# OpenMendel/MendelIHT.jl

Measured on NVIDIA B200. Metric: iht_iterations_per_sec, higher is better.
Workload: dtype f64 (sweep: f32 LUT partials per slab of 640 samples (512 without the ternary copy), f64 across slabs; top-k candidates re-scored in f64)

## Files before the change

mendeliht.jl_b200/csrc/common.cuh:

```cuda
#pragma once
#include <cuda_runtime.h>
#include <stdint.h>
#include <stdio.h>
#include <memory>
#include <string>
#include <vector>
#include <stdexcept>
#include "../../include/ihtb200.h"

namespace ihtb {

struct Error : std::runtime_error {
    int code;
    Error(int c, const std::string& m) : std::runtime_error(m), code(c) {}
};
void set_last_error(const std::string& m);
const std::string& last_error();
struct LaunchCounter {
    int64_t v = 0;
    LaunchCounter& operator++(int) { __atomic_fetch_add(&v, 1, __ATOMIC_RELAXED); return *this; }
    operator int64_t() const { return __atomic_load_n(&v, __ATOMIC_RELAXED); }
};
LaunchCounter& launch_counter();
bool debug_sync();

#define IHTB_CUDA(call)                                                                      \
    do {                                                                                     \
        cudaError_t e__ = (call);                                                            \
        if (e__ != cudaSuccess)                                                              \
            throw ::ihtb::Error(IHTB_ECUDA, std::string(#call) + ": " + cudaGetErrorString(e__)); \
    } while (0)

#define IHTB_CHECK(cond, code, msg)                                  \
    do {                                                             \
        if (!(cond)) throw ::ihtb::Error((code), (msg));             \
    } while (0)

#define IHTB_LAUNCH(kernel, grid, block, smem, stream, ...)          \
    do {                                                             \
        kernel<<<(grid), (block), (smem), (stream)>>>(__VA_ARGS__);  \
        ::ihtb::launch_counter()++;                                  \
        IHTB_CUDA(cudaGetLastError());                               \
        if (::ihtb::debug_sync()) {                                  \
            cudaError_t e2__ = cudaStreamSynchronize(stream);        \
            if (e2__ != cudaSuccess)                                 \
                throw ::ihtb::Error(IHTB_ECUDA, std::string("kernel " #kernel " failed: ") + cudaGetErrorString(e2__)); \
        }                                                            \
    } while (0)

template <typename F>
static inline int32_t guard(F&& f) {
    try {
        f();
        return IHTB_OK;
    } catch (const Error& e) {
        set_last_error(e.what());
        return e.code;
    } catch (const std::bad_alloc&) {
        set_last_error("out of host memory");
        return IHTB_ENOMEM;
    } catch (const std::exception& e) {
        set_last_error(e.what());
        return IHTB_EINVAL;
    }
}

template <typename T>
struct DBuf {
    T* p = nullptr;
    size_t n = 0;
    DBuf() = default;
    explicit DBuf(size_t count) { alloc(count); }
    DBuf(const DBuf&) = delete;
    DBuf& operator=(const DBuf&) = delete;
    ~DBuf() { release(); }
    void alloc(size_t count) {
        release();
        n = count;
        if (count) {
            cudaError_t e = cudaMalloc((void**)&p, count * sizeof(T));
            if (e != cudaSuccess) {
                p = nullptr; n = 0;
                throw Error(IHTB_ENOMEM, std::string("cudaMalloc of ") + std::to_string(count * sizeof(T)) +
                                             " bytes failed: " + cudaGetErrorString(e));
            }
        }
    }
    void release() {
        if (p) cudaFree(p);
        p = nullptr; n = 0;
    }
    void zero(cudaStream_t s) { if (n) IHTB_CUDA(cudaMemsetAsync(p, 0, n * sizeof(T), s)); }
};

template <typename T>
struct HBuf {
    T* p = nullptr;
    size_t n = 0;
    HBuf() = default;
    HBuf(const HBuf&) = delete;
    HBuf& operator=(const HBuf&) = delete;
    ~HBuf() { if (p) cudaFreeHost(p); }
    void alloc(size_t count) {
        if (p) cudaFreeHost(p);
        p = nullptr; n = count;
        if (count) IHTB_CUDA(cudaMallocHost((void**)&p, count * sizeof(T)));
    }
};

static inline int64_t ceil_div(int64_t a, int64_t b) { return (a + b - 1) / b; }

bool smem_attr_needed(const void* kernel, int device);
template <typename K>
static inline void ensure_dynamic_smem(K kernel, int bytes) {
    int dev = 0;
    IHTB_CUDA(cudaGetDevice(&dev));
    if (!smem_attr_needed(reinterpret_cast<const void*>(kernel), dev)) return;
    IHTB_CUDA(cudaFuncSetAttribute(kernel, cudaFuncAttributeMaxDynamicSharedMemorySize, bytes));
}

struct TopkFuse;
ihtb_geno* dense_new_handle(int64_t n, int64_t p, int dtype, int standardize, int32_t den = 0);
void dense_upload(ihtb_geno* g, const void* x, int64_t ld_host, int64_t j_dst, int64_t ncols);
void dense_finalize(ihtb_geno* g);
int64_t dense_stream_bytes(const ihtb_geno* g);
void dense_decode_block(const ihtb_geno* g, int64_t i0, int64_t i1, int64_t j0, int64_t j1, double* d_out);
void dense_xt_v(const ihtb_geno* g, const double* dV, int64_t m, double* dOut, cudaStream_t s, DBuf<double>* part,
                const TopkFuse* tf);
void dense_sweep_kernel_only(const ihtb_geno* g, const double* dV, DBuf<double>* part, cudaStream_t s);
void dense_x_support(const ihtb_geno* g, const int64_t* d_idx, int64_t k, const double* d_coef, int64_t m,
                     double* d_out, cudaStream_t s);
void dense_xt_gather2(const ihtb_geno* g, const int64_t* d_cols_a, int64_t n_a, const int64_t* d_cols_b, int64_t n_b,
                      const double* d_v, int64_t m, double* d_out, cudaStream_t s);
void dense_init_beta_moments(const ihtb_geno* g, const double* d_w, const double* d_wy, double* d_sx, double* d_sxx,
                             double* d_sxy, cudaStream_t s);
void dense_decode_cols(const ihtb_geno* g, const int64_t* d_cols, int64_t k, double* d_out, cudaStream_t s);
const double* geno_bound_scale(const ihtb_geno* g);
double geno_bound_coef(const ihtb_geno* g, double plink_coef);

}

enum { GENO_PLINK = 0, GENO_DENSE = 1 };

struct ihtb_geno {
    int kind = 0;
    int device = 0;
    int64_t n = 0;
    int64_t p = 0;
    int64_t j0 = 0;
    int64_t nbytes = 0;
    int64_t stride = 0;
    int64_t cs_j = 0, cs_s = 0;
    int quad = 0;
    int64_t p4 = 0;
    int center = 1, scale = 1, impute = 1;
    int sm_count = 148;
    ihtb::DBuf<uint8_t> bed;
    ihtb::DBuf<uint8_t> tern;
    int64_t tern_slabs = 0;
    ihtb::DBuf<double> mu, sinv;
    ihtb::DBuf<double> sgn;
    ihtb::DBuf<int32_t> nmiss;
    ihtb::DBuf<int64_t> miss_ptr;
    ihtb::DBuf<int32_t> miss_idx;
    int64_t total_missing = 0;
    bool ready = false;
    int dtype = 0;
    int standardize = 0;
    int32_t den = 0;
    int64_t ld = 0;
    ihtb::DBuf<uint8_t> dense;
    ihtb::DBuf<double> dscale;
    double dcoef = 0.0;
    std::shared_ptr<void> bgen_stage;
};
static inline bool geno_is_dense(const ihtb_geno* g) { return g->kind == GENO_DENSE; }

static inline void geno_require_ready(const ihtb_geno* g) {
    IHTB_CHECK(g && g->ready, IHTB_EINVAL, "genotype handle is not finalized (ihtb_geno_finalize)");
}

struct GenoView {
    const uint8_t* bed;
    int64_t cs_j, cs_s, nbytes, stride, n, p;
    int quad;
    const double* mu;
    const double* sinv;
    const int32_t* nmiss;
    int impute;
};
static inline GenoView geno_view(const ihtb_geno* g) {
    return GenoView{g->bed.p, g->cs_j, g->cs_s, g->nbytes, g->stride, g->n, g->p, g->quad, g->mu.p, g->sinv.p,
                    g->nmiss.p, g->impute};
}
__device__ __forceinline__ const uint8_t* gv_ptr(const GenoView& g, int64_t j, int64_t b) {
    if (g.quad)
        return g.bed + (b >> 7) * g.cs_s + (j >> 2) * 512 + ((b & 127) >> 2) * 16 + (j & 3) * 4 + (b & 3);
    return g.bed + j * g.cs_j + (b >> 7) * g.cs_s + (b & 127);
}

namespace ihtb {

__device__ __forceinline__ double warp_sum(double v) {
#pragma unroll
    for (int o = 16; o > 0; o >>= 1) v += __shfl_xor_sync(0xffffffffu, v, o);
    return v;
}
__device__ __forceinline__ float warp_sum(float v) {
#pragma unroll
    for (int o = 16; o > 0; o >>= 1) v += __shfl_xor_sync(0xffffffffu, v, o);
    return v;
}
__device__ __forceinline__ int warp_sum(int v) {
#pragma unroll
    for (int o = 16; o > 0; o >>= 1) v += __shfl_xor_sync(0xffffffffu, v, o);
    return v;
}

__device__ __forceinline__ double block_sum(double v, double* sh) {
    v = warp_sum(v);
    int lane = threadIdx.x & 31, w = threadIdx.x >> 5;
    __syncthreads();
    if (lane == 0) sh[w] = v;
    __syncthreads();
    int nw = (blockDim.x + 31) >> 5;
    v = (threadIdx.x < nw) ? sh[threadIdx.x] : 0.0;
    if (w == 0) v = warp_sum(v);
    return v;
}

void sweep_xt_v(const ihtb_geno* g, const double* dV, int64_t m, double* dOut, int mode, cudaStream_t s,
                double* sweep_seconds);
void x_support(const ihtb_geno* g, const int64_t* d_idx_local, int64_t k, const double* d_coef, int64_t m,
               double* d_out, cudaStream_t s);
void xt_gather(const ihtb_geno* g, const int64_t* d_cols_local, int64_t ncols, const double* d_v, int64_t m,
               const double* d_vsum , double* d_out , cudaStream_t s);
void xt_gather2(const ihtb_geno* g, const int64_t* d_cols_a, int64_t n_a, const int64_t* d_cols_b, int64_t n_b,
                const double* d_v, int64_t m, const double* d_vsum, double* d_out, cudaStream_t s, bool blocked = false);

struct TopkFuse;
void dense_xt_v(const ihtb_geno* g, const double* dV, int64_t m, double* dOut, cudaStream_t s, void* scratch_any,
                const TopkFuse* tf);
void dense_x_support(const ihtb_geno* g, const int64_t* d_idx, int64_t k, const double* d_coef, int64_t m,
                     double* d_out, cudaStream_t s);
void dense_xt_gather2(const ihtb_geno* g, const int64_t* d_cols_a, int64_t n_a, const int64_t* d_cols_b, int64_t n_b,
                      const double* d_v, int64_t m, double* d_out, cudaStream_t s);
void dense_init_beta_moments(const ihtb_geno* g, const double* d_w, const double* d_wy, double* d_sx, double* d_sxx,
                             double* d_sxy, cudaStream_t s, void* scratch_any);
void dense_decode_cols(const ihtb_geno* g, const int64_t* d_cols, int64_t k, double* d_out, cudaStream_t s);
const double* geno_bound_scale(const ihtb_geno* g);
double geno_bound_coef(const ihtb_geno* g, double plink_coef);

}
```

mendeliht.jl_b200/csrc/fit.cu:

```cuda
#include "glm.cuh"
#include "topk.cuh"
#include "comm.cuh"
#include "debias.cuh"
#include "groups.cuh"
#include "pairer.cuh"
#include <algorithm>
#include <chrono>
#include <cmath>
#include <memory>
#include <mutex>
#include <string.h>
#include <unordered_map>

namespace ihtb {
void sweep_xt_v_with_means(const ihtb_geno* g, const double* dV, const double* vbar_host, int64_t m, double* dOut,
                           int mode, cudaStream_t s, void* scratch_any, float* sweep_ms, double* d_l2 = nullptr,
                           const TopkFuse* tf = nullptr);
void* sweep_scratch_create();
void sweep_scratch_destroy(void* p);
void sweep_class_sums(const ihtb_geno* g, const double* d_v, double* d_w1, double* d_w2, double* d_wm, cudaStream_t s,
                      void* scratch_any);
}

using namespace ihtb;

static const double kFastBound = 1.0 / 262144.0;
static const double kExactBound = 1e-13;
static const double kPairBound = 3.1 / 2048.0;

struct ihtb_fit {
    const ihtb_geno* g = nullptr;
    int device = 0;
    int64_t n = 0, p = 0, q = 0;
    ihtb_comm* comm = nullptr;
    int64_t j0 = 0, p_global = 0;
    std::vector<int64_t> shard_j0;
    DBuf<int64_t> d_selall, d_pack, d_packall;
    HBuf<int64_t> h_selall, h_packall;
    int capx = 512;
    ihtb_cfg cfg{};
    cudaStream_t s = nullptr;
    std::vector<uint8_t> zkeep;
    int zkeepn = 0;
    int cap = 4096;

    DBuf<unsigned> d_done;
    DBuf<double> d_y, d_z, d_w, d_xb, d_zc, d_mu, d_r, d_xs, d_dfa, d_part, d_scal, d_small, d_coef, d_gout,
        d_vbar;
    DBuf<uint8_t> d_mask;
    DBuf<uint32_t> d_keyL, d_keyU;
    DBuf<int> d_hist;
    DBuf<int64_t> d_sel;
    DBuf<int64_t> d_idx, d_cols;
    HBuf<double> h_scal, h_gout;
    HBuf<int64_t> h_sel;
    void* sweep_scratch = nullptr;
    cudaEvent_t ev0 = nullptr, ev1 = nullptr, tm0 = nullptr, tm1 = nullptr;
    bool sweep_pending = false;
    struct FusedStep {
        std::vector<int64_t> uni_loc;
        size_t maxsupp = 0;
        int M = 0;
        int winner = -1;
    };
    FusedStep* fz = nullptr;
    DBuf<double> d_pick;
    HBuf<double> h_pick;
    SweepPairer* pairer = nullptr;
    int pair_slot = 0;
    double sweep_coef = kFastBound;
    GlmCtx glm{};
    TopkCtx tk{};

    std::vector<int64_t> idx, idx0, best_idx;
    std::vector<double> b, b0, best_b;
    std::vector<double> c, c0, best_c, df2, h_y, h_mu;
    std::vector<uint8_t> idc, idc0;
    std::unordered_map<int64_t, double> df_exact;
    std::vector<double> wt;
    DBuf<double> d_wt;
    double w_at(int64_t j) const { return wt.empty() ? 1.0 : wt[(size_t)j]; }
    void set_weights(const double* w) {
        if (!w) { wt.clear(); tk.wt = nullptr; return; }
        for (int64_t j = 0; j < p_global; ++j)
            IHTB_CHECK(w[j] > 0.0 && std::isfinite(w[j]), IHTB_EDOMAIN, "weights must be positive and finite");
        wt.assign(w, w + p_global);
        if (d_wt.n < (size_t)p) d_wt.alloc((size_t)p);
        IHTB_CUDA(cudaMemcpyAsync(d_wt.p, wt.data() + j0, (size_t)p * sizeof(double), cudaMemcpyHostToDevice, s));
        sync();
        tk.wt = d_wt.p;
    }
    std::vector<int64_t> cand_cache;
    bool df_sparse = false;
    std::vector<int64_t> dfs_idx;
    std::vector<double> dfs_val;
    double rbar = 0.0, bound = 0.0, sum_w = 0.0, sum_wy = 0.0, last_dev = 0.0, denom_next = 0.0;
    bool denom_ready = false;
    bool inited = false;

    int64_t n_sweeps = 0, n_backtracks = 0, n_cand_iter = 0, n_pair_overflow = 0;
    int last_count = 0;
    double sweep_ms_total = 0.0;
    double pve = 0.0;

    ~ihtb_fit() {
        if (sweep_scratch) sweep_scratch_destroy(sweep_scratch);
        if (ev0) cudaEventDestroy(ev0);
        if (ev1) cudaEventDestroy(ev1);
        if (tm0) cudaEventDestroy(tm0);
        if (tm1) cudaEventDestroy(tm1);
        if (s) cudaStreamDestroy(s);
    }

    void sync() { IHTB_CUDA(cudaStreamSynchronize(s)); }
    void readback_scal(int nv) {
        IHTB_CUDA(cudaMemcpyAsync(h_scal.p, d_scal.p, nv * sizeof(double), cudaMemcpyDeviceToHost, s));
        sync();
    }
    template <typename T>
    void upload(T* dst, const T* src, size_t count) {
        if (count) IHTB_CUDA(cudaMemcpyAsync(dst, src, count * sizeof(T), cudaMemcpyHostToDevice, s));
    }

    bool is_local(int64_t j) const { return j >= j0 && j < j0 + p; }
    int nranks() const { return comm ? comm->nranks : 1; }

    void support_matvec(const std::vector<int64_t>& cols, const std::vector<double>& coef, double* d_out) {
        std::vector<int64_t> ii; std::vector<double> vv;
        for (size_t t = 0; t < cols.size(); ++t)
            if (coef[t] != 0.0 && is_local(cols[t])) { ii.push_back(cols[t] - j0); vv.push_back(coef[t]); }
        if (!ii.empty()) {
            upload(d_idx.p, ii.data(), ii.size());
            upload(d_coef.p, vv.data(), vv.size());
        }
        support_matvec_dev(ii.empty() ? nullptr : d_idx.p, (int64_t)ii.size(), d_coef.p, d_out);
    }

    void support_matvec_dev(const int64_t* d_idx_loc, int64_t k_loc, const double* d_coef_loc, double* d_out) {
        support_matvec_dev_m(d_idx_loc, k_loc, d_coef_loc, 1, d_out);
    }
    void support_matvec_dev_m(const int64_t* d_idx_loc, int64_t k_loc, const double* d_coef_loc, int m, double* d_out) {
        const size_t cnt = (size_t)n * (size_t)m;
        if (!comm) {
            if (k_loc > 0) x_support(g, d_idx_loc, k_loc, d_coef_loc, m, d_out, s);
            else IHTB_CUDA(cudaMemsetAsync(d_out, 0, cnt * sizeof(double), s));
            return;
        }
        if (m == 1 && p2p_pushall_ok(comm, cnt)) {
            if (k_loc > 0) x_support_push(g, d_idx_loc, k_loc, d_coef_loc, comm, s);
            else p2p_push(comm, nullptr, cnt, s);
            p2p_reduce(comm, d_out, cnt, s);
            return;
        }
        if (p2p_mapped(comm) && cnt <= comm->red_cap) {
            double* part = p2p_partial_ptr(comm);
            if (k_loc > 0) x_support(g, d_idx_loc, k_loc, d_coef_loc, m, part, s);
            else IHTB_CUDA(cudaMemsetAsync(part, 0, cnt * sizeof(double), s));
            p2p_allreduce_2phase(comm, cnt, d_out, s);
            return;
        }
        if (k_loc > 0) x_support(g, d_idx_loc, k_loc, d_coef_loc, m, d_out, s);
        else IHTB_CUDA(cudaMemsetAsync(d_out, 0, cnt * sizeof(double), s));
        comm_allreduce_sum_f64(comm, d_out, cnt, s);
    }

    void update_xb() { support_matvec(idx, b, d_xb.p); }

    double glm_update(int add_zc) {
        upload(d_small.p, c.data(), (size_t)q);
        glm_mu(glm, d_small.p, add_zc, s);
        readback_scal(3);
        double dev = h_scal.p[0], lp = h_scal.p[1], sw = h_scal.p[2];
        last_dev = dev;
        if (cfg.dist == IHTB_NORMAL) {
            double phi = dev / (double)n;
            double sigma = std::sqrt(phi);
            return -0.5 * (dev / phi) - sw * (0.5 * std::log(2.0 * M_PI) + std::log(sigma));
        }
        return lp;
    }

    static double digamma(double x) {
        double r = 0.0;
        while (x < 6.0) { r -= 1.0 / x; x += 1.0; }
        double f = 1.0 / (x * x);
        return r + std::log(x) - 0.5 / x -
               f * (1.0 / 12 - f * (1.0 / 120 - f * (1.0 / 252 - f * (1.0 / 240 - f * (1.0 / 132)))));
    }
    static double trigamma(double x) {
        double r = 0.0;
        while (x < 6.0) { r += 1.0 / (x * x); x += 1.0; }
        double f = 1.0 / (x * x);
        return r + 1.0 / x + f / 2 + f / x * (1.0 / 6 - f * (1.0 / 30 - f * (1.0 / 42 - f * (1.0 / 30))));
    }
    void fetch_mu() {
        h_mu.resize((size_t)n);
        IHTB_CUDA(cudaMemcpyAsync(h_mu.data(), d_mu.p, n * sizeof(double), cudaMemcpyDeviceToHost, s));
        sync();
    }
    double nb_logl(double r) {
        glm.nb_r = r;
        return glm_update(1);
    }
    void mle_for_r() {
        fetch_mu();
        const std::vector<double>& y = h_y;
        double r = glm.nb_r;
        if (cfg.est_r == 1) {
            double num = 0.0, den = 0.0;
            for (int64_t i = 0; i < n; ++i) {
                for (int64_t j = 0; j <= (int64_t)y[i] - 1; ++j) num += r / (r + (double)j);
                den += std::log(r / (r + h_mu[i]));
            }
            glm.nb_r = -num / den;
            return;
        }
        auto d1 = [&](double rr) {
            double a = 0.0;
            for (int64_t i = 0; i < n; ++i)
                a += -(y[i] + rr) / (h_mu[i] + rr) - std::log(h_mu[i] + rr) + 1.0 + std::log(rr) + digamma(rr + y[i]) -
                     digamma(rr);
            return a;
        };
        auto d2 = [&](double rr) {
            double a = 0.0;
            for (int64_t i = 0; i < n; ++i)
                a += (y[i] + rr) / ((h_mu[i] + rr) * (h_mu[i] + rr)) - 2.0 / (h_mu[i] + rr) + 1.0 / rr +
                     trigamma(rr + y[i]) - trigamma(rr);
            return a;
        };
        double new_r = 1.0, stepsize = 1.0;
        for (int it = 0; it < 100; ++it) {
            double dx = d1(r), dx2 = d2(r);
            double increment = dx2 < 0 ? dx / dx2 : dx;
            new_r = r - stepsize * increment;
            double old_logl = nb_logl(r);
            for (int j = 0; j < 20; ++j) {
                if (new_r <= 0) {
                    stepsize /= 2; new_r = r - stepsize * increment;
                } else {
                    double new_logl = nb_logl(new_r);
                    if (old_logl >= new_logl) { stepsize /= 2; new_r = r - stepsize * increment; }
                    else break;
                }
            }
            if (std::fabs(r - new_r) <= 1e-6) { glm.nb_r = new_r; return; }
            r = new_r;
        }
        glm.nb_r = r;
    }
    double mu_r_logl() {
        double l = glm_update(1);
        if (cfg.est_r != 0) {
            mle_for_r();
            l = glm_update(1);
        }
        return l;
    }

    void exact_df(const std::vector<int64_t>& cols, bool exchange = true) {
        std::vector<int64_t> need;
        for (int64_t j : cols)
            if (!df_exact.count(j) && (exchange || is_local(j))) need.push_back(j);
        if (need.empty()) { if (!exchange) sync(); return; }
        IHTB_CHECK((int64_t)need.size() <= (int64_t)d_cols.n, IHTB_ENUMERIC, "too many columns to re-score");
        std::vector<int64_t> loc(need.size());
        for (size_t t = 0; t < need.size(); ++t) loc[t] = is_local(need[t]) ? need[t] - j0 : -1;
        upload(d_cols.p, loc.data(), loc.size());
        xt_gather2(g, d_cols.p, (int64_t)need.size(), nullptr, 0, d_r.p, 1, d_vbar.p, d_gout.p, s,
                   false);
        if (exchange) comm_allreduce_sum_f64(comm, d_gout.p, need.size(), s);
        IHTB_CUDA(cudaMemcpyAsync(h_gout.p, d_gout.p, need.size() * sizeof(double), cudaMemcpyDeviceToHost, s));
        sync();
        for (size_t t = 0; t < need.size(); ++t) df_exact[need[t]] = h_gout.p[t];
        n_cand_iter += (int64_t)need.size();
    }

    void score_and_sweep() {
        glm_score(glm, s, d_vbar.p);
        IHTB_CUDA(cudaMemcpyAsync(h_scal.p, d_scal.p, (2 + q) * sizeof(double), cudaMemcpyDeviceToHost, s));
        IHTB_CUDA(cudaEventRecord(ev0, s));
        sweep_coef = geno_bound_coef(g, cfg.sweep_mode == IHTB_SWEEP_FAST ? kFastBound : kExactBound);
        const double t_sw = now();
        if (pairer && cfg.sweep_mode == IHTB_SWEEP_FAST) {
            IHTB_CHECK(!grouped() && !comm, IHTB_EUNSUPPORTED, "paired sweeps serve plain single-device fits only");
            if (pairer->sweep(pair_slot, g, d_r.p, d_vbar.p, d_dfa.p, s, sweep_scratch)) {
                sweep_coef = kPairBound;
                IHTB_CUDA(cudaMemcpyAsync(h_scal.p + 3 + q, pairer->d_l2 + pair_slot, sizeof(double), cudaMemcpyDeviceToHost, s));
            }
        } else if (cfg.k > 0 && !(grouped() && !init_plain)) {
            const TopkFuse tf = topk_absdf_fuse_begin(tk, geno_bound_scale(g), d_scal.p, sweep_coef);
            sweep_xt_v_with_means(g, d_r.p, d_vbar.p, 1, d_dfa.p, cfg.sweep_mode, s, sweep_scratch, nullptr, nullptr, &tf);
        } else {
            sweep_xt_v_with_means(g, d_r.p, d_vbar.p, 1, d_dfa.p, cfg.sweep_mode, s, sweep_scratch, nullptr);
        }
        IHTB_CUDA(cudaEventRecord(ev1, s));
        ++n_sweeps;
        const double t_sel = now();
        dbg[0] += t_sel - t_sw;
        select_rescore(false);
        dbg[1] += now() - t_sel;
    }

    void select_rescore(bool rerun) {
        if (grouped() && !init_plain) {
            select_groups(rerun);
            if (!rerun) finish_sweep_scalars(sweep_coef);
            return;
        }
        df_exact.clear(); cand_cache.clear();
        df_sparse = false;
        const double coef = sweep_coef;
        std::vector<std::pair<int64_t, double>> cvals;
        const bool fused = fz != nullptr && !rerun;
        std::vector<int64_t> supp_loc;
        if (fused) supp_loc = fz->uni_loc;
        else
            for (int64_t j : idx)
                if (is_local(j)) supp_loc.push_back(j - j0);
        const int nsupp = (int)supp_loc.size();
        const int64_t* d_supp = fused ? d_idx.p : d_cols.p;
        int glaunch = 0;
        if (cfg.k > 0) {
            const int64_t ksel = cfg.k + (int64_t)(fused ? fz->maxsupp : idx.size());
            const bool paired = coef == kPairBound;
            if (tk.fused_hist) topk_candidates_absdf_finish(tk, ksel, s);
            else
                topk_candidates_absdf(tk, d_dfa.p, paired ? g->sgn.p : geno_bound_scale(g), rerun ? nullptr : d_scal.p, coef, ksel, s,
                                      bound, (paired && !rerun) ? pairer->d_l2 + pair_slot : nullptr);
            const int64_t want = sweep_coef == kPairBound ? std::max<int64_t>(ksel + 1024, last_count + last_count / 4 + 256)
                                                          : ksel + 64;
            glaunch = (int)std::min<int64_t>(comm ? capx / 2 : cap, want);
        }
        if (nsupp && !fused) upload(d_cols.p, supp_loc.data(), supp_loc.size());
        xt_gather2(g, tk.cand, glaunch, d_supp, nsupp, d_r.p, 1, d_vbar.p, d_gout.p, s);
        denom_ready = false;
        if (!rerun) {
            if (fused) {
                glm_winner_coef(d_pick.p, d_coefM.p, nsupp, d_gout.p + glaunch, d_coef.p, d_cM.p, q, d_small.p + q, s);
                support_matvec_dev(d_supp, nsupp, d_coef.p, d_xs.p);
                IHTB_CUDA(cudaMemcpyAsync(h_pick.p, d_pick.p, (size_t)(1 + fz->M) * sizeof(double), cudaMemcpyDeviceToHost, s));
                IHTB_CUDA(cudaMemcpyAsync(h_scalM.p, d_scalM.p, (size_t)(3 * fz->M) * sizeof(double), cudaMemcpyDeviceToHost, s));
            } else {
                support_matvec_dev(d_supp, nsupp, d_gout.p + glaunch, d_xs.p);
                std::vector<double> mask((size_t)q);
                for (int64_t l = 0; l < q; ++l) mask[l] = idc[l] ? 1.0 : 0.0;
                upload(d_small.p + q, mask.data(), (size_t)q);
            }
            glm_stepsize(glm, d_scal.p + 2, d_xs.p, s, d_small.p + q, d_scal.p + 2 + q);
            IHTB_CUDA(cudaMemcpyAsync(h_scal.p + 2 + q, d_scal.p + 2 + q, sizeof(double), cudaMemcpyDeviceToHost, s));
            denom_ready = true;
        }
        if (!comm) {
            IHTB_CUDA(cudaMemcpyAsync(h_sel.p, d_sel.p, (2 + glaunch) * sizeof(int64_t), cudaMemcpyDeviceToHost, s));
            IHTB_CUDA(cudaMemcpyAsync(h_gout.p, d_gout.p, (glaunch + nsupp) * sizeof(double), cudaMemcpyDeviceToHost, s));
            sync();
            const double t_host = now();
            struct Acc { double& a; double t0; ~Acc() { a += now() - t0; } } acc_host{dbg[2], t_host};
            if (fused) adopt_winner();
            const TopkState* st = reinterpret_cast<const TopkState*>(h_sel.p);
            const int count = cfg.k > 0 ? st->count : 0;
            dbg[3] += (double)std::min(count, glaunch);
            if (count > cap && coef == kPairBound && !rerun) {
                ++n_pair_overflow;
                sweep_coef = kFastBound;
                sweep_xt_v_with_means(g, d_r.p, d_vbar.p, 1, d_dfa.p, IHTB_SWEEP_FAST, s, sweep_scratch, nullptr);
                IHTB_CUDA(cudaEventRecord(ev1, s));
                select_rescore(false);
                return;
            }
            IHTB_CHECK(count <= cap, IHTB_ENUMERIC,
                       "degenerate projection: more than " + std::to_string(cap) +
                           " entries lie within the sweep error bound of the k-th largest |gradient|");
            last_count = count;
            cvals.reserve((size_t)count);
            for (int t = 0; t < std::min(count, glaunch); ++t) cvals.push_back({h_sel.p[2 + t], h_gout.p[t]});
            for (int t = 0; t < nsupp; ++t) df_exact[supp_loc[t] + j0] = h_gout.p[glaunch + t];
            if (count > glaunch) {
                IHTB_CUDA(cudaMemcpyAsync(h_sel.p, d_sel.p, (2 + count) * sizeof(int64_t), cudaMemcpyDeviceToHost, s));
                sync();
                std::vector<int64_t> rest(h_sel.p + 2 + glaunch, h_sel.p + 2 + count);
                exact_df(rest);
                for (int64_t j : rest) cvals.push_back({j, df_exact.at(j)});
            }
        } else {
            const int nr = nranks();
            const size_t blk = 2 + 2 * (size_t)capx;
            IHTB_CHECK(nsupp <= capx / 2, IHTB_ENUMERIC, "support too large for the sharded candidate exchange");
            pack_sweep_candidates(d_pack.p, reinterpret_cast<const TopkState*>(d_sel.p), tk.cand, glaunch, d_gout.p,
                                  d_supp, nsupp, d_gout.p + glaunch, j0, capx, s);
            comm_allgather_i64(comm, d_pack.p, d_packall.p, blk, s);
            IHTB_CUDA(cudaMemcpyAsync(h_packall.p, d_packall.p, nr * blk * sizeof(int64_t), cudaMemcpyDeviceToHost, s));
            sync();
            if (fused) adopt_winner();
            for (int r = 0; r < nr; ++r) {
                const int64_t* b_ = h_packall.p + (size_t)r * blk;
                IHTB_CHECK(b_[0] <= glaunch, IHTB_ENUMERIC,
                           "degenerate projection: too many local candidates within the sweep error bound");
                const int half = capx / 2;
                auto take = [&](int t, bool is_cand) {
                    const int64_t j = b_[2 + t];
                    if (j < 0) return;
                    double v;
                    memcpy(&v, &b_[2 + capx + t], sizeof(double));
                    if (is_cand) cvals.push_back({j, v});
                    else df_exact[j] = v;
                };
                for (int t = 0; t < (int)b_[0]; ++t) take(t, true);
                for (int t = 0; t < (int)b_[1]; ++t) take(half + t, false);
            }
        }
        std::sort(cvals.begin(), cvals.end());
        cvals.erase(std::unique(cvals.begin(), cvals.end(), [](const std::pair<int64_t, double>& x, const std::pair<int64_t, double>& y) {
                        return x.first == y.first; }), cvals.end());
        n_cand_iter += (int64_t)cvals.size();
        std::vector<char> keep(cvals.size(), 1);
        if ((int64_t)cvals.size() > cfg.k) {
            std::vector<std::pair<double, size_t>> outside;
            outside.reserve(cvals.size());
            for (size_t t = 0; t < cvals.size(); ++t)
                if (!std::binary_search(idx.begin(), idx.end(), cvals[t].first))
                    outside.push_back({std::fabs(cvals[t].second) * w_at(cvals[t].first), t});
            if ((int64_t)outside.size() > cfg.k) {
                std::nth_element(outside.begin(), outside.begin() + (cfg.k - 1), outside.end(),
                                 [](const std::pair<double, size_t>& x, const std::pair<double, size_t>& y) {
                                     return x.first > y.first;
                                 });
                const double thr = outside[(size_t)cfg.k - 1].first * (1.0 - 1e-12);
                std::fill(keep.begin(), keep.end(), 0);
                for (const auto& e : outside)
                    if (e.first >= thr) keep[e.second] = 1;
            }
        }
        for (size_t t = 0; t < cvals.size(); ++t)
            if (keep[t]) {
                cand_cache.push_back(cvals[t].first);
                df_exact[cvals[t].first] = cvals[t].second;
            }
        if (rerun) return;
        finish_sweep_scalars(coef);
    }

    void finish_sweep_scalars(double coef) {
        float ms = 0.f;
        IHTB_CUDA(cudaEventElapsedTime(&ms, ev0, ev1));
        sweep_ms_total += ms;
        double rsum = h_scal.p[0], rl1 = h_scal.p[1];
        for (int64_t l = 0; l < q; ++l) df2[l] = h_scal.p[2 + l];
        denom_next = h_scal.p[2 + q];
        rbar = rsum / (double)n;
        bound = coef == kPairBound ? coef * h_scal.p[3 + q]
                                   : coef * (rl1 + std::fabs(rsum));
    }

    double df_at(int64_t j) const {
        if (df_sparse) {
            auto it = std::lower_bound(dfs_idx.begin(), dfs_idx.end(), j);
            return (it != dfs_idx.end() && *it == j) ? dfs_val[it - dfs_idx.begin()] : 0.0;
        }
        return df_exact.at(j);
    }

    double stepsize() {
        std::vector<double> coef(idx.size());
        double numer = 0.0;
        for (size_t t = 0; t < idx.size(); ++t) { coef[t] = df_at(idx[t]); numer += coef[t] * coef[t]; }
        if (denom_ready && !df_sparse) {
            denom_ready = false;
            for (int64_t l = 0; l < q; ++l)
                if (idc[l]) numer += df2[l] * df2[l];
            double eta = numer / denom_next;
            if (std::isinf(eta) || std::isnan(eta)) eta = 1e-8;
            return eta;
        }
        denom_ready = false;
        support_matvec(idx, coef, d_xs.p);
        std::vector<double> d2((size_t)q);
        for (int64_t l = 0; l < q; ++l) {
            d2[l] = idc[l] ? df2[l] : 0.0;
            if (idc[l]) numer += df2[l] * df2[l];
        }
        upload(d_small.p + q, d2.data(), (size_t)q);
        glm_stepsize(glm, d_small.p + q, d_xs.p, s);
        readback_scal(1);
        double denom = h_scal.p[0];
        double eta = numer / denom;
        if (std::isinf(eta) || std::isnan(eta)) eta = 1e-8;
        return eta;
    }

    static double b_lookup(const std::vector<int64_t>& ii, const std::vector<double>& vv, int64_t j) {
        auto it = std::lower_bound(ii.begin(), ii.end(), j);
        return (it != ii.end() && *it == j) ? vv[it - ii.begin()] : 0.0;
    }

    void gradstep(double eta) {
        if (grouped()) { gradstep_group(eta); return; }
        std::vector<int64_t> cand;
        cand = df_sparse ? dfs_idx : cand_cache;
        cand.insert(cand.end(), idx0.begin(), idx0.end());
        std::sort(cand.begin(), cand.end());
        cand.erase(std::unique(cand.begin(), cand.end()), cand.end());

        struct Item { double a; int64_t pos; double v; };
        std::vector<Item> items;
        items.reserve(cand.size() + (size_t)q);
        for (int64_t j : cand) {
            double v = b_lookup(idx0, b0, j) + eta * df_at(j);
            if (!wt.empty()) {
                const double w = wt[(size_t)j], a = v * w;
                items.push_back({std::fabs(a), j, a / w});
            } else {
                items.push_back({std::fabs(v), j, v});
            }
        }
        for (int64_t l = 0; l < q; ++l) {
            c[l] = c0[l] + eta * df2[l];
            if (!zkeep[l]) items.push_back({std::fabs(c[l]), p_global + l, c[l]});
        }
        int64_t k = cfg.k;
        std::sort(items.begin(), items.end(), [](const Item& x, const Item& y) {
            return x.a > y.a || (x.a == y.a && x.pos < y.pos);
        });
        idx.clear(); b.clear();
        const double thr = project_threshold(items, k);
        std::vector<std::pair<int64_t, double>> keep;
        for (size_t t = 0; t < items.size(); ++t) {
            const bool kept = items[t].a >= thr;
            if (items[t].pos >= p_global) {
                if (!kept) c[items[t].pos - p_global] = 0.0;
            } else if (kept && items[t].v != 0.0) {
                keep.push_back({items[t].pos, items[t].v});
            }
        }
        for (int64_t l = 0; l < q; ++l) idc[l] = c[l] != 0.0;
        choose_prune(keep);
        std::sort(keep.begin(), keep.end());
        for (auto& kv : keep) { idx.push_back(kv.first); b.push_back(kv.second); }
    }

    template <typename ItemT>
    static double project_threshold(const std::vector<ItemT>& sorted_items, int64_t k) {
        if (k <= 0) return INFINITY;
        return (int64_t)sorted_items.size() >= k ? sorted_items[(size_t)k - 1].a : 0.0;
    }
    void choose_prune(std::vector<std::pair<int64_t, double>>& keep) const {
        int64_t nonzero = (int64_t)keep.size() - zkeepn;
        for (int64_t l = 0; l < q; ++l) nonzero += idc[l] ? 1 : 0;
        const int64_t limit = cfg.k + zkeepn;
        if (nonzero <= limit) return;
        std::vector<std::pair<int64_t, double>> byabs = keep;
        std::sort(byabs.begin(), byabs.end(), [](const std::pair<int64_t, double>& x, const std::pair<int64_t, double>& y) {
            return std::fabs(x.second) < std::fabs(y.second) || (std::fabs(x.second) == std::fabs(y.second) && x.first > y.first);
        });
        const size_t excess = std::min<size_t>((size_t)(nonzero - limit), byabs.size());
        for (size_t t = 0; t < excess; ++t) keep.erase(std::find(keep.begin(), keep.end(), byabs[t]));
    }

    std::unique_ptr<GroupCtx> grpctx;
    bool init_plain = false;
    bool grouped() const { return (bool)grpctx; }
    void set_groups(const int32_t* group1, int J, const int64_t* ks, int64_t n_groups) {
        if (!group1) { grpctx.reset(); return; }
        IHTB_CHECK(J >= 0, IHTB_EINVAL, "Value of J (max number of groups) must be nonnegative!");
        std::unique_ptr<GroupCtx> gc(new GroupCtx());
        std::vector<double> h_sinv((size_t)p);
        IHTB_CUDA(cudaMemcpy(h_sinv.data(), geno_bound_scale(g), (size_t)p * sizeof(double), cudaMemcpyDeviceToHost));
        gc->build(p, j0, p_global, group1, J, ks, n_groups, cfg.k, h_sinv.data());
        grpctx = std::move(gc);
    }

    void select_groups(bool rerun) {
        GroupCtx& gc = *grpctx;
        df_exact.clear(); cand_cache.clear();
        df_sparse = false; denom_ready = false;
        const double coef = sweep_coef;
        group_topk(gc, d_dfa.p, geno_bound_scale(g), rerun ? nullptr : d_scal.p, coef, bound, cfg.k, s);
        const size_t G = (size_t)gc.G, nT = 2 * G + 1;
        const int nr = nranks();
        std::vector<double> TL(G), TU(G);
        bool overflow = false;
        if (comm) {
            if (gc.d_Tall.n < nT * (size_t)nr) { gc.d_Tall.alloc(nT * (size_t)nr); gc.h_Tall.alloc(nT * (size_t)nr); }
            comm_allgather_i64(comm, reinterpret_cast<const int64_t*>(gc.d_gT.p), gc.d_Tall.p, nT, s);
            IHTB_CUDA(cudaMemcpyAsync(gc.h_Tall.p, gc.d_Tall.p, nT * (size_t)nr * sizeof(int64_t), cudaMemcpyDeviceToHost, s));
            sync();
            std::fill(TL.begin(), TL.end(), 0.0); std::fill(TU.begin(), TU.end(), 0.0);
            for (int rk = 0; rk < nr; ++rk) {
                const double* T = reinterpret_cast<const double*>(gc.h_Tall.p) + (size_t)rk * nT;
                for (size_t gi = 0; gi < G; ++gi) { TL[gi] = std::max(TL[gi], T[gi]); TU[gi] += T[G + gi]; }
                overflow = overflow || T[2 * G] != 0.0;
            }
        } else {
            IHTB_CUDA(cudaMemcpyAsync(gc.h_gT.p, gc.d_gT.p, nT * sizeof(double), cudaMemcpyDeviceToHost, s));
            sync();
            for (size_t gi = 0; gi < G; ++gi) { TL[gi] = gc.h_gT.p[gi]; TU[gi] = gc.h_gT.p[G + gi]; }
            overflow = gc.h_gT.p[2 * G] != 0.0;
        }
        IHTB_CHECK(!overflow, IHTB_ENUMERIC,
                   "degenerate group projection: too many entries of one group lie within the sweep error bound of its "
                   "2k-th largest |gradient|");
        std::vector<char> has(G, 0);
        for (int64_t j : idx) has[(size_t)gc.grp[(size_t)j]] = 1;
        std::vector<int32_t> chosen;
        std::vector<double> lows;
        for (size_t gi = 0; gi < G; ++gi) {
            if (has[gi]) chosen.push_back((int32_t)gi);
            else lows.push_back(TL[gi]);
        }
        if (gc.J > 0 && !lows.empty()) {
            const size_t need = std::min<size_t>((size_t)gc.J, lows.size());
            std::nth_element(lows.begin(), lows.begin() + (need - 1), lows.end(), std::greater<double>());
            const double thr = lows[need - 1];
            for (size_t gi = 0; gi < G; ++gi)
                if (!has[gi] && TU[gi] >= thr) chosen.push_back((int32_t)gi);
        }
        IHTB_CHECK(chosen.size() <= 65536, IHTB_ENUMERIC, "degenerate group projection: too many groups tie at the J-th norm");
        std::sort(chosen.begin(), chosen.end());
        const int nc = (int)chosen.size();
        const int64_t nsupp = (int64_t)idx.size();
        const int64_t list_slots = (int64_t)nc * gc.lcap, slots = list_slots + nsupp;
        if (slots == 0) return;
        gc.ensure_chosen(std::max(nc, 1));
        if (gc.d_oidx.n < (size_t)slots) {
            gc.d_oidx.alloc((size_t)slots); gc.d_oval.alloc((size_t)slots);
            gc.h_oidx.alloc((size_t)slots); gc.h_oval.alloc((size_t)slots);
        }
        if (nc) {
            IHTB_CUDA(cudaMemcpyAsync(gc.d_chosen.p, chosen.data(), (size_t)nc * sizeof(int32_t), cudaMemcpyHostToDevice, s));
            group_take(gc, nc, s);
        }
        std::vector<int64_t> supp_loc((size_t)nsupp);
        for (int64_t t = 0; t < nsupp; ++t) supp_loc[(size_t)t] = is_local(idx[(size_t)t]) ? idx[(size_t)t] - j0 : -1;
        upload(gc.d_oidx.p + list_slots, supp_loc.data(), (size_t)nsupp);
        xt_gather(g, gc.d_oidx.p, slots, d_r.p, 1, d_vbar.p, gc.d_oval.p, s);
        auto take = [&](int64_t t, int64_t j, double v) {
            if (j < 0) return;
            df_exact[j] = v;
            if (t < list_slots) cand_cache.push_back(j);
        };
        if (comm) {
            const size_t blk = 2 * (size_t)slots;
            if (gc.d_blk.n < blk) gc.d_blk.alloc(blk);
            if (gc.d_blkall.n < blk * (size_t)nr) { gc.d_blkall.alloc(blk * (size_t)nr); gc.h_blkall.alloc(blk * (size_t)nr); }
            group_pack(gc.d_oidx.p, gc.d_oval.p, slots, j0, gc.d_blk.p, s);
            comm_allgather_i64(comm, gc.d_blk.p, gc.d_blkall.p, blk, s);
            IHTB_CUDA(cudaMemcpyAsync(gc.h_blkall.p, gc.d_blkall.p, blk * (size_t)nr * sizeof(int64_t), cudaMemcpyDeviceToHost, s));
            sync();
            for (int rk = 0; rk < nr; ++rk) {
                const int64_t* b_ = gc.h_blkall.p + (size_t)rk * blk;
                for (int64_t t = 0; t < slots; ++t) {
                    double v;
                    memcpy(&v, &b_[slots + t], sizeof(double));
                    take(t, b_[t], v);
                }
            }
        } else {
            IHTB_CUDA(cudaMemcpyAsync(gc.h_oidx.p, gc.d_oidx.p, (size_t)slots * sizeof(int64_t), cudaMemcpyDeviceToHost, s));
            IHTB_CUDA(cudaMemcpyAsync(gc.h_oval.p, gc.d_oval.p, (size_t)slots * sizeof(double), cudaMemcpyDeviceToHost, s));
            sync();
            for (int64_t t = 0; t < slots; ++t) take(t, gc.h_oidx.p[t], gc.h_oval.p[t]);
        }
        std::sort(cand_cache.begin(), cand_cache.end());
        cand_cache.erase(std::unique(cand_cache.begin(), cand_cache.end()), cand_cache.end());
        n_cand_iter += (int64_t)cand_cache.size();
    }

    struct GItem { double a; int64_t j; double v; int g; };
    std::vector<std::pair<int64_t, double>> project_groups(std::vector<GItem>& items) const {
        const GroupCtx& gc = *grpctx;
        std::sort(items.begin(), items.end(), [](const GItem& x, const GItem& y) { return x.a > y.a || (x.a == y.a && x.j < y.j); });
        std::unordered_map<int, std::pair<int64_t, double>> acc;
        for (const GItem& it : items) {
            auto& e = acc[it.g];
            if (e.first < gc.k_of(it.g, cfg.k)) { e.second += it.v * it.v; ++e.first; }
        }
        std::vector<std::pair<double, int>> order;
        for (const auto& kv : acc) order.push_back({kv.second.second, kv.first});
        std::sort(order.begin(), order.end(), [](const std::pair<double, int>& x, const std::pair<double, int>& y) {
            return x.first > y.first || (x.first == y.first && x.second < y.second);
        });
        std::unordered_map<int, int> rank;
        for (size_t i = 0; i < order.size(); ++i) rank[order[i].second] = (int)i + 1;
        std::unordered_map<int, int64_t> cnt;
        std::vector<std::pair<int64_t, double>> keep;
        for (const GItem& it : items) {
            int64_t& c_ = cnt[it.g];
            if (rank[it.g] > gc.J || c_ >= gc.k_of(it.g, cfg.k)) continue;
            ++c_;
            if (it.v != 0.0) keep.push_back({it.j, it.v});
        }
        std::sort(keep.begin(), keep.end());
        return keep;
    }

    void gradstep_group(double eta) {
        const GroupCtx& gc = *grpctx;
        std::vector<int64_t> cand = df_sparse ? dfs_idx : cand_cache;
        cand.insert(cand.end(), idx0.begin(), idx0.end());
        std::sort(cand.begin(), cand.end());
        cand.erase(std::unique(cand.begin(), cand.end()), cand.end());
        std::vector<GItem> items;
        items.reserve(cand.size());
        for (int64_t j : cand) {
            const double v = b_lookup(idx0, b0, j) + eta * df_at(j);
            items.push_back({std::fabs(v), j, v, gc.grp[(size_t)j]});
        }
        for (int64_t l = 0; l < q; ++l) c[l] = c0[l] + eta * df2[l];
        auto keep = project_groups(items);
        for (int64_t l = 0; l < q; ++l) idc[l] = c[l] != 0.0;
        if (!gc.ks_vector) {
            int64_t nonzero = (int64_t)keep.size() - zkeepn;
            for (int64_t l = 0; l < q; ++l) nonzero += idc[l] ? 1 : 0;
            const int64_t limit = (int64_t)(gc.J == 0 ? 1 : gc.J) * (cfg.k + zkeepn);
            if (nonzero > limit) {
                std::vector<std::pair<int64_t, double>> byabs = keep;
                std::sort(byabs.begin(), byabs.end(), [](const std::pair<int64_t, double>& x, const std::pair<int64_t, double>& y) {
                    return std::fabs(x.second) < std::fabs(y.second) || (std::fabs(x.second) == std::fabs(y.second) && x.first > y.first);
                });
                const size_t excess = std::min<size_t>((size_t)(nonzero - limit), byabs.size());
                for (size_t t = 0; t < excess; ++t)
                    keep.erase(std::find(keep.begin(), keep.end(), byabs[t]));
            }
        }
        idx.clear(); b.clear();
        for (auto& kv : keep) { idx.push_back(kv.first); b.push_back(kv.second); }
    }

    DebiasWs debias_ws;
    void debias() {
        if (idx.empty()) return;
        std::vector<int64_t> loc(idx.size());
        for (size_t t = 0; t < idx.size(); ++t) loc[t] = is_local(idx[t]) ? idx[t] - j0 : -1;
        upload(d_cols.p, loc.data(), loc.size());
        debias_irls(g, d_y.p, cfg.dist, cfg.link, glm.nb_r, d_cols.p, (int)idx.size(), b.data(), debias_ws, s, comm);
        ++n_debias;
    }
    int64_t n_debias = 0;

    double save_prev(double cur, double best) {
        idx0 = idx; b0 = b; c0 = c; idc0 = idc;
        if (cur > best) { best_idx = idx; best_b = b; best_c = c; }
        return std::max(cur, best);
    }

    double check_convergence() const {
        double the_norm = 0.0, b0max = 0.0;
        size_t i = 0, j = 0;
        while (i < idx.size() || j < idx0.size()) {
            double x = 0.0, y = 0.0;
            if (j >= idx0.size() || (i < idx.size() && idx[i] < idx0[j])) x = b[i++];
            else if (i >= idx.size() || idx0[j] < idx[i]) y = b0[j++];
            else { x = b[i++]; y = b0[j++]; }
            the_norm = std::max(the_norm, std::fabs(x - y));
            b0max = std::max(b0max, std::fabs(y));
        }
        for (int64_t l = 0; l < q; ++l) {
            the_norm = std::max(the_norm, std::fabs(c[l] - c0[l]));
            b0max = std::max(b0max, std::fabs(c0[l]));
        }
        return the_norm / (b0max + 1.0);
    }

    void save_best_model() {
        idx.clear(); b.clear();
        for (size_t t = 0; t < best_idx.size(); ++t)
            if (best_b[t] != 0.0) { idx.push_back(best_idx[t]); b.push_back(best_b[t]); }
        c = best_c;
        for (int64_t l = 0; l < q; ++l) idc[l] = c[l] != 0.0;
        update_xb();
        glm_update(0);
    }

    void compute_pve() {
        glm_sum2(glm, d_mu.p, d_y.p, s);
        readback_scal(2);
        double mm = h_scal.p[0] / (double)n, my = h_scal.p[1] / (double)n;
        glm_ssq2(glm, d_mu.p, mm, d_y.p, my, s);
        readback_scal(2);
        pve = h_scal.p[0] / h_scal.p[1];
    }

    void do_init_beta() {
        IHTB_CHECK(cfg.dist == IHTB_NORMAL, IHTB_EINVAL, "Intializing beta values only work for Gaussian phenotypes! Sorry!");
        DBuf<double> cls((size_t)(7 * p));
        double *W1 = cls.p, *W2 = W1 + p, *Wm = W2 + p, *Y1 = Wm + p, *Y2 = Y1 + p, *Ym = Y2 + p, *bd = Ym + p;
        init_beta_products(glm, d_xs.p, s);
        if (geno_is_dense(g)) {
            dense_init_beta_moments(g, d_w.p, d_xs.p, W1, W2, Wm, s);
            n_sweeps += 1;
            init_beta_solve_moments(glm, p, W1, W2, Wm, sum_w, sum_wy, bd, s);
        } else {
            sweep_class_sums(g, d_w.p, W1, W2, Wm, s, sweep_scratch);
            sweep_class_sums(g, d_xs.p, Y1, Y2, Ym, s, sweep_scratch);
            n_sweeps += 2;
            init_beta_solve(glm, p, W1, W2, Wm, Y1, Y2, Ym, sum_w, sum_wy, g->mu.p, g->sinv.p, g->impute, bd, s);
        }
        if (comm) comm_allreduce_sum_f64(comm, d_scal.p, 1, s);
        readback_scal(1);
        double c0sum = h_scal.p[0];
        std::fill(c.begin(), c.end(), 0.0);
        if (q > 1) {
            init_beta_cov_sums(glm, s);
            readback_scal(3 * ((int)q - 1));
            for (int64_t l = 1; l < q; ++l) {
                double sx = h_scal.p[3 * (l - 1)], sxx = h_scal.p[3 * (l - 1) + 1], sxy = h_scal.p[3 * (l - 1) + 2];
                double icpt = sum_wy, slope = sxy;
                double u11 = std::sqrt(sum_w), u12 = sx / u11, dd = sxx - u12 * u12;
                if (sum_w > 0 && dd > 0) {
                    double u22 = std::sqrt(dd), t1 = sum_wy / u11, t2 = (sxy - u12 * t1) / u22;
                    slope = t2 / u22; icpt = (t1 - u12 * slope) / u11;
                }
                c0sum += icpt;
                c[l] = std::min(std::max(slope, -2.0), 2.0);
            }
        }
        c[0] = std::min(std::max(c0sum / (double)(p_global + q - 1), -2.0), 2.0);
        std::vector<int64_t> cand;
        if (cfg.k > 0) {
            topk_candidates(tk, bd, nullptr, g->sinv.p, 1.0, 0.0, cfg.k, s);
            IHTB_CUDA(cudaMemcpyAsync(h_sel.p, d_sel.p, (2 + cap) * sizeof(int64_t), cudaMemcpyDeviceToHost, s));
            sync();
            const TopkState* st = reinterpret_cast<const TopkState*>(h_sel.p);
            IHTB_CHECK(st->count <= cap, IHTB_ENUMERIC, "degenerate projection of the initial beta (too many ties)");
            cand.assign(h_sel.p + 2, h_sel.p + 2 + st->count);
            std::sort(cand.begin(), cand.end());
        }
        std::vector<double> vals(cand.size());
        if (!cand.empty()) {
            upload(d_cols.p, cand.data(), cand.size());
            take_values(bd, d_cols.p, (int64_t)cand.size(), d_gout.p, s);
            IHTB_CUDA(cudaMemcpyAsync(vals.data(), d_gout.p, cand.size() * sizeof(double), cudaMemcpyDeviceToHost, s));
            sync();
        }
        if (comm) {
            const size_t blk = 2 + 2 * (size_t)capx;
            IHTB_CHECK((int64_t)cand.size() <= capx, IHTB_ENUMERIC, "degenerate projection of the initial beta (too many ties)");
            std::vector<int64_t> mine(blk, 0);
            mine[0] = (int64_t)cand.size();
            for (size_t t = 0; t < cand.size(); ++t) {
                mine[2 + t] = cand[t] + j0;
                memcpy(&mine[2 + capx + t], &vals[t], sizeof(double));
            }
            upload(d_pack.p, mine.data(), blk);
            comm_allgather_i64(comm, d_pack.p, d_packall.p, blk, s);
            const int nr = nranks();
            IHTB_CUDA(cudaMemcpyAsync(h_packall.p, d_packall.p, nr * blk * sizeof(int64_t), cudaMemcpyDeviceToHost, s));
            sync();
            cand.clear(); vals.clear();
            for (int rk = 0; rk < nr; ++rk) {
                const int64_t* b_ = h_packall.p + (size_t)rk * blk;
                for (int64_t t = 0; t < b_[0]; ++t) {
                    double v;
                    memcpy(&v, &b_[2 + capx + t], sizeof(double));
                    cand.push_back(b_[2 + t]);
                    vals.push_back(v);
                }
            }
        }
        struct Item { double a; int64_t pos; double v; };
        std::vector<Item> items;
        for (size_t t = 0; t < cand.size(); ++t) {
            const double w = w_at(cand[t]), a = vals[t] * w;
            items.push_back({std::fabs(a), cand[t], wt.empty() ? vals[t] : a / w});
        }
        for (int64_t l = 0; l < q; ++l)
            if (!zkeep[l]) items.push_back({std::fabs(c[l]), p_global + l, c[l]});
        std::sort(items.begin(), items.end(), [](const Item& x, const Item& y) {
            return x.a > y.a || (x.a == y.a && x.pos < y.pos);
        });
        const double thr = project_threshold(items, cfg.k);
        std::vector<std::pair<int64_t, double>> keep;
        for (size_t t = 0; t < items.size(); ++t) {
            const bool kept = items[t].a >= thr;
            if (items[t].pos >= p_global) {
                if (!kept) c[items[t].pos - p_global] = 0.0;
            } else if (kept && items[t].v != 0.0) {
                keep.push_back({items[t].pos, items[t].v});
            }
        }
        std::sort(keep.begin(), keep.end());
        idx.clear(); b.clear();
        for (auto& kv : keep) { idx.push_back(kv.first); b.push_back(kv.second); }
        for (int64_t l = 0; l < q; ++l) idc[l] = c[l] != 0.0;
        select_rescore(true);
    }

    void init(const uint8_t* train_mask, bool init_beta = false) {
        idx.clear(); b.clear(); idx0.clear(); b0.clear(); best_idx.clear(); best_b.clear();
        c.assign((size_t)q, 0.0); c0 = c; best_c = c; df2.assign((size_t)q, 0.0);
        idc.assign(zkeep.begin(), zkeep.end()); idc0 = idc;
        df_exact.clear(); dfs_idx.clear(); dfs_val.clear(); df_sparse = false;
        last_bt = kMaxBatch;
        d_xb.zero(s);
        const uint8_t* dm = nullptr;
        if (train_mask) {
            upload(d_mask.p, train_mask, (size_t)n);
            dm = d_mask.p;
        }
        glm_set_weights(glm, dm, s);
        readback_scal(2);
        sum_w = h_scal.p[0];
        sum_wy = h_scal.p[1];
        double ybar = h_scal.p[1] / sum_w;
        for (int it = 0; it < 20; ++it) {
            double g1 = glm_linkinv(cfg.link, c[0]);
            double g2 = glm_mueta(cfg.link, c[0]);
            double step = (g1 - ybar) / g2;
            step = std::min(std::max(step, -1.0), 1.0);
            c[0] = c[0] - step;
            if (std::fabs(g1 - ybar) < 1e-10) break;
        }
        glm_update(1);
        init_plain = grouped() && !grpctx->ks_vector && !init_beta;
        score_and_sweep();
        init_plain = false;
        if (grouped() && grpctx->ks_vector && !init_beta) {
            std::vector<GItem> items;
            for (int64_t j : cand_cache) { double v = df_exact.at(j); items.push_back({std::fabs(v), j, v, grpctx->grp[(size_t)j]}); }
            auto keep = project_groups(items);
            for (auto& kv : keep) { dfs_idx.push_back(kv.first); dfs_val.push_back(kv.second); }
            df_sparse = true;
            idx.clear(); b.clear();
            for (int64_t l = 0; l < q; ++l) idc[l] = 1;
            inited = true;
            return;
        }
        if (init_beta) {
            do_init_beta();
            inited = true;
            return;
        }
        std::vector<int64_t> cand = cand_cache;
        struct Item { double a; int64_t pos; double v; };
        std::vector<Item> items;
        for (int64_t j : cand) {
            double v = df_exact.at(j);
            const double w = w_at(j), a = v * w;
            items.push_back({std::fabs(a), j, wt.empty() ? v : a / w});
        }
        for (int64_t l = 0; l < q; ++l)
            if (!zkeep[l]) items.push_back({std::fabs(df2[l]), p_global + l, df2[l]});
        std::sort(items.begin(), items.end(), [](const Item& x, const Item& y) {
            return x.a > y.a || (x.a == y.a && x.pos < y.pos);
        });
        const double thr = project_threshold(items, cfg.k);
        std::vector<std::pair<int64_t, double>> keep;
        for (size_t t = 0; t < items.size(); ++t) {
            const bool kept = items[t].a >= thr;
            if (items[t].pos >= p_global) {
                if (!kept) df2[items[t].pos - p_global] = 0.0;
            } else if (kept && items[t].v != 0.0) {
                keep.push_back({items[t].pos, items[t].v});
            }
        }
        std::sort(keep.begin(), keep.end());
        for (auto& kv : keep) { dfs_idx.push_back(kv.first); dfs_val.push_back(kv.second); }
        df_sparse = true;
        for (int64_t l = 0; l < q; ++l) idc[l] = zkeep[l];
        choose_prune(keep);
        std::sort(keep.begin(), keep.end());
        idx.clear();
        for (auto& kv : keep) idx.push_back(kv.first);
        b.assign(idx.size(), 0.0);
        inited = true;
    }

    double phase[4] = {0, 0, 0, 0};
    double dbg[6] = {0, 0, 0, 0, 0, 0};
    static double now() {
        return std::chrono::duration<double>(std::chrono::steady_clock::now().time_since_epoch()).count();
    }
    static constexpr int kMaxBatch = 4;
    static constexpr int64_t kAdaptiveBatchN = 131072;
    int last_bt = kMaxBatch;
    DBuf<double> d_xbM, d_zcM, d_muM, d_partM, d_scalM, d_cM, d_coefM;
    HBuf<double> h_scalM;
    bool batch_ok() const {
        static const bool off = [] { const char* e = getenv("IHTB_NO_BATCH"); return e && *e == '1'; }();
        return !off && cfg.est_r == 0 && cfg.max_step >= 1 && cfg.max_step + 1 <= kMaxBatch;
    }
    struct StepModel { double eta; std::vector<int64_t> idx; std::vector<double> b, c; std::vector<uint8_t> idc; };
    std::vector<StepModel> step_models;
    void ensure_batch_buffers() {
        if (d_xbM.n < (size_t)(kMaxBatch * n)) {
            d_xbM.alloc((size_t)(kMaxBatch * n)); d_zcM.alloc((size_t)(kMaxBatch * n)); d_muM.alloc((size_t)(kMaxBatch * n));
            d_partM.alloc((size_t)kMaxBatch * GLM_MAX_BLOCKS * 3); d_scalM.alloc(kMaxBatch * 3); h_scalM.alloc(kMaxBatch * 3);
            d_cM.alloc((size_t)(kMaxBatch * q)); d_coefM.alloc((size_t)kMaxBatch * (size_t)cap);
            d_pick.alloc(1 + kMaxBatch); h_pick.alloc(1 + kMaxBatch);
        }
    }
    struct StepPlan { int M; int m0; std::vector<int64_t> uni, loc; size_t UL; };
    StepPlan plan_step(double eta0, int m0 = 0, int m1 = -1) {
        const int Mtot = cfg.max_step + 1;
        if (m1 < 0) m1 = Mtot;
        if (m0 == 0) step_models.assign((size_t)Mtot, StepModel{});
        for (int m = m0; m < m1; ++m) {
            double e = eta0;
            for (int i = 0; i < m; ++i) e /= 2;
            if (m) { idx = idx0; b = b0; c = c0; }
            gradstep(e);
            step_models[(size_t)m] = StepModel{e, idx, b, c, idc};
        }
        const int M = m1 - m0;
        StepPlan pl; pl.M = M; pl.m0 = m0;
        for (int m = m0; m < m1; ++m) {
            const StepModel& md = step_models[(size_t)m];
            pl.uni.insert(pl.uni.end(), md.idx.begin(), md.idx.end());
        }
        std::sort(pl.uni.begin(), pl.uni.end());
        pl.uni.erase(std::unique(pl.uni.begin(), pl.uni.end()), pl.uni.end());
        const size_t U = pl.uni.size();
        IHTB_CHECK(U * (size_t)M <= d_coefM.n && U <= d_idx.n, IHTB_ENUMERIC, "support union too large for the batched step");
        std::vector<size_t> keep_pos;
        for (size_t t = 0; t < U; ++t)
            if (is_local(pl.uni[t])) { pl.loc.push_back(pl.uni[t] - j0); keep_pos.push_back(t); }
        pl.UL = pl.loc.size();
        std::vector<double> coefL(pl.UL * (size_t)M, 0.0), cM((size_t)(M * q));
        for (int m = 0; m < M; ++m) {
            const StepModel& md = step_models[(size_t)(m0 + m)];
            size_t u = 0;
            for (size_t t = 0; t < md.idx.size(); ++t) {
                if (!is_local(md.idx[t])) continue;
                const int64_t lj = md.idx[t] - j0;
                while (pl.loc[u] != lj) ++u;
                coefL[u + (size_t)m * pl.UL] = md.b[t];
            }
            for (int64_t l = 0; l < q; ++l) cM[(size_t)(m * q + l)] = md.c[(size_t)l];
        }
        if (pl.UL) {
            upload(d_idx.p, pl.loc.data(), pl.UL);
            upload(d_coefM.p, coefL.data(), coefL.size());
        }
        upload(d_cM.p, cM.data(), cM.size());
        return pl;
    }
    void adopt_model(int m) {
        const StepModel& win = step_models[(size_t)m];
        idx = win.idx; b = win.b; c = win.c; idc = win.idc;
    }
    double logl_from_sums(const double* s3) const {
        if (cfg.dist == IHTB_NORMAL) {
            const double dev = s3[0], sw = s3[2], phi = dev / (double)n, sigma = std::sqrt(phi);
            return -0.5 * (dev / phi) - sw * (0.5 * std::log(2.0 * M_PI) + std::log(sigma));
        }
        return s3[1];
    }

    void one_step_batched(double old_logl, double& eta, int& eta_step, double& new_logl) {
        ensure_batch_buffers();
        double t0 = now();
        const double eta0 = stepsize();
        double t1 = now(); phase[0] += t1 - t0;
        const int Mtot = cfg.max_step + 1;
        int first = Mtot;
        if (n >= kAdaptiveBatchN) first = std::min(Mtot, last_bt + 1 + (last_bt > 0 ? 1 : 0));
        const StepPlan pl = plan_step(eta0, 0, first);
        double t2 = now(); phase[1] += t2 - t1;
        finish_batched(pl, eta0, t2, old_logl, eta, eta_step, new_logl);
    }
    void finish_batched(const StepPlan& pl, double eta0, double t2, double old_logl, double& eta, int& eta_step,
                        double& new_logl) {
        const int Mtot = cfg.max_step + 1;
        auto eval = [&](const StepPlan& P) {
            const size_t off = (size_t)P.m0 * (size_t)n;
            support_matvec_dev_m(P.UL ? d_idx.p : nullptr, (int64_t)P.UL, d_coefM.p, P.M, d_xbM.p + off);
            glm_mu_batched(glm, d_cM.p, P.M, d_xbM.p + off, d_zcM.p + off, d_muM.p + off, d_partM.p, d_scalM.p + 3 * P.m0, s);
            IHTB_CUDA(cudaMemcpyAsync(h_scalM.p + 3 * P.m0, d_scalM.p + 3 * P.m0, (size_t)(3 * P.M) * sizeof(double),
                                      cudaMemcpyDeviceToHost, s));
            sync();
        };
        int have = pl.M;
        eval(pl);
        int sidx = 0;
        new_logl = logl_from_sums(h_scalM.p);
        while (old_logl > new_logl && sidx < cfg.max_step) {
            ++sidx;
            if (sidx >= have) { eval(plan_step(eta0, have, Mtot)); have = Mtot; }
            new_logl = logl_from_sums(h_scalM.p + 3 * sidx);
            ++n_backtracks;
        }
        last_bt = sidx;
        adopt_model(sidx);
        eta = step_models[(size_t)sidx].eta; eta_step = sidx;
        last_dev = h_scalM.p[3 * sidx];
        const size_t nb = (size_t)n * sizeof(double);
        IHTB_CUDA(cudaMemcpyAsync(d_xb.p, d_xbM.p + (size_t)sidx * n, nb, cudaMemcpyDeviceToDevice, s));
        IHTB_CUDA(cudaMemcpyAsync(d_zc.p, d_zcM.p + (size_t)sidx * n, nb, cudaMemcpyDeviceToDevice, s));
        IHTB_CUDA(cudaMemcpyAsync(d_mu.p, d_muM.p + (size_t)sidx * n, nb, cudaMemcpyDeviceToDevice, s));
        double t3 = now(); phase[2] += t3 - t2;
        score_and_sweep();
        phase[3] += now() - t3;
        IHTB_CHECK(!std::isnan(new_logl), IHTB_ENUMERIC, "Loglikelihood function is NaN, aborting...");
        IHTB_CHECK(!std::isinf(new_logl), IHTB_ENUMERIC, "Loglikelihood function is Inf, aborting...");
    }

    bool fuse_ok() const {
        const char* e = getenv("IHTB_FUSE");
        return e && *e == '1' && !grouped() && denom_ready && !df_sparse;
    }
    void adopt_winner() {
        fz->winner = (int)h_pick.p[0];
        adopt_model(fz->winner);
    }
    void one_step_fused(double old_logl, double& eta, int& eta_step, double& new_logl) {
        ensure_batch_buffers();
        double t0 = now();
        const double eta0 = stepsize();
        double t1 = now(); phase[0] += t1 - t0;
        const StepPlan pl = plan_step(eta0);
        const int M = pl.M;
        double t2 = now(); phase[1] += t2 - t1;
        if (comm && pl.UL > (size_t)capx / 2) {
            finish_batched(pl, eta0, t2, old_logl, eta, eta_step, new_logl);
            return;
        }
        support_matvec_dev_m(pl.UL ? d_idx.p : nullptr, (int64_t)pl.UL, d_coefM.p, M, d_xbM.p);
        glm_mu_batched(glm, d_cM.p, M, d_xbM.p, d_zcM.p, d_muM.p, d_partM.p, d_scalM.p, s);
        glm_pick_model(glm, d_scalM.p, M, old_logl, cfg.max_step, d_pick.p, d_xbM.p, d_zcM.p, d_muM.p, s);
        FusedStep ctx;
        ctx.uni_loc = pl.loc; ctx.M = M;
        for (const StepModel& md : step_models) ctx.maxsupp = std::max(ctx.maxsupp, md.idx.size());
        double t3 = now(); phase[2] += t3 - t2;
        fz = &ctx;
        try {
            score_and_sweep();
        } catch (...) {
            fz = nullptr;
            throw;
        }
        fz = nullptr;
        phase[3] += now() - t3;
        const int w = ctx.winner;
        n_backtracks += w;
        eta = step_models[(size_t)w].eta; eta_step = w;
        new_logl = h_pick.p[1 + w];
        last_dev = h_scalM.p[3 * w];
        IHTB_CHECK(!std::isnan(new_logl), IHTB_ENUMERIC, "Loglikelihood function is NaN, aborting...");
        IHTB_CHECK(!std::isinf(new_logl), IHTB_ENUMERIC, "Loglikelihood function is Inf, aborting...");
    }

    void one_step(double old_logl, double& eta, int& eta_step, double& new_logl) {
        if (batch_ok()) {
            if (fuse_ok()) one_step_fused(old_logl, eta, eta_step, new_logl);
            else one_step_batched(old_logl, eta, eta_step, new_logl);
            return;
        }
        double t0 = now();
        eta = stepsize();
        double t1 = now(); phase[0] += t1 - t0;
        gradstep(eta);
        double t2 = now(); phase[1] += t2 - t1;
        update_xb();
        new_logl = mu_r_logl();
        double t3 = now(); phase[2] += t3 - t2;
        eta_step = 0;
        while (old_logl > new_logl && eta_step < cfg.max_step) {
            eta /= 2;
            idx = idx0; b = b0; c = c0;
            double u0 = now();
            gradstep(eta);
            double u1 = now(); phase[1] += u1 - u0;
            update_xb();
            new_logl = mu_r_logl();
            phase[2] += now() - u1;
            ++eta_step;
            ++n_backtracks;
        }
        double t4 = now();
        score_and_sweep();
        phase[3] += now() - t4;
        IHTB_CHECK(!std::isnan(new_logl), IHTB_ENUMERIC, "Loglikelihood function is NaN, aborting...");
        IHTB_CHECK(!std::isinf(new_logl), IHTB_ENUMERIC, "Loglikelihood function is Inf, aborting...");
    }

    void run(ihtb_result* res, ihtb_iter_trace* trace, int64_t trace_cap) {
        IHTB_CHECK(inited, IHTB_EINVAL, "ihtb_fit_init must be called before ihtb_fit_run");
        auto t0 = std::chrono::steady_clock::now();
        int64_t launches0 = launch_counter();
        int64_t mm_iter = 0, n_steps = 0;
        double next_logl = -INFINITY, best_logl = -INFINITY;
        n_backtracks = 0;
        int64_t sweeps0 = n_sweeps;
        double sweep_ms0 = sweep_ms_total;
        for (int64_t iter = 1; iter <= cfg.max_iter; ++iter) {
            if (iter >= cfg.max_iter) {
                best_logl = save_prev(next_logl, best_logl);
                save_best_model();
                mm_iter = iter;
                break;
            }
            best_logl = save_prev(next_logl, best_logl);
            double eta; int eta_step;
            n_cand_iter = 0;
            one_step(next_logl, eta, eta_step, next_logl);
            ++n_steps;
            if (cfg.debias && iter >= 5 && idx == idx0) debias();
            double scaled_norm = check_convergence();
            if (trace && iter - 1 < trace_cap)
                trace[iter - 1] = ihtb_iter_trace{next_logl, scaled_norm, eta, eta_step, (int32_t)n_cand_iter};
            if (iter >= cfg.min_iter && scaled_norm < cfg.tol) {
                best_logl = save_prev(next_logl, best_logl);
                save_best_model();
                mm_iter = iter;
                break;
            }
        }
        compute_pve();
        IHTB_CHECK(!p2p_failed(comm), IHTB_ECUDA, "peer-memory all-reduce timed out waiting for another rank");
        inited = false;
        if (res) {
            res->time = std::chrono::duration<double>(std::chrono::steady_clock::now() - t0).count();
            res->logl = best_logl;
            res->iter = mm_iter;
            res->sigma_g = pve;
            res->n_sweeps = n_sweeps - sweeps0 + 1;
            res->n_backtracks = n_backtracks;
            res->sweep_seconds = (sweep_ms_total - sweep_ms0) * 1e-3;
            res->n_launches = launch_counter() - launches0;
            res->n_steps = n_steps;
        }
    }
};

extern "C" {

static std::mutex g_cache_mu;
static std::vector<ihtb_fit*> g_cache;
static const size_t kCacheMax = 16;

static ihtb_fit* cache_take(int device, int64_t n, int64_t p, int64_t q, int cap) {
    std::lock_guard<std::mutex> lk(g_cache_mu);
    for (size_t i = 0; i < g_cache.size(); ++i) {
        ihtb_fit* f = g_cache[i];
        if (f->device == device && f->n == n && f->p == p && f->q == q && f->cap == cap) {
            g_cache.erase(g_cache.begin() + i);
            return f;
        }
    }
    return nullptr;
}

void ihtb_internal_fit_cache_clear(int device) {
    std::vector<ihtb_fit*> drop;
    {
        std::lock_guard<std::mutex> lk(g_cache_mu);
        for (size_t i = 0; i < g_cache.size();) {
            if (device < 0 || g_cache[i]->device == device) { drop.push_back(g_cache[i]); g_cache.erase(g_cache.begin() + i); }
            else ++i;
        }
    }
    for (ihtb_fit* f : drop) { cudaSetDevice(f->device); delete f; }
}

static thread_local int t_min_cap = 0;
void ihtb_internal_next_fit_min_cap(int cap) { t_min_cap = cap; }

static ihtb_fit* fit_allocate(const ihtb_geno* g, int64_t q, int cap) {
    std::unique_ptr<ihtb_fit> f(new ihtb_fit());
    int64_t n = g->n, p = g->p;
    f->device = g->device; f->n = n; f->p = p; f->q = q; f->cap = cap;
    IHTB_CUDA(cudaStreamCreateWithFlags(&f->s, cudaStreamNonBlocking));
    IHTB_CUDA(cudaEventCreate(&f->ev0));
    IHTB_CUDA(cudaEventCreate(&f->ev1));
    f->d_y.alloc(n); f->d_z.alloc(n * q); f->d_w.alloc(n); f->d_xb.alloc(n); f->d_zc.alloc(n); f->d_mu.alloc(n);
    f->d_r.alloc(n); f->d_xs.alloc(n + 2 * (size_t)cap + 64); f->d_dfa.alloc(p); f->d_mask.alloc(n);
    f->d_part.alloc((size_t)GLM_MAX_BLOCKS * (2 + q)); f->d_scal.alloc(2 + q + 8); f->d_small.alloc(2 * q);
    size_t cols_cap = 2 * (size_t)cap + 64;
    f->d_coef.alloc(cols_cap); f->d_gout.alloc(cols_cap); f->d_vbar.alloc(1);
    f->d_idx.alloc(cols_cap); f->d_cols.alloc(cols_cap);
    f->d_keyL.alloc(p); f->d_keyU.alloc(p); f->d_hist.alloc(2 * 3 * 2048); f->d_sel.alloc(2 + cap);
    f->h_scal.alloc(2 + q + 8); f->h_gout.alloc(cols_cap); f->h_sel.alloc(2 + cap);
    f->sweep_scratch = sweep_scratch_create();
    f->d_hist.zero(f->s);
    return f.release();
}

int32_t ihtb_fit_create_sharded(const ihtb_geno* g, ihtb_comm* comm, int64_t p_global, const double* y,
                                const double* z, int64_t q, const uint8_t* zkeep, const ihtb_cfg* cfg, ihtb_fit** out);

int32_t ihtb_fit_create(const ihtb_geno* g, const double* y, const double* z, int64_t q, const uint8_t* zkeep,
                        const ihtb_cfg* cfg, ihtb_fit** out) {
    return ihtb_fit_create_sharded(g, nullptr, g ? g->p : 0, y, z, q, zkeep, cfg, out);
}

int32_t ihtb_fit_create_sharded(const ihtb_geno* g, ihtb_comm* comm, int64_t p_global, const double* y,
                                const double* z, int64_t q, const uint8_t* zkeep, const ihtb_cfg* cfg, ihtb_fit** out) {
    return guard([&] {
        IHTB_CHECK(g && y && z && cfg && out, IHTB_EINVAL, "NULL argument");
        IHTB_CHECK(p_global >= g->p, IHTB_EDIM, "p_global is smaller than the local shard");
        geno_require_ready(g);
        IHTB_CHECK(!(geno_is_dense(g) && comm && comm->nranks > 1), IHTB_EUNSUPPORTED,
                   "SNP-sharded fits need PLINK handles: a dense matrix is fitted on one device");
        IHTB_CHECK(q >= 1, IHTB_EDIM, "z must have at least the intercept column");
        IHTB_CHECK(cfg->k >= 0, IHTB_EINVAL, "Value of k (max predictors per group) must be nonnegative!");
        IHTB_CHECK(cfg->max_iter >= 0, IHTB_EINVAL, "Value of max_iter must be nonnegative!");
        IHTB_CHECK(cfg->max_step >= 0, IHTB_EINVAL, "Value of max_step must be nonnegative!");
        IHTB_CHECK(cfg->tol > 2.220446049250313e-16, IHTB_EINVAL, "Value of global tol must exceed machine precision!");
        IHTB_CHECK(cfg->dist >= IHTB_NORMAL && cfg->dist <= IHTB_NEGBIN, IHTB_EINVAL, "unknown distribution");
        IHTB_CHECK(cfg->link >= IHTB_LINK_IDENTITY && cfg->link <= IHTB_LINK_INVSQ, IHTB_EINVAL, "unknown link");
        IHTB_CHECK(cfg->sweep_mode == IHTB_SWEEP_FAST || cfg->sweep_mode == IHTB_SWEEP_EXACT, IHTB_EINVAL,
                   "bad sweep_mode");
        IHTB_CHECK(cfg->k <= p_global, IHTB_EINVAL, "k cannot exceed the number of SNPs");
        IHTB_CUDA(cudaSetDevice(g->device));
        int cap = (int)std::max<int64_t>(4096, 4 * cfg->k + 1024);
        if (t_min_cap > cap) cap = t_min_cap;
        t_min_cap = 0;
        std::unique_ptr<ihtb_fit> f(cache_take(g->device, g->n, g->p, q, cap));
        if (!f) f.reset(fit_allocate(g, q, cap));
        int64_t n = g->n, p = g->p;
        f->g = g; f->cfg = *cfg;
        f->comm = (comm && comm->nranks > 1) ? comm : nullptr;
        f->j0 = f->comm ? g->j0 : 0;
        f->p_global = f->comm ? p_global : g->p;
        f->shard_j0.clear();
        if (f->comm) {
            const int nr = comm->nranks;
            p2p_setup(comm, (size_t)ihtb_fit::kMaxBatch * (size_t)n,
                      (size_t)(2 + 2 * std::max<int64_t>(1024, 2 * (2 * cfg->k + 64 + 64))), f->s);
            if (f->d_selall.n < (size_t)nr * (2 + cap)) {
                f->d_selall.alloc((size_t)nr * (2 + cap));
                f->h_selall.alloc((size_t)nr * (2 + cap));
            }
            f->capx = (int)std::max<int64_t>(1024, 2 * (2 * cfg->k + 64 + 64));
            const size_t blk = 2 + 2 * (size_t)f->capx;
            if (f->d_packall.n < (size_t)nr * blk) {
                f->d_pack.alloc(blk);
                f->d_packall.alloc((size_t)nr * blk);
                f->h_packall.alloc((size_t)nr * blk);
            }
            int64_t mine = g->j0;
            IHTB_CUDA(cudaMemcpyAsync(f->d_sel.p, &mine, sizeof(int64_t), cudaMemcpyHostToDevice, f->s));
            comm_allgather_i64(comm, f->d_sel.p, f->d_selall.p, 1, f->s);
            f->shard_j0.resize(nr);
            IHTB_CUDA(cudaMemcpyAsync(f->shard_j0.data(), f->d_selall.p, nr * sizeof(int64_t), cudaMemcpyDeviceToHost,
                                      f->s));
            IHTB_CUDA(cudaStreamSynchronize(f->s));

        }
        f->zkeep.assign((size_t)q, 1);
        if (zkeep) for (int64_t l = 0; l < q; ++l) f->zkeep[l] = zkeep[l] ? 1 : 0;
        f->zkeepn = 0;
        for (auto v : f->zkeep) f->zkeepn += v;
        f->d_hist.zero(f->s);
        f->inited = false; f->sweep_pending = false; f->denom_ready = false;
        f->n_sweeps = 0; f->n_backtracks = 0; f->sweep_ms_total = 0.0;
        for (int i = 0; i < 4; ++i) f->phase[i] = 0.0;
        IHTB_CHECK(cfg->est_r == 0 || cfg->dist == IHTB_NEGBIN, IHTB_EINVAL,
                   "Only negative binomial regression currently supports nuisance parameter estimation");
        IHTB_CHECK(cfg->est_r >= 0 && cfg->est_r <= 2, IHTB_EINVAL, "Only support method is Newton or MM");
        if (cfg->est_r != 0) f->h_y.assign(y, y + n); else f->h_y.clear();
        IHTB_CUDA(cudaMemcpyAsync(f->d_y.p, y, n * sizeof(double), cudaMemcpyHostToDevice, f->s));
        IHTB_CUDA(cudaMemcpyAsync(f->d_z.p, z, n * q * sizeof(double), cudaMemcpyHostToDevice, f->s));
        f->d_xb.zero(f->s); f->d_zc.zero(f->s);
        f->glm = GlmCtx{n, q, f->d_z.p, f->d_y.p, f->d_w.p, f->d_xb.p, f->d_zc.p, f->d_mu.p, f->d_r.p, f->d_part.p,
                        f->d_scal.p, cfg->dist, cfg->link, cfg->nb_r};
        if (f->d_done.n < 8) { f->d_done.alloc(8); }
        IHTB_CUDA(cudaMemsetAsync(f->d_done.p, 0, 8 * sizeof(unsigned), f->s));
        f->glm.done = f->d_done.p;
        f->tk = TopkCtx{p, f->d_keyL.p, f->d_keyU.p, f->d_hist.p, reinterpret_cast<TopkState*>(f->d_sel.p),
                        f->d_sel.p + 2, f->cap};
        f->wt.clear();
        f->grpctx.reset();
        f->init_plain = false;
        f->sync();
        *out = f.release();
    });
}

int32_t ihtb_fit_set_weights(ihtb_fit* f, const double* weight) {
    return guard([&] {
        IHTB_CHECK(f, IHTB_EINVAL, "NULL fit handle");
        IHTB_CUDA(cudaSetDevice(f->g->device));
        f->set_weights(weight);
    });
}

int32_t ihtb_fit_set_groups(ihtb_fit* f, const int32_t* group, int32_t J, const int64_t* ks, int64_t n_groups) {
    return guard([&] {
        IHTB_CHECK(f, IHTB_EINVAL, "NULL fit handle");
        IHTB_CUDA(cudaSetDevice(f->g->device));
        f->set_groups(group, J, ks, n_groups);
    });
}

int32_t ihtb_fit_set_k(ihtb_fit* f, int64_t k) {
    return guard([&] {
        IHTB_CHECK(f, IHTB_EINVAL, "NULL fit handle");
        IHTB_CHECK(k >= 0 && k <= f->p, IHTB_EINVAL, "Sparsity level cannot be larger than total number of variables");
        IHTB_CHECK(4 * k + 1024 <= f->cap, IHTB_EINVAL,
                   "k exceeds the candidate capacity this fit handle was created with (create it with the largest k)");
        IHTB_CHECK(!f->grouped() || f->grpctx->ks_vector || k <= f->grpctx->kcap, IHTB_EINVAL,
                   "k exceeds the group candidate capacity (create the fit with the largest k of the path)");
        f->cfg.k = k;
    });
}

int32_t ihtb_fit_init(ihtb_fit* f, const uint8_t* train_mask) {
    return guard([&] {
        IHTB_CHECK(f, IHTB_EINVAL, "NULL fit handle");
        IHTB_CUDA(cudaSetDevice(f->g->device));
        f->init(train_mask);
    });
}

int32_t ihtb_fit_init_beta(ihtb_fit* f, const uint8_t* train_mask) {
    return guard([&] {
        IHTB_CHECK(f, IHTB_EINVAL, "NULL fit handle");
        IHTB_CUDA(cudaSetDevice(f->g->device));
        f->init(train_mask, true);
    });
}

int32_t ihtb_fit_run(ihtb_fit* f, ihtb_result* result, ihtb_iter_trace* trace, int64_t trace_cap) {
    return guard([&] {
        IHTB_CHECK(f, IHTB_EINVAL, "NULL fit handle");
        IHTB_CUDA(cudaSetDevice(f->g->device));
        f->run(result, trace, trace_cap);
    });
}

int32_t ihtb_fit_get(const ihtb_fit* f, double* beta, double* c, double* mu, double* xb) {
    return guard([&] {
        IHTB_CHECK(f, IHTB_EINVAL, "NULL fit handle");
        IHTB_CUDA(cudaSetDevice(f->g->device));
        if (beta) {
            std::fill(beta, beta + f->p_global, 0.0);
            for (size_t t = 0; t < f->best_idx.size(); ++t) beta[f->best_idx[t]] = f->best_b[t];
        }
        if (c) std::copy(f->best_c.begin(), f->best_c.end(), c);
        if (mu) IHTB_CUDA(cudaMemcpy(mu, f->d_mu.p, f->n * sizeof(double), cudaMemcpyDeviceToHost));
        if (xb) IHTB_CUDA(cudaMemcpy(xb, f->d_xb.p, f->n * sizeof(double), cudaMemcpyDeviceToHost));
    });
}

int32_t ihtb_fit_get_sparse(const ihtb_fit* f, int64_t* idx, double* val, int64_t cap, int64_t* nnz) {
    return guard([&] {
        IHTB_CHECK(f && nnz, IHTB_EINVAL, "NULL argument");
        *nnz = (int64_t)f->best_idx.size();
        for (size_t t = 0; t < f->best_idx.size() && (int64_t)t < cap; ++t) {
            if (idx) idx[t] = f->best_idx[t];
            if (val) val[t] = f->best_b[t];
        }
    });
}

int32_t ihtb_fit_predict(ihtb_fit* f, const uint8_t* test_mask, double* deviance) {
    return guard([&] {
        IHTB_CHECK(f && deviance, IHTB_EINVAL, "NULL argument");
        IHTB_CUDA(cudaSetDevice(f->g->device));
        const uint8_t* dm = nullptr;
        if (test_mask) {
            f->upload(f->d_mask.p, test_mask, (size_t)f->n);
            dm = f->d_mask.p;
        }
        glm_set_weights(f->glm, dm, f->s);
        f->update_xb();
        f->glm_update(1);
        *deviance = f->last_dev;
    });
}

int32_t ihtb_fit_timer(ihtb_fit* f, int32_t which, double* ms) {
    return guard([&] {
        IHTB_CHECK(f, IHTB_EINVAL, "NULL fit handle");
        IHTB_CUDA(cudaSetDevice(f->g->device));
        if (!f->tm0) { IHTB_CUDA(cudaEventCreate(&f->tm0)); IHTB_CUDA(cudaEventCreate(&f->tm1)); }
        if (which == 0) {
            IHTB_CUDA(cudaStreamSynchronize(f->s));
            IHTB_CUDA(cudaEventRecord(f->tm0, f->s));
        } else {
            IHTB_CUDA(cudaEventRecord(f->tm1, f->s));
            IHTB_CUDA(cudaEventSynchronize(f->tm1));
            float t = 0.f;
            IHTB_CUDA(cudaEventElapsedTime(&t, f->tm0, f->tm1));
            if (ms) *ms = t;
        }
    });
}

int32_t ihtb_fit_phase_times(const ihtb_fit* f, double* out4) {
    return guard([&] {
        IHTB_CHECK(f && out4, IHTB_EINVAL, "NULL argument");
        for (int i = 0; i < 4; ++i) out4[i] = f->phase[i];
    });
}

void ihtb_internal_fit_debug(const ihtb_fit* f, double* out8) {
    for (int i = 0; i < 6; ++i) out8[i] = f->dbg[i];
    out8[6] = f->sweep_ms_total * 1e-3;
    out8[7] = (double)f->n_sweeps;
}

void ihtb_internal_fit_set_pairer(ihtb_fit* f, void* pairer, int slot) {
    f->pairer = reinterpret_cast<ihtb::SweepPairer*>(pairer);
    f->pair_slot = slot;
}

int32_t ihtb_fit_destroy(ihtb_fit* f) {
    return guard([&] {
        if (!f) return;
        cudaSetDevice(f->device);
        cudaStreamSynchronize(f->s);
        f->g = nullptr;
        f->pairer = nullptr;
        {
            std::lock_guard<std::mutex> lk(g_cache_mu);
            if (g_cache.size() < kCacheMax) { g_cache.push_back(f); return; }
        }
        delete f;
    });
}

}
```

mendeliht.jl_b200/csrc/glm.cu:

```cuda
#include "glm.cuh"

namespace ihtb {

constexpr int GLM_THREADS = 256;

static inline int glm_grid(int64_t n) {
    int64_t b = ceil_div(n, GLM_THREADS);
    return (int)(b < 1 ? 1 : (b > GLM_MAX_BLOCKS ? GLM_MAX_BLOCKS : b));
}

__device__ __forceinline__ void cta_finalize(const double* part, int nv, double* out, unsigned* done,
                                             double* mean_out = nullptr, int64_t n = 1) {
    __shared__ int s_last;
    if (threadIdx.x == 0) {
        __threadfence();
        const unsigned t = atomicAdd(done, 1u);
        s_last = (t == gridDim.x - 1);
    }
    __syncthreads();
    if (!s_last) return;
    __threadfence();
    const int warp = threadIdx.x >> 5, lane = threadIdx.x & 31, nw = blockDim.x >> 5;
    const int nblocks = (int)gridDim.x;
    for (int v = warp; v < nv; v += nw) {
        double a = 0.0;
        for (int b = lane; b < nblocks; b += 32) a += __ldcg(part + (int64_t)b * nv + v);
        a = warp_sum(a);
        if (lane == 0) {
            out[v] = a;
            if (mean_out && v == 0) mean_out[0] = a / (double)n;
        }
    }
    if (threadIdx.x == 0) *done = 0u;
}

__global__ void __launch_bounds__(GLM_THREADS)
k_glm_mu(int64_t n, int64_t q, const double* __restrict__ Z, const double* __restrict__ c, double* __restrict__ xb,
         double* __restrict__ zc, double* __restrict__ mu, const double* __restrict__ y, const double* __restrict__ w,
         int dist, int link, double nb_r, int add_zc, double* __restrict__ part, double* __restrict__ out = nullptr,
         unsigned* __restrict__ done = nullptr) {
    __shared__ double sh[32];
    c += blockIdx.y * q; xb += blockIdx.y * n; zc += blockIdx.y * n; mu += blockIdx.y * n;
    part += (int64_t)blockIdx.y * gridDim.x * 3;
    double a_dev = 0.0, a_lp = 0.0, a_w = 0.0;
    const bool clampit = dist != IHTB_NORMAL;
    for (int64_t i = blockIdx.x * (int64_t)blockDim.x + threadIdx.x; i < n; i += (int64_t)gridDim.x * blockDim.x) {
        double z = 0.0;
        for (int64_t l = 0; l < q; ++l) z += Z[i + l * n] * c[l];
        double x = xb[i];
        if (clampit) {
            x = fmin(fmax(x, -20.0), 20.0);
            z = fmin(fmax(z, -20.0), 20.0);
            xb[i] = x;
        }
        zc[i] = z;
        double m = glm_linkinv(link, add_zc ? x + z : x);
        mu[i] = m;
        double wi = w[i], yi = y[i];
        a_dev += wi * glm_devresid(dist, yi, m, nb_r);
        if (dist != IHTB_NORMAL) a_lp += wi * glm_logpdf_nophi(dist, yi, m, nb_r);
        a_w += wi;
    }
    a_dev = block_sum(a_dev, sh);
    a_lp = block_sum(a_lp, sh);
    a_w = block_sum(a_w, sh);
    if (threadIdx.x == 0) {
        part[blockIdx.x * 3 + 0] = a_dev;
        part[blockIdx.x * 3 + 1] = a_lp;
        part[blockIdx.x * 3 + 2] = a_w;
    }
    if (done) cta_finalize(part, 3, out + blockIdx.y * 3, done + blockIdx.y);
}

__global__ void __launch_bounds__(GLM_THREADS)
k_score(int64_t n, int64_t q, const double* __restrict__ Z, const double* __restrict__ xb,
        const double* __restrict__ zc, const double* __restrict__ mu, const double* __restrict__ y,
        const double* __restrict__ w, int dist, int link, double nb_r, double* __restrict__ r,
        double* __restrict__ part, double* __restrict__ out = nullptr, unsigned* __restrict__ done = nullptr,
        double* __restrict__ mean_out = nullptr) {
    __shared__ double sh[32];
    const int nv = 2 + (int)q;
    double a_r = 0.0, a_abs = 0.0;
    for (int64_t i = blockIdx.x * (int64_t)blockDim.x + threadIdx.x; i < n; i += (int64_t)gridDim.x * blockDim.x) {
        double eta = xb[i] + zc[i];
        double m = mu[i];
        double ri = glm_mueta(link, eta) / glm_var(dist, m, nb_r) * (y[i] - m) * w[i];
        r[i] = ri;
        a_r += ri;
        a_abs += fabs(ri);
    }
    a_r = block_sum(a_r, sh);
    a_abs = block_sum(a_abs, sh);
    if (threadIdx.x == 0) {
        part[blockIdx.x * nv + 0] = a_r;
        part[blockIdx.x * nv + 1] = a_abs;
    }
    for (int64_t l = 0; l < q; ++l) {
        double a = 0.0;
        for (int64_t i = blockIdx.x * (int64_t)blockDim.x + threadIdx.x; i < n; i += (int64_t)gridDim.x * blockDim.x)
            a += Z[i + l * n] * r[i];
        a = block_sum(a, sh);
        if (threadIdx.x == 0) part[blockIdx.x * nv + 2 + l] = a;
    }
    if (done) cta_finalize(part, nv, out, done, mean_out, n);
}

__global__ void __launch_bounds__(GLM_THREADS)
k_stepsize(int64_t n, int64_t q, const double* __restrict__ Z, const double* __restrict__ d2,
           const double* __restrict__ d2mask, const double* __restrict__ xs, const double* __restrict__ xb,
           const double* __restrict__ zc,
           const double* __restrict__ mu, const double* __restrict__ w, int dist, int link, double nb_r,
           double* __restrict__ part, double* __restrict__ out = nullptr, unsigned* __restrict__ done = nullptr) {
    __shared__ double sh[32];
    double a = 0.0;
    for (int64_t i = blockIdx.x * (int64_t)blockDim.x + threadIdx.x; i < n; i += (int64_t)gridDim.x * blockDim.x) {
        double zd = 0.0;
        for (int64_t l = 0; l < q; ++l) zd += Z[i + l * n] * (d2mask ? d2[l] * d2mask[l] : d2[l]);
        double g = glm_mueta(link, xb[i] + zc[i]);
        double sw = sqrt(g * g / glm_var(dist, mu[i], nb_r)) * w[i];
        double v = (xs[i] + zd) * sw;
        a += v * v;
    }
    a = block_sum(a, sh);
    if (threadIdx.x == 0) part[blockIdx.x] = a;
    if (done) cta_finalize(part, 1, out, done);
}

__global__ void __launch_bounds__(GLM_THREADS)
k_sum2(int64_t n, const double* __restrict__ a, const double* __restrict__ b, double* __restrict__ part) {
    __shared__ double sh[32];
    double sa = 0.0, sb = 0.0;
    for (int64_t i = blockIdx.x * (int64_t)blockDim.x + threadIdx.x; i < n; i += (int64_t)gridDim.x * blockDim.x) {
        sa += a[i]; sb += b[i];
    }
    sa = block_sum(sa, sh); sb = block_sum(sb, sh);
    if (threadIdx.x == 0) { part[blockIdx.x * 2] = sa; part[blockIdx.x * 2 + 1] = sb; }
}
__global__ void __launch_bounds__(GLM_THREADS)
k_ssq2(int64_t n, const double* __restrict__ a, double ma, const double* __restrict__ b, double mb,
       double* __restrict__ part) {
    __shared__ double sh[32];
    double sa = 0.0, sb = 0.0;
    for (int64_t i = blockIdx.x * (int64_t)blockDim.x + threadIdx.x; i < n; i += (int64_t)gridDim.x * blockDim.x) {
        double da = a[i] - ma, db = b[i] - mb;
        sa += da * da; sb += db * db;
    }
    sa = block_sum(sa, sh); sb = block_sum(sb, sh);
    if (threadIdx.x == 0) { part[blockIdx.x * 2] = sa; part[blockIdx.x * 2 + 1] = sb; }
}

__global__ void __launch_bounds__(GLM_THREADS)
k_set_weights(int64_t n, const uint8_t* __restrict__ mask, const double* __restrict__ y, double* __restrict__ w,
              double* __restrict__ part) {
    __shared__ double sh[32];
    double sw = 0.0, sy = 0.0;
    for (int64_t i = blockIdx.x * (int64_t)blockDim.x + threadIdx.x; i < n; i += (int64_t)gridDim.x * blockDim.x) {
        double wi = (mask == nullptr || mask[i]) ? 1.0 : 0.0;
        w[i] = wi;
        sw += wi;
        sy += y[i] * wi;
    }
    sw = block_sum(sw, sh); sy = block_sum(sy, sh);
    if (threadIdx.x == 0) { part[blockIdx.x * 2] = sw; part[blockIdx.x * 2 + 1] = sy; }
}

__global__ void k_finalize(const double* __restrict__ part, int nblocks, int nv, double* __restrict__ out,
                           double* __restrict__ mean_out = nullptr, int64_t n = 1) {
    part += (int64_t)blockIdx.y * nblocks * nv; out += blockIdx.y * nv;
    int v = (blockIdx.x * blockDim.x + threadIdx.x) >> 5;
    int lane = threadIdx.x & 31;
    if (v >= nv) return;
    double a = 0.0;
    for (int b = lane; b < nblocks; b += 32) a += part[b * nv + v];
    a = warp_sum(a);
    if (lane == 0) {
        out[v] = a;
        if (mean_out && v == 0 && blockIdx.y == 0) mean_out[0] = a / (double)n;
    }
}

__global__ void k_mean_from_sum(const double* __restrict__ scal, int64_t n, double* __restrict__ out) {
    out[0] = scal[0] / (double)n;
}

__global__ void k_wy(int64_t n, const double* __restrict__ w, const double* __restrict__ y, double* __restrict__ out) {
    int64_t i = blockIdx.x * (int64_t)blockDim.x + threadIdx.x;
    if (i < n) out[i] = w[i] * y[i];
}
__device__ __forceinline__ void init_beta_regress(double N, double SY, double sx, double sxx, double sxy, double& beta,
                                                  double& icpt) {
    double slope = sxy;
    icpt = SY;
    const double u11 = sqrt(N), u12 = sx / u11, dd = sxx - u12 * u12;
    if (N > 0.0 && dd > 0.0) {
        const double u22 = sqrt(dd), t1 = SY / u11, t2 = (sxy - u12 * t1) / u22;
        slope = t2 / u22;
        icpt = (t1 - u12 * slope) / u11;
    }
    beta = fmin(fmax(slope, -2.0), 2.0);
}
__global__ void __launch_bounds__(GLM_THREADS)
k_init_beta(int64_t p, const double* __restrict__ W1, const double* __restrict__ W2, const double* __restrict__ Wm,
            const double* __restrict__ Y1, const double* __restrict__ Y2, const double* __restrict__ Ym, double N,
            double SY, const double* __restrict__ mu, const double* __restrict__ sinv, int impute,
            double* __restrict__ beta, double* __restrict__ part) {
    __shared__ double sh[32];
    double acc = 0.0;
    for (int64_t j = blockIdx.x * (int64_t)blockDim.x + threadIdx.x; j < p; j += (int64_t)gridDim.x * blockDim.x) {
        const double m = mu[j], si = sinv[j];
        const double a0 = (0.0 - m) * si, a1 = (1.0 - m) * si, a2 = (2.0 - m) * si, am = impute ? 0.0 : a0;
        const double w1 = W1[j], w2 = W2[j], wm = Wm[j], w0 = N - w1 - w2 - wm;
        const double y1 = Y1[j], y2 = Y2[j], ym = Ym[j], y0 = SY - y1 - y2 - ym;
        const double sx = a0 * w0 + a1 * w1 + a2 * w2 + am * wm;
        const double sxx = a0 * a0 * w0 + a1 * a1 * w1 + a2 * a2 * w2 + am * am * wm;
        const double sxy = a0 * y0 + a1 * y1 + a2 * y2 + am * ym;
        double icpt;
        init_beta_regress(N, SY, sx, sxx, sxy, beta[j], icpt);
        acc += icpt;
    }
    acc = block_sum(acc, sh);
    if (threadIdx.x == 0) part[blockIdx.x] = acc;
}
__global__ void __launch_bounds__(GLM_THREADS)
k_init_beta_moments(int64_t p, const double* __restrict__ SX, const double* __restrict__ SXX,
                    const double* __restrict__ SXY, double N, double SY, double* __restrict__ beta,
                    double* __restrict__ part) {
    __shared__ double sh[32];
    double acc = 0.0;
    for (int64_t j = blockIdx.x * (int64_t)blockDim.x + threadIdx.x; j < p; j += (int64_t)gridDim.x * blockDim.x) {
        double icpt;
        init_beta_regress(N, SY, SX[j], SXX[j], SXY[j], beta[j], icpt);
        acc += icpt;
    }
    acc = block_sum(acc, sh);
    if (threadIdx.x == 0) part[blockIdx.x] = acc;
}
__global__ void __launch_bounds__(GLM_THREADS)
k_cov_sums(int64_t n, int64_t q, const double* __restrict__ Z, const double* __restrict__ y,
           const double* __restrict__ w, double* __restrict__ part) {
    __shared__ double sh[32];
    const int nv = 3 * ((int)q - 1);
    for (int64_t l = 1; l < q; ++l) {
        double a = 0.0, b = 0.0, c = 0.0;
        for (int64_t i = blockIdx.x * (int64_t)blockDim.x + threadIdx.x; i < n; i += (int64_t)gridDim.x * blockDim.x) {
            double z = Z[i + l * n], wi = w[i];
            a += wi * z; b += wi * z * z; c += wi * z * y[i];
        }
        a = block_sum(a, sh); b = block_sum(b, sh); c = block_sum(c, sh);
        if (threadIdx.x == 0) {
            part[blockIdx.x * nv + 3 * (l - 1)] = a;
            part[blockIdx.x * nv + 3 * (l - 1) + 1] = b;
            part[blockIdx.x * nv + 3 * (l - 1) + 2] = c;
        }
    }
}

void init_beta_products(GlmCtx& c, double* d_wy, cudaStream_t s) {
    IHTB_LAUNCH(k_wy, (unsigned)ceil_div(c.n, 256), 256, 0, s, c.n, c.w, c.y, d_wy);
}
void init_beta_solve(GlmCtx& c, int64_t p, const double* W1, const double* W2, const double* Wm, const double* Y1,
                     const double* Y2, const double* Ym, double N, double SY, const double* mu, const double* sinv,
                     int impute, double* d_beta, cudaStream_t s) {
    int grid = glm_grid(p);
    IHTB_LAUNCH(k_init_beta, grid, GLM_THREADS, 0, s, p, W1, W2, Wm, Y1, Y2, Ym, N, SY, mu, sinv, impute, d_beta, c.part);
    IHTB_LAUNCH(k_finalize, 1, 32, 0, s, c.part, grid, 1, c.scal);
}
void init_beta_solve_moments(GlmCtx& c, int64_t p, const double* SX, const double* SXX, const double* SXY, double N,
                             double SY, double* d_beta, cudaStream_t s) {
    int grid = glm_grid(p);
    IHTB_LAUNCH(k_init_beta_moments, grid, GLM_THREADS, 0, s, p, SX, SXX, SXY, N, SY, d_beta, c.part);
    IHTB_LAUNCH(k_finalize, 1, 32, 0, s, c.part, grid, 1, c.scal);
}
void init_beta_cov_sums(GlmCtx& c, cudaStream_t s) {
    int grid = glm_grid(c.n);
    int nv = 3 * ((int)c.q - 1);
    IHTB_LAUNCH(k_cov_sums, grid, GLM_THREADS, 0, s, c.n, c.q, c.Z, c.y, c.w, c.part);
    IHTB_LAUNCH(k_finalize, (unsigned)ceil_div(nv, 4), 128, 0, s, c.part, grid, nv, c.scal);
}
void glm_mean_from_sum(GlmCtx& c, double* d_mean, cudaStream_t s) {
    IHTB_LAUNCH(k_mean_from_sum, 1, 1, 0, s, c.scal, c.n, d_mean);
}
void glm_mu(GlmCtx& c, const double* d_c, int add_zc, cudaStream_t s) {
    int grid = glm_grid(c.n);
    IHTB_LAUNCH(k_glm_mu, grid, GLM_THREADS, 0, s, c.n, c.q, c.Z, d_c, c.xb, c.zc, c.mu, c.y, c.w, c.dist, c.link,
                c.nb_r, add_zc, c.part, c.scal, c.done);
    if (!c.done) IHTB_LAUNCH(k_finalize, 1, 96, 0, s, c.part, grid, 3, c.scal);
}
void glm_mu_batched(GlmCtx& c, const double* d_cM, int M, double* xbM, double* zcM, double* muM, double* d_partM,
                    double* d_scalM, cudaStream_t s) {
    int grid = glm_grid(c.n);
    IHTB_LAUNCH(k_glm_mu, dim3(grid, M), GLM_THREADS, 0, s, c.n, c.q, c.Z, d_cM, xbM, zcM, muM, c.y, c.w, c.dist, c.link,
                c.nb_r, 1, d_partM, d_scalM, c.done);
    if (!c.done) IHTB_LAUNCH(k_finalize, dim3(1, M), 96, 0, s, d_partM, grid, 3, d_scalM);
}
__global__ void k_pick_model(const double* __restrict__ scalM, int M, double old_logl, int max_step, int dist, int64_t n,
                             double* __restrict__ pick) {
    if (threadIdx.x != 0 || blockIdx.x != 0) return;
    for (int m = 0; m < M; ++m) {
        const double dev = scalM[3 * m], lp = scalM[3 * m + 1], sw = scalM[3 * m + 2];
        double l = lp;
        if (dist == IHTB_NORMAL) {
            const double phi = dev / (double)n, sigma = sqrt(phi);
            l = -0.5 * (dev / phi) - sw * (0.5 * log(2.0 * 3.14159265358979323846) + log(sigma));
        }
        pick[1 + m] = l;
    }
    int w = 0;
    while (old_logl > pick[1 + w] && w < max_step) ++w;
    pick[0] = (double)w;
}
__global__ void k_take_model(const double* __restrict__ pick, int64_t n, const double* __restrict__ xbM,
                             const double* __restrict__ zcM, const double* __restrict__ muM, double* __restrict__ xb,
                             double* __restrict__ zc, double* __restrict__ mu) {
    const int64_t off = (int64_t)pick[0] * n;
    for (int64_t i = blockIdx.x * (int64_t)blockDim.x + threadIdx.x; i < n; i += (int64_t)gridDim.x * blockDim.x) {
        xb[i] = xbM[off + i]; zc[i] = zcM[off + i]; mu[i] = muM[off + i];
    }
}
__global__ void k_winner_coef(const double* __restrict__ pick, const double* __restrict__ coefM, int64_t U,
                              const double* __restrict__ df_uni, double* __restrict__ coef_out,
                              const double* __restrict__ cM, int64_t q, double* __restrict__ mask_out) {
    const int64_t w = (int64_t)pick[0];
    const int64_t t = blockIdx.x * (int64_t)blockDim.x + threadIdx.x;
    if (t < U) coef_out[t] = coefM[t + w * U] != 0.0 ? df_uni[t] : 0.0;
    if (t < q) mask_out[t] = cM[t + w * q] != 0.0 ? 1.0 : 0.0;
}
void glm_pick_model(GlmCtx& c, const double* d_scalM, int M, double old_logl, int max_step, double* d_pick,
                    const double* xbM, const double* zcM, const double* muM, cudaStream_t s) {
    IHTB_LAUNCH(k_pick_model, 1, 32, 0, s, d_scalM, M, old_logl, max_step, c.dist, c.n, d_pick);
    IHTB_LAUNCH(k_take_model, glm_grid(c.n), GLM_THREADS, 0, s, d_pick, c.n, xbM, zcM, muM, c.xb, c.zc, c.mu);
}
void glm_winner_coef(const double* d_pick, const double* d_coefM, int64_t U, const double* d_df_uni, double* d_coef_out,
                     const double* d_cM, int64_t q, double* d_mask_out, cudaStream_t s) {
    const int64_t m = U > q ? U : q;
    IHTB_LAUNCH(k_winner_coef, (unsigned)ceil_div(m > 0 ? m : 1, 128), 128, 0, s, d_pick, d_coefM, U, d_df_uni, d_coef_out,
                d_cM, q, d_mask_out);
}

void glm_score(GlmCtx& c, cudaStream_t s, double* d_mean) {
    int grid = glm_grid(c.n);
    int nv = 2 + (int)c.q;
    IHTB_LAUNCH(k_score, grid, GLM_THREADS, 0, s, c.n, c.q, c.Z, c.xb, c.zc, c.mu, c.y, c.w, c.dist, c.link, c.nb_r,
                c.r, c.part, c.scal, c.done, d_mean);
    if (!c.done) IHTB_LAUNCH(k_finalize, (unsigned)ceil_div(nv, 4), 128, 0, s, c.part, grid, nv, c.scal, d_mean, c.n);
}
void glm_stepsize(GlmCtx& c, const double* d_d2, const double* d_xs, cudaStream_t s, const double* d_d2mask,
                  double* d_out) {
    int grid = glm_grid(c.n);
    IHTB_LAUNCH(k_stepsize, grid, GLM_THREADS, 0, s, c.n, c.q, c.Z, d_d2, d_d2mask, d_xs, c.xb, c.zc, c.mu, c.w, c.dist,
                c.link, c.nb_r, c.part, d_out ? d_out : c.scal, c.done);
    if (!c.done) IHTB_LAUNCH(k_finalize, 1, 32, 0, s, c.part, grid, 1, d_out ? d_out : c.scal);
}
void glm_sum2(GlmCtx& c, const double* a, const double* b, cudaStream_t s) {
    int grid = glm_grid(c.n);
    IHTB_LAUNCH(k_sum2, grid, GLM_THREADS, 0, s, c.n, a, b, c.part);
    IHTB_LAUNCH(k_finalize, 1, 64, 0, s, c.part, grid, 2, c.scal);
}
void glm_ssq2(GlmCtx& c, const double* a, double ma, const double* b, double mb, cudaStream_t s) {
    int grid = glm_grid(c.n);
    IHTB_LAUNCH(k_ssq2, grid, GLM_THREADS, 0, s, c.n, a, ma, b, mb, c.part);
    IHTB_LAUNCH(k_finalize, 1, 64, 0, s, c.part, grid, 2, c.scal);
}
void glm_set_weights(GlmCtx& c, const uint8_t* d_mask, cudaStream_t s) {
    int grid = glm_grid(c.n);
    IHTB_LAUNCH(k_set_weights, grid, GLM_THREADS, 0, s, c.n, d_mask, c.y, c.w, c.part);
    IHTB_LAUNCH(k_finalize, 1, 64, 0, s, c.part, grid, 2, c.scal);
}

}
```

mendeliht.jl_b200/csrc/support.cu:

```cuda
#include "common.cuh"
#include "comm.cuh"
#include <algorithm>
#include <memory>
#include <mutex>
#include <unordered_map>

namespace ihtb {

constexpr int XS_CHUNK = 32;

template <int M, bool PUSH>
__global__ void __launch_bounds__(256)
k_x_support(GenoView gv, const int64_t* __restrict__ idx, int64_t k, const double* __restrict__ coef,
            double* __restrict__ out, P2PView pv, unsigned long long seq) {
    const int64_t nbytes = gv.nbytes, n = gv.n;
    const double* __restrict__ mu = gv.mu;
    const double* __restrict__ sinv = gv.sinv;
    const int impute = gv.impute;
    __shared__ double tab[XS_CHUNK][4][M];
    __shared__ int64_t cols[XS_CHUNK];
    int64_t b = blockIdx.x * (int64_t)blockDim.x + threadIdx.x;
    double acc[4][M];
#pragma unroll
    for (int s = 0; s < 4; ++s)
#pragma unroll
        for (int t = 0; t < M; ++t) acc[s][t] = 0.0;

    for (int64_t c0 = 0; c0 < k; c0 += XS_CHUNK) {
        int nc = (int)((k - c0 < XS_CHUNK) ? (k - c0) : XS_CHUNK);
        __syncthreads();
        for (int e = threadIdx.x; e < nc * 4 * M; e += blockDim.x) {
            int c = e / (4 * M), code = (e / M) & 3, t = e % M;
            int64_t j = idx[c0 + c];
            double m = mu[j];
            double g = (code == 2) ? 1.0 : (code == 3) ? 2.0 : (code == 1) ? (impute ? m : 0.0) : 0.0;
            double x = __dmul_rn(__dsub_rn(g, m), sinv[j]);
            tab[c][code][t] = __dmul_rn(x, coef[(c0 + c) + (int64_t)t * k]);
            if (code == 0 && t == 0) cols[c] = j;
        }
        __syncthreads();
        if (b < nbytes) {
            for (int c = 0; c < nc; ++c) {
                uint32_t byte = *gv_ptr(gv, cols[c], b);
#pragma unroll
                for (int s = 0; s < 4; ++s) {
                    uint32_t code = (byte >> (2 * s)) & 3u;
#pragma unroll
                    for (int t = 0; t < M; ++t) acc[s][t] = __dadd_rn(acc[s][t], tab[c][code][t]);
                }
            }
        }
    }
    if (PUSH) {
        __shared__ double stage[PUSH ? 1024 : 1];
        __syncthreads();
#pragma unroll
        for (int s = 0; s < 4; ++s) stage[4 * threadIdx.x + s] = acc[s][0];
        __syncthreads();
        const int64_t base = 1024 * (int64_t)blockIdx.x;
        for (int e = 2 * threadIdx.x; e < 1024; e += 512) {
            const int64_t i = base + e;
            if (i + 1 < n) {
                const double2 x = make_double2(stage[e], stage[e + 1]);
                for (int r = 0; r < pv.nranks; ++r) *reinterpret_cast<double2*>(pv.push_slot[r] + i) = x;
            } else if (i < n) {
                for (int r = 0; r < pv.nranks; ++r) pv.push_slot[r][i] = stage[e];
            }
        }
        p2p_publish(pv, seq);
        return;
    }
    if (b < nbytes) {
#pragma unroll
        for (int s = 0; s < 4; ++s) {
            int64_t i = 4 * b + s;
            if (i < n)
#pragma unroll
                for (int t = 0; t < M; ++t) out[i + (int64_t)t * n] = acc[s][t];
        }
    }
}

template <int M>
static void launch_x_support(const ihtb_geno* g, const int64_t* d_idx, int64_t k, const double* d_coef, double* d_out,
                             cudaStream_t s) {
    IHTB_LAUNCH((k_x_support<M, false>), (unsigned)ceil_div(g->nbytes, 256), 256, 0, s, geno_view(g), d_idx, k, d_coef,
                d_out, P2PView{}, 0ull);
}

void x_support_push(const ihtb_geno* g, const int64_t* d_idx, int64_t k, const double* d_coef, ihtb_comm* c,
                    cudaStream_t s) {
    IHTB_LAUNCH((k_x_support<1, true>), (unsigned)ceil_div(g->nbytes, 256), 256, 0, s, geno_view(g), d_idx, k, d_coef,
                (double*)nullptr, p2p_view(c), (unsigned long long)(c->seq[0] + 1));
}

void x_support(const ihtb_geno* g, const int64_t* d_idx, int64_t k, const double* d_coef, int64_t m, double* d_out,
               cudaStream_t s) {
    if (geno_is_dense(g)) { dense_x_support(g, d_idx, k, d_coef, m, d_out, s); return; }
    for (int64_t t0 = 0; t0 < m;) {
        int64_t mm = m - t0;
        const double* cf = d_coef + t0 * k;
        double* o = d_out + t0 * g->n;
        if (mm >= 4) { launch_x_support<4>(g, d_idx, k, cf, o, s); t0 += 4; }
        else if (mm == 3) { launch_x_support<3>(g, d_idx, k, cf, o, s); t0 += 3; }
        else if (mm == 2) { launch_x_support<2>(g, d_idx, k, cf, o, s); t0 += 2; }
        else { launch_x_support<1>(g, d_idx, k, cf, o, s); t0 += 1; }
    }
}

constexpr int XG_MAX_SPLIT = 64;


template <int M>
__global__ void __launch_bounds__(256)
k_xt_gather(GenoView gv, const int64_t* __restrict__ cols, int64_t n_a, const int64_t* __restrict__ cols_b,
            int64_t split_bytes, const double* __restrict__ v,
            const double* __restrict__ vbar, double* __restrict__ part ) {
    __shared__ double sh[32];
    const int64_t nbytes = gv.nbytes, n = gv.n;
    const int64_t c = blockIdx.x, sp = blockIdx.y;
    const int64_t j = c < n_a ? cols[c] : cols_b[c - n_a];
    if (j < 0) return;
    const int64_t b0 = sp * split_bytes;
    const int64_t b1 = (b0 + split_bytes < nbytes) ? b0 + split_bytes : nbytes;
    double a[M], mm[M], vb[M];
#pragma unroll
    for (int t = 0; t < M; ++t) { a[t] = 0.0; mm[t] = 0.0; vb[t] = vbar[t]; }
    for (int64_t b = b0 + threadIdx.x; b < b1; b += blockDim.x) {
        uint32_t byte = *gv_ptr(gv, j, b);
        if (byte == 0) continue;
#pragma unroll
        for (int s = 0; s < 4; ++s) {
            uint32_t code = (byte >> (2 * s)) & 3u;
            int64_t i = 4 * b + s;
            if (code != 0 && i < n) {
#pragma unroll
                for (int t = 0; t < M; ++t) {
                    double u = __dsub_rn(v[i + (int64_t)t * n], vb[t]);
                    if (code == 1) mm[t] = __dadd_rn(mm[t], u);
                    else a[t] = __dadd_rn(a[t], (code == 3) ? __dadd_rn(u, u) : u);
                }
            }
        }
    }
    double* o = part + (c * gridDim.y + sp) * (2 * M);
#pragma unroll
    for (int t = 0; t < M; ++t) {
        double at = block_sum(a[t], sh);
        double mt = block_sum(mm[t], sh);
        if (threadIdx.x == 0) { o[2 * t] = at; o[2 * t + 1] = mt; }
    }
}

template <int M>
__global__ void k_xt_gather_fin(GenoView gv, const int64_t* __restrict__ cols, int64_t n_a,
                                const int64_t* __restrict__ cols_b, int64_t ncols, int nsplit,
                                const double* __restrict__ vbar, const double* __restrict__ part,
                                double* __restrict__ out) {
    int64_t e = blockIdx.x * (int64_t)blockDim.x + threadIdx.x;
    if (e >= ncols * M) return;
    int64_t c = e / M;
    int t = (int)(e % M);
    const int64_t jc = c < n_a ? cols[c] : cols_b[c - n_a];
    if (jc < 0) { out[c + (int64_t)t * ncols] = 0.0; return; }
    double at = 0.0, mt = 0.0;
    for (int sp = 0; sp < nsplit; ++sp) {
        const double* o = part + (c * nsplit + sp) * (2 * M);
        at = __dadd_rn(at, o[2 * t]);
        mt = __dadd_rn(mt, o[2 * t + 1]);
    }
    int64_t j = jc;
    double corr = gv.impute ? mt : __dmul_rn(-vbar[t], (double)gv.nmiss[j]);
    out[c + (int64_t)t * ncols] = __dmul_rn(gv.sinv[j], __dadd_rn(at, __dmul_rn(gv.mu[j], corr)));
}

constexpr int XN_CHUNK = 512;
__global__ void __launch_bounds__(256)
k_xt_gather_nib(GenoView gv, const int64_t* __restrict__ cols, int64_t n_a, const int64_t* __restrict__ cols_b,
                int64_t ncols, const double* __restrict__ v, const double* __restrict__ vbar,
                double* __restrict__ part ) {
    __shared__ double T[8][16][32];
    const int64_t n = gv.n;
    const int64_t chunk = blockIdx.x, nchunks = gridDim.x;
    const int warp = threadIdx.x >> 5, lane = threadIdx.x & 31;
    {
        const double vb = vbar[0];
        const int64_t i0 = chunk * XN_CHUNK + 16 * lane + 2 * warp;
        const double u0 = (i0 < n) ? __dsub_rn(v[i0], vb) : 0.0;
        const double u1 = (i0 + 1 < n) ? __dsub_rn(v[i0 + 1], vb) : 0.0;
        const double d0[4] = {0.0, 0.0, u0, __dadd_rn(u0, u0)};
        const double d1[4] = {0.0, 0.0, u1, __dadd_rn(u1, u1)};
#pragma unroll
        for (int nib = 0; nib < 16; ++nib) T[warp][nib][lane] = __dadd_rn(d0[nib & 3], d1[nib >> 2]);
    }
    __syncthreads();
    const int64_t w = chunk * (XN_CHUNK / 16) + lane;
    const bool in_col = w < ((gv.nbytes + 3) >> 2);
    for (int64_t c = (int64_t)blockIdx.y * 8 + warp; c < ncols; c += (int64_t)gridDim.y * 8) {
        const int64_t j = c < n_a ? cols[c] : cols_b[c - n_a];
        if (j < 0) continue;
        const uint32_t x = in_col ? *reinterpret_cast<const uint32_t*>(gv_ptr(gv, j, 4 * w)) : 0u;
        double a = 0.0;
#pragma unroll
        for (int k = 0; k < 8; ++k) a = __dadd_rn(a, T[k][(x >> (4 * k)) & 15u][lane]);
        a = warp_sum(a);
        if (lane == 0) part[c * nchunks + chunk] = a;
    }
}

__global__ void __launch_bounds__(128)
k_xt_gather_fin_nib(GenoView gv, const int64_t* __restrict__ miss_ptr, const int32_t* __restrict__ miss_idx,
                    const int64_t* __restrict__ cols, int64_t n_a, const int64_t* __restrict__ cols_b, int64_t ncols,
                    int nchunks, const double* __restrict__ v, const double* __restrict__ vbar,
                    const double* __restrict__ part, double* __restrict__ out) {
    const int64_t c = (blockIdx.x * (int64_t)blockDim.x + threadIdx.x) >> 5;
    const int lane = threadIdx.x & 31;
    if (c >= ncols) return;
    const int64_t jc = c < n_a ? cols[c] : cols_b[c - n_a];
    if (jc < 0) { if (lane == 0) out[c] = 0.0; return; }
    double at = 0.0, mt = 0.0;
    for (int sp = lane; sp < nchunks; sp += 32) at = __dadd_rn(at, part[c * nchunks + sp]);
    const double vb = vbar[0];
    if (gv.impute)
        for (int64_t e = miss_ptr[jc] + lane; e < miss_ptr[jc + 1]; e += 32) mt = __dadd_rn(mt, __dsub_rn(v[miss_idx[e]], vb));
    at = warp_sum(at); mt = warp_sum(mt);
    if (lane == 0) {
        const double corr = gv.impute ? mt : __dmul_rn(-vb, (double)gv.nmiss[jc]);
        out[c] = __dmul_rn(gv.sinv[jc], __dadd_rn(at, __dmul_rn(gv.mu[jc], corr)));
    }
}

static DBuf<double>& gather_scratch(cudaStream_t s) {
    static std::mutex mu;
    static std::unordered_map<cudaStream_t, std::unique_ptr<DBuf<double>>> pool;
    std::lock_guard<std::mutex> lk(mu);
    auto& slot = pool[s];
    if (!slot) slot.reset(new DBuf<double>());
    return *slot;
}

template <int M>
static void launch_xt_gather(const ihtb_geno* g, const int64_t* d_cols, int64_t n_a, const int64_t* d_cols_b,
                             int64_t ncols, const double* d_v, const double* d_vbar, double* d_out, cudaStream_t s,
                             bool blocked) {
    DBuf<double>& sc = gather_scratch(s);
    (void)blocked;
    if (M == 1) {
        const int nchunks = (int)ceil_div(g->n, XN_CHUNK);
        const size_t need_b = (size_t)ncols * nchunks;
        if (sc.n < need_b) {
            IHTB_CUDA(cudaStreamSynchronize(s));
            sc.alloc(need_b < 65536 ? 65536 : need_b);
        }
        int groups = (int)std::max<int64_t>(1, std::min<int64_t>(ceil_div(ncols, 8), (8 * g->sm_count) / nchunks + 1));
        IHTB_LAUNCH(k_xt_gather_nib, dim3((unsigned)nchunks, (unsigned)groups), 256, 0, s, geno_view(g), d_cols, n_a,
                    d_cols_b, ncols, d_v, d_vbar, sc.p);
        IHTB_LAUNCH(k_xt_gather_fin_nib, (unsigned)ceil_div(ncols * 32, 128), 128, 0, s, geno_view(g), g->miss_ptr.p,
                    g->miss_idx.p, d_cols, n_a, d_cols_b, ncols, nchunks, d_v, d_vbar, sc.p, d_out);
        return;
    }
    int64_t split_bytes = ceil_div(ceil_div(g->nbytes, XG_MAX_SPLIT), 256) * 256;
    if (split_bytes < 1024) split_bytes = 1024;
    int nsplit = (int)ceil_div(g->nbytes, split_bytes);
    size_t need = (size_t)ncols * nsplit * 2 * M;
    if (sc.n < need) {
        IHTB_CUDA(cudaStreamSynchronize(s));
        sc.alloc(need < 65536 ? 65536 : need);
    }
    dim3 grid((unsigned)ncols, (unsigned)nsplit);
    IHTB_LAUNCH((k_xt_gather<M>), grid, 256, 0, s, geno_view(g), d_cols, n_a, d_cols_b, split_bytes, d_v, d_vbar, sc.p);
    IHTB_LAUNCH((k_xt_gather_fin<M>), (unsigned)ceil_div(ncols * M, 128), 128, 0, s, geno_view(g), d_cols, n_a, d_cols_b,
                ncols, nsplit, d_vbar, sc.p, d_out);
}

void xt_gather2(const ihtb_geno* g, const int64_t* d_cols_a, int64_t n_a, const int64_t* d_cols_b, int64_t n_b,
                const double* d_v, int64_t m, const double* d_vbar, double* d_out, cudaStream_t s, bool blocked) {
    const int64_t ncols = n_a + n_b;
    if (ncols == 0) return;
    if (geno_is_dense(g)) { dense_xt_gather2(g, d_cols_a, n_a, d_cols_b, n_b, d_v, m, d_out, s); return; }
    for (int64_t t0 = 0; t0 < m;) {
        int64_t mm = m - t0;
        const double* vv = d_v + t0 * g->n;
        const double* vb = d_vbar + t0;
        double* o = d_out + t0 * ncols;
        if (mm >= 4) { launch_xt_gather<4>(g, d_cols_a, n_a, d_cols_b, ncols, vv, vb, o, s, blocked); t0 += 4; }
        else if (mm == 3) { launch_xt_gather<3>(g, d_cols_a, n_a, d_cols_b, ncols, vv, vb, o, s, blocked); t0 += 3; }
        else if (mm == 2) { launch_xt_gather<2>(g, d_cols_a, n_a, d_cols_b, ncols, vv, vb, o, s, blocked); t0 += 2; }
        else { launch_xt_gather<1>(g, d_cols_a, n_a, d_cols_b, ncols, vv, vb, o, s, blocked); t0 += 1; }
    }
}

void xt_gather(const ihtb_geno* g, const int64_t* d_cols, int64_t ncols, const double* d_v, int64_t m,
               const double* d_vbar, double* d_out, cudaStream_t s) {
    xt_gather2(g, d_cols, ncols, nullptr, 0, d_v, m, d_vbar, d_out, s, false);
}

}

using namespace ihtb;

__global__ void k_gb_fill(double* v, int64_t n) {
    int64_t i = blockIdx.x * (int64_t)blockDim.x + threadIdx.x;
    if (i < n) {
        uint64_t h = (uint64_t)i * 0x9E3779B97F4A7C15ull + 12345ull;
        h ^= h >> 31; h *= 0xBF58476D1CE4E5B9ull; h ^= h >> 29;
        v[i] = (double)(h >> 11) * (1.0 / 9007199254740992.0) - 0.4;
        v[i + n] = v[i];
    }
}
extern "C" int32_t ihtb_gather_bench(const ihtb_geno* g, int64_t ncols, int32_t reps, double* ms_per_call,
                                     double* max_rel_diff) {
    return guard([&] {
        IHTB_CHECK(g && ncols >= 1 && reps >= 1, IHTB_EINVAL, "bad argument");
        IHTB_CHECK(!geno_is_dense(g), IHTB_EUNSUPPORTED, "the gather bench times the PLINK re-scoring kernels");
        geno_require_ready(g);
        IHTB_CUDA(cudaSetDevice(g->device));
        cudaStream_t s;
        IHTB_CUDA(cudaStreamCreateWithFlags(&s, cudaStreamNonBlocking));
        std::vector<int64_t> hc((size_t)ncols);
        for (int64_t t = 0; t < ncols; ++t) hc[(size_t)t] = (t * 7919) % g->p;
        DBuf<int64_t> d_cols((size_t)ncols);
        DBuf<double> d_v((size_t)(2 * g->n)), d_mean(2), d_a((size_t)ncols), d_b((size_t)(2 * ncols));
        IHTB_CUDA(cudaMemcpyAsync(d_cols.p, hc.data(), (size_t)ncols * sizeof(int64_t), cudaMemcpyHostToDevice, s));
        IHTB_LAUNCH(k_gb_fill, (unsigned)ceil_div(g->n, 256), 256, 0, s, d_v.p, g->n);
        const double mean[2] = {0.1, 0.1};
        IHTB_CUDA(cudaMemcpyAsync(d_mean.p, mean, sizeof(mean), cudaMemcpyHostToDevice, s));
        xt_gather2(g, d_cols.p, ncols, nullptr, 0, d_v.p, 1, d_mean.p, d_a.p, s);
        cudaEvent_t e0, e1;
        IHTB_CUDA(cudaEventCreate(&e0)); IHTB_CUDA(cudaEventCreate(&e1));
        IHTB_CUDA(cudaEventRecord(e0, s));
        for (int i = 0; i < reps; ++i) xt_gather2(g, d_cols.p, ncols, nullptr, 0, d_v.p, 1, d_mean.p, d_a.p, s);
        IHTB_CUDA(cudaEventRecord(e1, s));
        xt_gather2(g, d_cols.p, ncols, nullptr, 0, d_v.p, 2, d_mean.p, d_b.p, s);
        std::vector<double> ha((size_t)ncols), hb((size_t)(2 * ncols));
        IHTB_CUDA(cudaMemcpyAsync(ha.data(), d_a.p, ha.size() * sizeof(double), cudaMemcpyDeviceToHost, s));
        IHTB_CUDA(cudaMemcpyAsync(hb.data(), d_b.p, hb.size() * sizeof(double), cudaMemcpyDeviceToHost, s));
        IHTB_CUDA(cudaStreamSynchronize(s));
        float ms = 0.f;
        IHTB_CUDA(cudaEventElapsedTime(&ms, e0, e1));
        if (ms_per_call) *ms_per_call = ms / reps;
        double worst = 0.0, scale = 0.0;
        for (int64_t t = 0; t < ncols; ++t) scale = std::max(scale, std::fabs(hb[(size_t)t]));
        for (int64_t t = 0; t < ncols; ++t) worst = std::max(worst, std::fabs(ha[(size_t)t] - hb[(size_t)t]));
        if (max_rel_diff) *max_rel_diff = scale > 0 ? worst / scale : worst;
        cudaEventDestroy(e0); cudaEventDestroy(e1);
        cudaStreamDestroy(s);
    });
}

extern "C" int32_t ihtb_x_support(const ihtb_geno* g, const int64_t* idx, int64_t k, const double* coef, int64_t m,
                                  double* out) {
    return guard([&] {
        IHTB_CHECK(g && out && m >= 1 && k >= 0, IHTB_EINVAL, "bad argument");
        geno_require_ready(g);
        IHTB_CHECK(k == 0 || (idx && coef), IHTB_EINVAL, "NULL idx/coef");
        IHTB_CUDA(cudaSetDevice(g->device));
        for (int64_t c = 0; c < k; ++c)
            IHTB_CHECK(idx[c] >= 0 && idx[c] < g->p, IHTB_EDIM, "support index out of range");
        DBuf<double> d_out((size_t)(g->n * m));
        if (k == 0) {
            d_out.zero(0);
        } else {
            DBuf<int64_t> d_idx((size_t)k);
            DBuf<double> d_coef((size_t)(k * m));
            IHTB_CUDA(cudaMemcpy(d_idx.p, idx, k * sizeof(int64_t), cudaMemcpyHostToDevice));
            IHTB_CUDA(cudaMemcpy(d_coef.p, coef, k * m * sizeof(double), cudaMemcpyHostToDevice));
            x_support(g, d_idx.p, k, d_coef.p, m, d_out.p, 0);
        }
        IHTB_CUDA(cudaMemcpy(out, d_out.p, g->n * m * sizeof(double), cudaMemcpyDeviceToHost));
    });
}
```

mendeliht.jl_b200/csrc/sweep.cu:

```cuda
#include "common.cuh"
#include "pairer.cuh"
#include "topk.cuh"
#include <stdlib.h>

namespace ihtb {

void sweep_fast_partials(const ihtb_geno* g, const double* d_v, const double* d_vbar, float* d_part, int64_t* n_slabs,
                         cudaStream_t s);
int64_t sweep_fast_num_slabs(const ihtb_geno* g);
void sweep_exact_lut_partials(const ihtb_geno* g, const double* d_v, const double* d_vbar, double* d_part, cudaStream_t s,
                              int cls = 0);
void sweep_pair_partials(const ihtb_geno* g, const double* d_v0, const double* d_v1, const double* d_vbar,
                         const float* d_scale, float* d_part, cudaStream_t s);

static bool exact_uses_lut(const ihtb_geno* g) {
    static const bool legacy = [] { const char* e = getenv("IHTB_EXACT_LEGACY"); return e && *e == '1'; }();
    return g->cs_j == 128 && !legacy;
}

constexpr int EX_THREADS = 128;
constexpr int EX_CB = 8;
constexpr int EX_COLS_PER_CTA = 512;

__global__ void __launch_bounds__(EX_THREADS)
k_sweep_exact(GenoView gv, const double* __restrict__ v, const double* __restrict__ vbar_p, double* __restrict__ part ) {
    const double vbar = *vbar_p;
    __shared__ double red[EX_THREADS / 32][EX_CB];
    const int64_t p = gv.p, n = gv.n;
    const int64_t words = gv.stride >> 2;
    const int64_t slab = blockIdx.y;
    const int64_t w = slab * EX_THREADS + threadIdx.x;
    const bool live = w < words;
    double u[16];
#pragma unroll
    for (int s = 0; s < 16; ++s) {
        int64_t i = 16 * w + s;
        u[s] = (live && i < n) ? __dsub_rn(v[i], vbar) : 0.0;
    }
    const int64_t jbeg = blockIdx.x * (int64_t)EX_COLS_PER_CTA;
    const int64_t jend = (jbeg + EX_COLS_PER_CTA < p) ? jbeg + EX_COLS_PER_CTA : p;
    const int lane = threadIdx.x & 31, warp = threadIdx.x >> 5;
    for (int64_t j0 = jbeg; j0 < jend; j0 += EX_CB) {
        uint32_t wd[EX_CB];
#pragma unroll
        for (int c = 0; c < EX_CB; ++c) {
            int64_t j = j0 + c;
            wd[c] = (live && j < jend) ? *reinterpret_cast<const uint32_t*>(gv_ptr(gv, j, 4 * w)) : 0u;
        }
        double acc[EX_CB];
#pragma unroll
        for (int c = 0; c < EX_CB; ++c) {
            double a = 0.0;
            uint32_t x = wd[c];
#pragma unroll
            for (int s = 0; s < 16; ++s) {
                uint32_t code = (x >> (2 * s)) & 3u;
                double dos = (code == 2) ? 1.0 : ((code == 3) ? 2.0 : 0.0);
                a = fma(u[s], dos, a);
            }
            acc[c] = warp_sum(a);
        }
        __syncthreads();
        if (lane == 0) {
#pragma unroll
            for (int c = 0; c < EX_CB; ++c) red[warp][c] = acc[c];
        }
        __syncthreads();
        if (threadIdx.x < EX_CB && j0 + threadIdx.x < jend) {
            double t = 0.0;
#pragma unroll
            for (int q = 0; q < EX_THREADS / 32; ++q) t += red[q][threadIdx.x];
            part[slab * p + j0 + threadIdx.x] = t;
        }
    }
}

template <typename T>
__global__ void __launch_bounds__(256)
k_sweep_epilogue(const T* __restrict__ part, int64_t n_slabs, int64_t p,
                 const double* __restrict__ mu, const double* __restrict__ sinv,
                 const int32_t* __restrict__ nmiss, const int64_t* __restrict__ miss_ptr,
                 const int32_t* __restrict__ miss_idx, const double* __restrict__ v,
                 const double* __restrict__ vbar_p,
                 int impute, double* __restrict__ out, const float* __restrict__ scale_p = nullptr,
                 TopkFuse tf = TopkFuse()) {
    __shared__ int sh[TOPK_BINS];
    const bool fuse = tf.keyL != nullptr;
    if (fuse) {
        topk_first_kernel_housekeeping(tf.hist_other, tf.st, tf.cand, tf.cand_fill);
        for (int b = threadIdx.x; b < TOPK_BINS; b += blockDim.x) sh[b] = 0;
        __syncthreads();
    }
    int64_t j = blockIdx.x * (int64_t)blockDim.x + threadIdx.x;
    if (j < p) {
        const double vbar = *vbar_p;
        double a = 0.0;
        for (int64_t s = 0; s < n_slabs; ++s) a += (double)part[s * p + j];
        if (scale_p) a /= (double)*scale_p;
        double corr = 0.0;
        int nm = nmiss[j];
        if (nm) {
            if (impute) {
                for (int64_t e = miss_ptr[j]; e < miss_ptr[j + 1]; ++e) corr += v[miss_idx[e]] - vbar;
            } else {
                corr = -vbar * (double)nm;
            }
        }
        const double df = sinv[j] * (a + mu[j] * corr);
        out[j] = df;
        if (fuse) {
            const double bound = tf.bound_coef * (tf.scal[1] + fabs(tf.scal[0]));
            const double w = tf.wt ? tf.wt[j] : 1.0;
            uint32_t kl, ku;
            topk_make_keys(0.0 + 1.0 * df, w, fabs(1.0) * tf.scale[j] * bound * w, kl, ku);
            tf.keyL[j] = kl; tf.keyU[j] = ku;
            atomicAdd(&sh[kl >> 21], 1);
        }
    }
    if (fuse) {
        __syncthreads();
        for (int b = threadIdx.x; b < TOPK_BINS; b += blockDim.x)
            if (sh[b]) atomicAdd(&tf.hist[b], sh[b]);
    }
}

__global__ void k_vec_mean(const double* __restrict__ v, int64_t n, double* __restrict__ out) {
    __shared__ double sh[32];
    double a = 0.0;
    for (int64_t i = threadIdx.x; i < n; i += blockDim.x) a += v[i];
    a = block_sum(a, sh);
    if (threadIdx.x == 0) out[0] = a / (double)n;
}

__global__ void k_pair_scale(const double* __restrict__ v0, const double* __restrict__ v1, int64_t n,
                             const double* __restrict__ vbar, float* __restrict__ scale) {
    __shared__ double sh[32];
    for (int t = 0; t < 2; ++t) {
        const double* v = t ? v1 : v0;
        const double vb = vbar[t];
        double m = 0.0;
        for (int64_t i = threadIdx.x; i < n; i += blockDim.x) m = fmax(m, fabs(v[i] - vb));
#pragma unroll
        for (int o = 16; o > 0; o >>= 1) m = fmax(m, __shfl_xor_sync(0xffffffffu, m, o));
        __syncthreads();
        if ((threadIdx.x & 31) == 0) sh[threadIdx.x >> 5] = m;
        __syncthreads();
        if (threadIdx.x == 0) {
            for (int w = 1; w < (int)(blockDim.x >> 5); ++w) m = fmax(m, sh[w]);
            int e = 0;
            if (m > 0.0 && isfinite(m)) frexp(m, &e);
            scale[t] = ldexpf(1.0f, 9 - e);
        }
    }
}

__global__ void k_l2norm(const double* __restrict__ v, int64_t n, const double* __restrict__ vbar, double* __restrict__ out) {
    __shared__ double sh[32];
    const double vb = vbar[0];
    double a = 0.0;
    for (int64_t i = threadIdx.x; i < n; i += blockDim.x) { const double u = v[i] - vb; a += u * u; }
    a = block_sum(a, sh);
    if (threadIdx.x == 0) out[0] = sqrt(a);
}

struct SweepScratch {
    DBuf<double> part64;
    DBuf<float> part32;
    DBuf<float> scale;
};

void sweep_xt_v_with_means(const ihtb_geno* g, const double* dV, const double* d_vbar, int64_t m, double* dOut,
                           int mode, cudaStream_t s, void* scratch_any, float* sweep_ms, double* d_l2 = nullptr,
                           const TopkFuse* tf = nullptr) {
    IHTB_CHECK(!tf || (m == 1 && mode != IHTB_SWEEP_PAIR), IHTB_EINVAL, "fused selection stage: one right-hand side");
    const TopkFuse fuse = tf ? *tf : TopkFuse();
    SweepScratch local;
    SweepScratch* sc = scratch_any ? reinterpret_cast<SweepScratch*>(scratch_any) : &local;
    cudaEvent_t e0 = nullptr, e1 = nullptr;
    if (sweep_ms) {
        IHTB_CUDA(cudaEventCreate(&e0)); IHTB_CUDA(cudaEventCreate(&e1));
        IHTB_CUDA(cudaEventRecord(e0, s));
    }
    if (geno_is_dense(g)) {
        dense_xt_v(g, dV, m, dOut, s, &sc->part64, tf);
    } else {
        if (d_l2)
            for (int64_t t = 0; t < m; ++t) IHTB_LAUNCH(k_l2norm, 1, 1024, 0, s, dV + t * g->n, g->n, d_vbar + t, d_l2 + t);
        for (int64_t t = 0; t < m; ++t) {
            const double* v = dV + t * g->n;
            double* out = dOut + t * g->p;
            if (mode == IHTB_SWEEP_PAIR && g->cs_j == 128 && t + 1 < m) {
                const int64_t n_slabs = sweep_fast_num_slabs(g);
                if (sc->part32.n < (size_t)(2 * n_slabs * g->p)) sc->part32.alloc((size_t)(2 * n_slabs * g->p));
                if (sc->scale.n < 2) sc->scale.alloc(2);
                IHTB_LAUNCH(k_pair_scale, 1, 1024, 0, s, v, v + g->n, g->n, d_vbar + t, sc->scale.p);
                sweep_pair_partials(g, v, v + g->n, d_vbar + t, sc->scale.p, sc->part32.p, s);
                for (int h = 0; h < 2; ++h)
                    IHTB_LAUNCH((k_sweep_epilogue<float>), (unsigned)ceil_div(g->p, 256), 256, 0, s,
                                sc->part32.p + (size_t)h * n_slabs * g->p, n_slabs, g->p, g->mu.p, g->sinv.p, g->nmiss.p,
                                g->miss_ptr.p, g->miss_idx.p, v + h * g->n, d_vbar + t + h, g->impute, out + h * g->p,
                                sc->scale.p + h);
                ++t;
                continue;
            }
            if (mode == IHTB_SWEEP_EXACT && exact_uses_lut(g)) {
                const int64_t n_slabs = g->stride / 128;
                if (sc->part64.n < (size_t)(n_slabs * g->p)) sc->part64.alloc((size_t)(n_slabs * g->p));
                sweep_exact_lut_partials(g, v, d_vbar + t, sc->part64.p, s);
                IHTB_LAUNCH((k_sweep_epilogue<double>), (unsigned)ceil_div(g->p, 256), 256, 0, s, sc->part64.p, n_slabs,
                            g->p, g->mu.p, g->sinv.p, g->nmiss.p, g->miss_ptr.p, g->miss_idx.p, v, d_vbar + t,
                            g->impute, out, (const float*)nullptr, fuse);
            } else if (mode == IHTB_SWEEP_EXACT) {
                int64_t words = g->stride >> 2;
                int64_t n_slabs = ceil_div(words, EX_THREADS);
                if (sc->part64.n < (size_t)(n_slabs * g->p)) sc->part64.alloc((size_t)(n_slabs * g->p));
                dim3 grid((unsigned)ceil_div(g->p, EX_COLS_PER_CTA), (unsigned)n_slabs);
                IHTB_LAUNCH(k_sweep_exact, grid, EX_THREADS, 0, s, geno_view(g), v, d_vbar + t, sc->part64.p);
                IHTB_LAUNCH((k_sweep_epilogue<double>), (unsigned)ceil_div(g->p, 256), 256, 0, s, sc->part64.p, n_slabs,
                            g->p, g->mu.p, g->sinv.p, g->nmiss.p, g->miss_ptr.p, g->miss_idx.p, v, d_vbar + t,
                            g->impute, out, (const float*)nullptr, fuse);
            } else {
                int64_t n_slabs = sweep_fast_num_slabs(g);
                if (sc->part32.n < (size_t)(n_slabs * g->p)) sc->part32.alloc((size_t)(n_slabs * g->p));
                sweep_fast_partials(g, v, d_vbar + t, sc->part32.p, &n_slabs, s);
                IHTB_LAUNCH((k_sweep_epilogue<float>), (unsigned)ceil_div(g->p, 256), 256, 0, s, sc->part32.p, n_slabs,
                            g->p, g->mu.p, g->sinv.p, g->nmiss.p, g->miss_ptr.p, g->miss_idx.p, v, d_vbar + t,
                            g->impute, out, (const float*)nullptr, fuse);
            }
        }
    }
    if (sweep_ms) {
        IHTB_CUDA(cudaEventRecord(e1, s));
        IHTB_CUDA(cudaEventSynchronize(e1));
        IHTB_CUDA(cudaEventElapsedTime(sweep_ms, e0, e1));
        cudaEventDestroy(e0); cudaEventDestroy(e1);
    }
}

__global__ void k_copy2(const double* __restrict__ a, const double* __restrict__ b, double* __restrict__ out) {
    out[0] = a[0]; out[1] = b[0];
}

SweepPairer::SweepPairer(int dev) : device(dev) {
    IHTB_CUDA(cudaSetDevice(dev));
    for (int i = 0; i < 2; ++i) IHTB_CUDA(cudaEventCreateWithFlags(&ready[i], cudaEventDisableTiming));
    IHTB_CUDA(cudaEventCreateWithFlags(&done, cudaEventDisableTiming));
    IHTB_CUDA(cudaMalloc((void**)&d_vbar2, 2 * sizeof(double)));
    IHTB_CUDA(cudaMalloc((void**)&d_l2, 2 * sizeof(double)));
    scratch = new SweepScratch();
}
SweepPairer::~SweepPairer() {
    cudaSetDevice(device);
    cudaDeviceSynchronize();
    for (int i = 0; i < 2; ++i) if (ready[i]) cudaEventDestroy(ready[i]);
    if (done) cudaEventDestroy(done);
    if (d_vbar2) cudaFree(d_vbar2);
    if (d_l2) cudaFree(d_l2);
    delete reinterpret_cast<SweepScratch*>(scratch);
}

void SweepPairer::leave() {
    std::lock_guard<std::mutex> lk(mu);
    --active;
    cv.notify_all();
}

bool SweepPairer::sweep(int slot, const ihtb_geno* g, const double* d_v, const double* d_vbar, double* d_out,
                        cudaStream_t s, void* solo_scratch) {
    const int other = slot ^ 1;
    IHTB_CUDA(cudaEventRecord(ready[slot], s));
    std::unique_lock<std::mutex> lk(mu);
    if (active >= 2 && !geno_is_dense(g) && g->cs_j == 128) {
        req[slot] = Req{d_v, d_vbar, d_out, s};
        has[slot] = true;
        if (has[other]) {
            const Req a = req[0], b = req[1];
            SweepScratch* sc = reinterpret_cast<SweepScratch*>(scratch);
            const int64_t n_slabs = sweep_fast_num_slabs(g);
            if (sc->part32.n < (size_t)(2 * n_slabs * g->p)) sc->part32.alloc((size_t)(2 * n_slabs * g->p));
            if (sc->scale.n < 2) sc->scale.alloc(2);
            IHTB_CUDA(cudaStreamWaitEvent(s, ready[other], 0));
            IHTB_LAUNCH(k_copy2, 1, 1, 0, s, a.vbar, b.vbar, d_vbar2);
            IHTB_LAUNCH(k_pair_scale, 1, 1024, 0, s, a.v, b.v, g->n, d_vbar2, sc->scale.p);
            IHTB_LAUNCH(k_l2norm, 1, 1024, 0, s, a.v, g->n, d_vbar2, d_l2);
            IHTB_LAUNCH(k_l2norm, 1, 1024, 0, s, b.v, g->n, d_vbar2 + 1, d_l2 + 1);
            sweep_pair_partials(g, a.v, b.v, d_vbar2, sc->scale.p, sc->part32.p, s);
            const Req* rq[2] = {&a, &b};
            for (int h = 0; h < 2; ++h)
                IHTB_LAUNCH((k_sweep_epilogue<float>), (unsigned)ceil_div(g->p, 256), 256, 0, s,
                            sc->part32.p + (size_t)h * n_slabs * g->p, n_slabs, g->p, g->mu.p, g->sinv.p, g->nmiss.p,
                            g->miss_ptr.p, g->miss_idx.p, rq[h]->v, d_vbar2 + h, g->impute, rq[h]->out, sc->scale.p + h);
            IHTB_CUDA(cudaEventRecord(done, s));
            has[0] = has[1] = false;
            ++round;
            ++n_pair;
            cv.notify_all();
            return true;
        }
        const unsigned long long r0 = round;
        cv.wait(lk, [&] { return round != r0 || active < 2; });
        if (round != r0) {
            IHTB_CUDA(cudaStreamWaitEvent(s, done, 0));
            return true;
        }
        has[slot] = false;
    }
    ++n_solo;
    lk.unlock();
    sweep_xt_v_with_means(g, d_v, d_vbar, 1, d_out, IHTB_SWEEP_FAST, s, solo_scratch, nullptr, nullptr);
    return false;
}

void* sweep_scratch_create() { return new SweepScratch(); }
void sweep_scratch_destroy(void* p) { delete reinterpret_cast<SweepScratch*>(p); }

}

using namespace ihtb;

extern "C" int32_t ihtb_xt_v(const ihtb_geno* g, const double* V, int64_t m, double* out, int32_t sweep_mode) {
    return guard([&] {
        IHTB_CHECK(g && V && out && m >= 1, IHTB_EINVAL, "bad argument");
        geno_require_ready(g);
        IHTB_CHECK(sweep_mode == IHTB_SWEEP_FAST || sweep_mode == IHTB_SWEEP_EXACT || sweep_mode == IHTB_SWEEP_PAIR,
                   IHTB_EINVAL, "bad sweep_mode");
        IHTB_CUDA(cudaSetDevice(g->device));
        DBuf<double> dV((size_t)(g->n * m)), dOut((size_t)(g->p * m)), dmean((size_t)m);
        IHTB_CUDA(cudaMemcpy(dV.p, V, g->n * m * sizeof(double), cudaMemcpyHostToDevice));
        for (int64_t t = 0; t < m; ++t)
            IHTB_LAUNCH(k_vec_mean, 1, 1024, 0, 0, dV.p + t * g->n, g->n, dmean.p + t);
        sweep_xt_v_with_means(g, dV.p, dmean.p, m, dOut.p, sweep_mode, 0, nullptr, nullptr, nullptr);
        IHTB_CUDA(cudaMemcpy(out, dOut.p, g->p * m * sizeof(double), cudaMemcpyDeviceToHost));
    });
}

namespace ihtb {
void sweep_fast_kernel_only(const ihtb_geno* g, const double* d_v, const double* d_vbar, float* d_part, cudaStream_t s);
__global__ void k_fill_vec(double* v, int64_t n, uint64_t seed) {
    int64_t i = blockIdx.x * (int64_t)blockDim.x + threadIdx.x;
    if (i >= n) return;
    uint64_t x = seed + (uint64_t)i * 0x9E3779B97F4A7C15ull;
    x ^= x >> 30; x *= 0xBF58476D1CE4E5B9ull; x ^= x >> 27; x *= 0x94D049BB133111EBull; x ^= x >> 31;
    v[i] = ((double)(x >> 11) * (1.0 / 9007199254740992.0) - 0.5) * 2.0;
}
}

extern "C" int32_t ihtb_sweep_bench(const ihtb_geno* g, int32_t sweep_mode, int32_t warmup, int32_t reps,
                                    double* ms_kernel, double* ms_total) {
    return guard([&] {
        IHTB_CHECK(g && reps >= 1 && warmup >= 0, IHTB_EINVAL, "bad argument");
        geno_require_ready(g);
        IHTB_CUDA(cudaSetDevice(g->device));
        cudaStream_t s;
        IHTB_CUDA(cudaStreamCreateWithFlags(&s, cudaStreamNonBlocking));
        const int64_t mrhs = sweep_mode == IHTB_SWEEP_PAIR ? 2 : 1;
        DBuf<double> dV((size_t)(g->n * mrhs)), dOut((size_t)(g->p * mrhs));
        IHTB_LAUNCH(k_fill_vec, (unsigned)ceil_div(g->n * mrhs, 256), 256, 0, s, dV.p, g->n * mrhs, 12345ull);
        DBuf<double> dmean((size_t)mrhs);
        for (int64_t t = 0; t < mrhs; ++t) IHTB_LAUNCH(k_vec_mean, 1, 1024, 0, s, dV.p + t * g->n, g->n, dmean.p + t);
        SweepScratch sc;
        cudaEvent_t e0, e1;
        IHTB_CUDA(cudaEventCreate(&e0)); IHTB_CUDA(cudaEventCreate(&e1));
        for (int i = 0; i < warmup; ++i)
            sweep_xt_v_with_means(g, dV.p, dmean.p, mrhs, dOut.p, sweep_mode, s, &sc, nullptr, nullptr);
        IHTB_CUDA(cudaEventRecord(e0, s));
        for (int i = 0; i < reps; ++i)
            sweep_xt_v_with_means(g, dV.p, dmean.p, mrhs, dOut.p, sweep_mode, s, &sc, nullptr, nullptr);
        IHTB_CUDA(cudaEventRecord(e1, s));
        IHTB_CUDA(cudaEventSynchronize(e1));
        float ms = 0.f;
        IHTB_CUDA(cudaEventElapsedTime(&ms, e0, e1));
        if (ms_total) *ms_total = ms / reps;
        if (ms_kernel) {
            *ms_kernel = 0.0;
            if (geno_is_dense(g)) {
                IHTB_CUDA(cudaEventRecord(e0, s));
                for (int i = 0; i < reps; ++i) dense_sweep_kernel_only(g, dV.p, &sc.part64, s);
                IHTB_CUDA(cudaEventRecord(e1, s));
                IHTB_CUDA(cudaEventSynchronize(e1));
                IHTB_CUDA(cudaEventElapsedTime(&ms, e0, e1));
                *ms_kernel = ms / reps;
            } else if (sweep_mode == IHTB_SWEEP_PAIR) {
                IHTB_CHECK(g->cs_j == 128, IHTB_EUNSUPPORTED, "the pair sweep needs a tiled layout");
                IHTB_CUDA(cudaEventRecord(e0, s));
                for (int i = 0; i < reps; ++i)
                    sweep_pair_partials(g, dV.p, dV.p + g->n, dmean.p, sc.scale.p, sc.part32.p, s);
                IHTB_CUDA(cudaEventRecord(e1, s));
                IHTB_CUDA(cudaEventSynchronize(e1));
                IHTB_CUDA(cudaEventElapsedTime(&ms, e0, e1));
                *ms_kernel = ms / reps;
            } else if (sweep_mode == IHTB_SWEEP_FAST) {
                IHTB_CUDA(cudaEventRecord(e0, s));
                for (int i = 0; i < reps; ++i) sweep_fast_kernel_only(g, dV.p, dmean.p, sc.part32.p, s);
                IHTB_CUDA(cudaEventRecord(e1, s));
                IHTB_CUDA(cudaEventSynchronize(e1));
                IHTB_CUDA(cudaEventElapsedTime(&ms, e0, e1));
                *ms_kernel = ms / reps;
            } else if (exact_uses_lut(g)) {
                IHTB_CUDA(cudaEventRecord(e0, s));
                for (int i = 0; i < reps; ++i) sweep_exact_lut_partials(g, dV.p, dmean.p, sc.part64.p, s);
                IHTB_CUDA(cudaEventRecord(e1, s));
                IHTB_CUDA(cudaEventSynchronize(e1));
                IHTB_CUDA(cudaEventElapsedTime(&ms, e0, e1));
                *ms_kernel = ms / reps;
            } else {
                int64_t words = g->stride >> 2;
                int64_t n_slabs = ceil_div(words, EX_THREADS);
                dim3 grid((unsigned)ceil_div(g->p, EX_COLS_PER_CTA), (unsigned)n_slabs);
                IHTB_CUDA(cudaEventRecord(e0, s));
                for (int i = 0; i < reps; ++i)
                    IHTB_LAUNCH(k_sweep_exact, grid, EX_THREADS, 0, s, geno_view(g), dV.p, dmean.p, sc.part64.p);
                IHTB_CUDA(cudaEventRecord(e1, s));
                IHTB_CUDA(cudaEventSynchronize(e1));
                IHTB_CUDA(cudaEventElapsedTime(&ms, e0, e1));
                *ms_kernel = ms / reps;
            }
        }
        cudaEventDestroy(e0); cudaEventDestroy(e1);
        cudaStreamDestroy(s);
    });
}

namespace ihtb {

__global__ void __launch_bounds__(EX_THREADS)
k_sweep_class_exact(GenoView gv, const double* __restrict__ v, double* __restrict__ part1, double* __restrict__ part2) {
    __shared__ double red[EX_THREADS / 32][2 * EX_CB];
    const int64_t p = gv.p, n = gv.n;
    const int64_t words = gv.stride >> 2;
    const int64_t slab = blockIdx.y;
    const int64_t w = slab * EX_THREADS + threadIdx.x;
    const bool live = w < words;
    double u[16];
#pragma unroll
    for (int s = 0; s < 16; ++s) {
        int64_t i = 16 * w + s;
        u[s] = (live && i < n) ? v[i] : 0.0;
    }
    const int64_t jbeg = blockIdx.x * (int64_t)EX_COLS_PER_CTA;
    const int64_t jend = (jbeg + EX_COLS_PER_CTA < p) ? jbeg + EX_COLS_PER_CTA : p;
    const int lane = threadIdx.x & 31, warp = threadIdx.x >> 5;
    for (int64_t j0 = jbeg; j0 < jend; j0 += EX_CB) {
        double a1[EX_CB], a2[EX_CB];
#pragma unroll
        for (int c = 0; c < EX_CB; ++c) {
            int64_t j = j0 + c;
            uint32_t x = (live && j < jend) ? *reinterpret_cast<const uint32_t*>(gv_ptr(gv, j, 4 * w)) : 0u;
            double s1 = 0.0, s2 = 0.0;
#pragma unroll
            for (int s = 0; s < 16; ++s) {
                uint32_t code = (x >> (2 * s)) & 3u;
                s1 += (code == 2) ? u[s] : 0.0;
                s2 += (code == 3) ? u[s] : 0.0;
            }
            a1[c] = warp_sum(s1);
            a2[c] = warp_sum(s2);
        }
        __syncthreads();
        if (lane == 0) {
#pragma unroll
            for (int c = 0; c < EX_CB; ++c) { red[warp][c] = a1[c]; red[warp][EX_CB + c] = a2[c]; }
        }
        __syncthreads();
        if (threadIdx.x < 2 * EX_CB) {
            int c = threadIdx.x % EX_CB;
            if (j0 + c < jend) {
                double t = 0.0;
#pragma unroll
                for (int q = 0; q < EX_THREADS / 32; ++q) t += red[q][threadIdx.x];
                (threadIdx.x < EX_CB ? part1 : part2)[slab * p + j0 + c] = t;
            }
        }
    }
}

__global__ void k_class_epilogue(const double* __restrict__ part1, const double* __restrict__ part2, int64_t n_slabs,
                                 int64_t p, const int64_t* __restrict__ miss_ptr, const int32_t* __restrict__ miss_idx,
                                 const double* __restrict__ v, double* __restrict__ out1, double* __restrict__ out2,
                                 double* __restrict__ outm) {
    int64_t j = blockIdx.x * (int64_t)blockDim.x + threadIdx.x;
    if (j >= p) return;
    double a = 0.0, b = 0.0, m = 0.0;
    for (int64_t s = 0; s < n_slabs; ++s) { a += part1[s * p + j]; b += part2[s * p + j]; }
    for (int64_t e = miss_ptr[j]; e < miss_ptr[j + 1]; ++e) m += v[miss_idx[e]];
    out1[j] = a; out2[j] = b; outm[j] = m;
}

void sweep_class_sums(const ihtb_geno* g, const double* d_v, double* d_w1, double* d_w2, double* d_wm, cudaStream_t s,
                      void* scratch_any) {
    SweepScratch* sc = reinterpret_cast<SweepScratch*>(scratch_any);
    if (exact_uses_lut(g)) {
        const int64_t ns = g->stride / 128;
        if (sc->part64.n < (size_t)(2 * ns * g->p)) sc->part64.alloc((size_t)(2 * ns * g->p));
        double* q1 = sc->part64.p;
        double* q2 = sc->part64.p + ns * g->p;
        sweep_exact_lut_partials(g, d_v, nullptr, q1, s, 1);
        sweep_exact_lut_partials(g, d_v, nullptr, q2, s, 2);
        IHTB_LAUNCH(k_class_epilogue, (unsigned)ceil_div(g->p, 256), 256, 0, s, q1, q2, ns, g->p, g->miss_ptr.p,
                    g->miss_idx.p, d_v, d_w1, d_w2, d_wm);
        return;
    }
    int64_t words = g->stride >> 2;
    int64_t n_slabs = ceil_div(words, EX_THREADS);
    if (sc->part64.n < (size_t)(2 * n_slabs * g->p)) sc->part64.alloc((size_t)(2 * n_slabs * g->p));
    double* p1 = sc->part64.p;
    double* p2 = sc->part64.p + n_slabs * g->p;
    dim3 grid((unsigned)ceil_div(g->p, EX_COLS_PER_CTA), (unsigned)n_slabs);
    IHTB_LAUNCH(k_sweep_class_exact, grid, EX_THREADS, 0, s, geno_view(g), d_v, p1, p2);
    IHTB_LAUNCH(k_class_epilogue, (unsigned)ceil_div(g->p, 256), 256, 0, s, p1, p2, n_slabs, g->p, g->miss_ptr.p,
                g->miss_idx.p, d_v, d_w1, d_w2, d_wm);
}

}
```

mendeliht.jl_b200/csrc/topk.cu:

```cuda
#include "topk.cuh"
#include "comm.cuh"

namespace ihtb {

constexpr int TK_THREADS = 256;
constexpr int TK_BINS = 2048;

static inline int tk_grid(int64_t p) {
    int64_t b = ceil_div(p, TK_THREADS * 4);
    return (int)(b < 1 ? 1 : (b > 592 ? 592 : b));
}

__device__ __forceinline__ void hist_flush(const int* sh, int* g, int nb) {
    for (int b = threadIdx.x; b < nb; b += blockDim.x)
        if (sh[b]) atomicAdd(&g[b], sh[b]);
}

__global__ void __launch_bounds__(TK_THREADS)
k_keys_hist0(int64_t p, const double* __restrict__ dfa, const double* __restrict__ b0d,
             const double* __restrict__ sinv, int64_t p_mod, const double* __restrict__ bounds, double eta,
             double bound, const double* __restrict__ scal, double bound_coef, const double* __restrict__ wt,
             uint32_t* __restrict__ keyL, uint32_t* __restrict__ keyU, int* __restrict__ hist,
             const double* __restrict__ l2, int* __restrict__ hist_other, TopkState* __restrict__ st,
             int64_t* __restrict__ cand, int cand_fill) {
    topk_first_kernel_housekeeping(hist_other, st, cand, cand_fill);
    if (l2) bound = bound_coef * l2[0];
    else if (scal) bound = bound_coef * (scal[1] + fabs(scal[0]));
    __shared__ int sh[TK_BINS];
    for (int b = threadIdx.x; b < TK_BINS; b += blockDim.x) sh[b] = 0;
    __syncthreads();
    for (int64_t j = blockIdx.x * (int64_t)blockDim.x + threadIdx.x; j < p; j += (int64_t)gridDim.x * blockDim.x) {
        double v = (b0d ? b0d[j] : 0.0) + eta * dfa[j];
        const double w = wt ? wt[j] : 1.0;
        const double bj = bounds ? bounds[j / p_mod] : bound;
        uint32_t kl, ku;
        topk_make_keys(v, w, fabs(eta) * sinv[bounds ? (j % p_mod) : j] * bj * w, kl, ku);
        keyL[j] = kl; keyU[j] = ku;
        atomicAdd(&sh[kl >> 21], 1);
    }
    __syncthreads();
    hist_flush(sh, hist, TK_BINS);
}

constexpr int TK_HIST_STRIDE = 3 * TK_BINS;

__device__ __forceinline__ void block_pick(const int* __restrict__ hist, int nb, int k, int* sh_scan ,
                                           int* sh_out ) {
    constexpr int PER = TK_BINS / TK_THREADS;
    const int t = threadIdx.x;
    int c[PER];
    int s = 0;
#pragma unroll
    for (int i = 0; i < PER; ++i) {
        const int r = t * PER + i;
        c[i] = (r < nb) ? hist[nb - 1 - r] : 0;
        s += c[i];
    }
    int incl = s;
#pragma unroll
    for (int o = 1; o < 32; o <<= 1) {
        int v = __shfl_up_sync(0xffffffffu, incl, o);
        if ((t & 31) >= o) incl += v;
    }
    if ((t & 31) == 31) sh_scan[t >> 5] = incl;
    __syncthreads();
    if (t < 32) {
        int v = (t < TK_THREADS / 32) ? sh_scan[t] : 0;
        int sc = v;
#pragma unroll
        for (int o = 1; o < 32; o <<= 1) {
            int u = __shfl_up_sync(0xffffffffu, sc, o);
            if (t >= o) sc += u;
        }
        if (t < TK_THREADS / 32) sh_scan[t] = sc - v;
    }
    __syncthreads();
    incl += sh_scan[t >> 5];
    int excl = incl - s;
    if (excl < k && k <= incl) {
#pragma unroll
        for (int i = 0; i < PER; ++i) {
            if (excl < k && k <= excl + c[i]) { sh_out[0] = nb - 1 - (t * PER + i); sh_out[1] = k - excl; }
            excl += c[i];
        }
    }
    __syncthreads();
}

__global__ void __launch_bounds__(TK_THREADS)
k_hist_fused(int64_t p, const uint32_t* __restrict__ keyL, const int* __restrict__ hists , int pass, int kk,
             int* __restrict__ hist_out) {
    __shared__ int sh[TK_BINS];
    __shared__ int sh_scan[32];
    __shared__ int sh_out[2];
    block_pick(hists, TK_BINS, kk, sh_scan, sh_out);
    uint32_t prefix = (uint32_t)sh_out[0] << 21;
    int shift = 10, bits = 11;
    uint32_t himask = 0xFFE00000u;
    if (pass == 2) {
        const int k1 = sh_out[1];
        __syncthreads();
        block_pick(hists + TK_BINS, TK_BINS, k1, sh_scan, sh_out);
        prefix |= (uint32_t)sh_out[0] << 10;
        shift = 0; bits = 10; himask = 0xFFFFFC00u;
    }
    const int nb = 1 << bits;
    for (int b = threadIdx.x; b < nb; b += blockDim.x) sh[b] = 0;
    __syncthreads();
    for (int64_t j = blockIdx.x * (int64_t)blockDim.x + threadIdx.x; j < p; j += (int64_t)gridDim.x * blockDim.x) {
        const uint32_t k = keyL[j];
        if ((k & himask) == prefix) atomicAdd(&sh[(k >> shift) & (nb - 1)], 1);
    }
    __syncthreads();
    hist_flush(sh, hist_out, nb);
}

__global__ void __launch_bounds__(TK_THREADS)
k_compact_fused(int64_t p, const uint32_t* __restrict__ keyU, const int* __restrict__ hists, int kk,
                TopkState* __restrict__ st, int64_t* __restrict__ cand, int cap) {
    __shared__ int sh_scan[32];
    __shared__ int sh_out[2];
    block_pick(hists, TK_BINS, kk, sh_scan, sh_out);
    uint32_t tau = (uint32_t)sh_out[0] << 21;
    int k1 = sh_out[1];
    __syncthreads();
    block_pick(hists + TK_BINS, TK_BINS, k1, sh_scan, sh_out);
    tau |= (uint32_t)sh_out[0] << 10;
    if (blockIdx.x == 0 && threadIdx.x == 0) { st->prefix = tau; st->k_rem = sh_out[1]; }
    for (int64_t j = blockIdx.x * (int64_t)blockDim.x + threadIdx.x; j < p; j += (int64_t)gridDim.x * blockDim.x) {
        if (keyU[j] >= tau) {
            int pos = atomicAdd(&st->count, 1);
            if (pos < cap) cand[pos] = j;
        }
    }
}

__global__ void k_scatter(double* __restrict__ dst, const int64_t* __restrict__ idx, const double* __restrict__ val,
                          int64_t k, int zero_only) {
    int64_t t = blockIdx.x * (int64_t)blockDim.x + threadIdx.x;
    if (t < k) dst[idx[t]] = zero_only ? 0.0 : val[t];
}

static void topk_run(TopkCtx& c, const double* d_dfa, const double* d_b0d, const double* d_sinv, int64_t p_mod,
                     const double* d_bounds, double eta, double bound, int64_t k, cudaStream_t s,
                     const double* d_scal = nullptr, double bound_coef = 0.0, const double* d_l2 = nullptr,
                     bool fill_cand = false) {
    int grid = tk_grid(c.p);
    c.fused_hist = nullptr;
    const int64_t total = c.comm ? c.p_total : c.p;
    int kk = (int)(k < total ? k : total);
    int* hs = c.hist + (size_t)(c.set & 1) * TK_HIST_STRIDE;
    int* ho = c.hist + (size_t)((c.set & 1) ^ 1) * TK_HIST_STRIDE;
    ++c.set;
    IHTB_LAUNCH(k_keys_hist0, grid, TK_THREADS, 0, s, c.p, d_dfa, d_b0d, d_sinv, p_mod, d_bounds, eta, bound, d_scal,
                bound_coef, c.wt, c.keyL, c.keyU, hs, d_l2, ho, c.st, c.cand, fill_cand ? c.cap : 0);
    if (c.comm) comm_allreduce_sum_i32(c.comm, hs, TK_BINS, s);
    IHTB_LAUNCH(k_hist_fused, grid, TK_THREADS, 0, s, c.p, c.keyL, hs, 1, kk, hs + TK_BINS);
    if (c.comm) comm_allreduce_sum_i32(c.comm, hs + TK_BINS, TK_BINS, s);
    IHTB_LAUNCH(k_compact_fused, grid, TK_THREADS, 0, s, c.p, c.keyU, hs, kk, c.st, c.cand, c.cap);
}

TopkFuse topk_absdf_fuse_begin(TopkCtx& c, const double* d_sinv, const double* d_scal, double bound_coef) {
    static_assert(TOPK_BINS == TK_BINS, "one bin count");
    int* hs = c.hist + (size_t)(c.set & 1) * TK_HIST_STRIDE;
    int* ho = c.hist + (size_t)((c.set & 1) ^ 1) * TK_HIST_STRIDE;
    ++c.set;
    c.fused_hist = hs;
    TopkFuse f;
    f.keyL = c.keyL; f.keyU = c.keyU; f.hist = hs; f.hist_other = ho; f.st = c.st; f.cand = c.cand; f.cand_fill = c.cap;
    f.scale = d_sinv; f.scal = d_scal; f.bound_coef = bound_coef; f.wt = c.wt;
    return f;
}
void topk_candidates_absdf_finish(TopkCtx& c, int64_t k, cudaStream_t s) {
    IHTB_CHECK(c.fused_hist != nullptr && !c.comm, IHTB_EINVAL, "no fused selection stage pending");
    int* hs = c.fused_hist;
    c.fused_hist = nullptr;
    const int grid = tk_grid(c.p);
    const int kk = (int)(k < c.p ? k : c.p);
    IHTB_LAUNCH(k_hist_fused, grid, TK_THREADS, 0, s, c.p, c.keyL, hs, 1, kk, hs + TK_BINS);
    IHTB_LAUNCH(k_compact_fused, grid, TK_THREADS, 0, s, c.p, c.keyU, hs, kk, c.st, c.cand, c.cap);
}

void topk_candidates(TopkCtx& c, const double* d_dfa, const double* d_b0d, const double* d_sinv, double eta,
                     double bound, int64_t k, cudaStream_t s) {
    topk_run(c, d_dfa, d_b0d, d_sinv, c.p, nullptr, eta, bound, k, s);
}

void topk_candidates_absdf(TopkCtx& c, const double* d_dfa, const double* d_sinv, const double* d_scal,
                           double bound_coef, int64_t k, cudaStream_t s, double host_bound, const double* d_l2) {
    topk_run(c, d_dfa, nullptr, d_sinv, c.p, nullptr, 1.0, (d_scal || d_l2) ? 0.0 : host_bound, k, s, d_scal, bound_coef,
             d_l2, true);
}

__global__ void k_take(const double* __restrict__ src, const int64_t* __restrict__ idx, int64_t k,
                       double* __restrict__ dst) {
    int64_t t = blockIdx.x * (int64_t)blockDim.x + threadIdx.x;
    if (t < k) dst[t] = src[idx[t]];
}
void take_values(const double* d_src, const int64_t* d_idx, int64_t k, double* d_dst, cudaStream_t s) {
    if (k) IHTB_LAUNCH(k_take, (unsigned)ceil_div(k, 128), 128, 0, s, d_src, d_idx, k, d_dst);
}

void topk_candidates_blocked(TopkCtx& c, const double* d_dfa, const double* d_b0d, const double* d_sinv, int64_t p_mod,
                             const double* d_bounds, double eta, int64_t k, cudaStream_t s) {
    topk_run(c, d_dfa, d_b0d, d_sinv, p_mod, d_bounds, eta, 0.0, k, s);
}

__global__ void k_pack_candidates(int64_t* __restrict__ block, int64_t count, const int64_t* __restrict__ gidx,
                                  const double* __restrict__ vals, int capx) {
    int64_t t = blockIdx.x * (int64_t)blockDim.x + threadIdx.x;
    if (t == 0) { block[0] = count; block[1] = 0; }
    if (t < count) {
        block[2 + t] = gidx[t];
        block[2 + capx + t] = __double_as_longlong(vals[t]);
    }
}
__global__ void k_pack_sweep(int64_t* __restrict__ block, const TopkState* __restrict__ st,
                             const int64_t* __restrict__ cand, int glaunch, const double* __restrict__ cand_vals,
                             const int64_t* __restrict__ supp, int nsupp, const double* __restrict__ supp_vals,
                             int64_t j0, int capx) {
    const int half = capx / 2;
    int t = blockIdx.x * blockDim.x + threadIdx.x;
    if (t == 0) { block[0] = st->count; block[1] = nsupp; }
    if (t < half) {
        const bool ok = t < st->count && t < glaunch;
        block[2 + t] = ok ? cand[t] + j0 : -1;
        block[2 + capx + t] = ok ? __double_as_longlong(cand_vals[t]) : 0;
    } else if (t < capx) {
        const int u = t - half;
        const bool ok = u < nsupp;
        block[2 + t] = ok ? supp[u] + j0 : -1;
        block[2 + capx + t] = ok ? __double_as_longlong(supp_vals[u]) : 0;
    }
}
void pack_sweep_candidates(int64_t* d_block, const TopkState* d_st, const int64_t* d_cand, int glaunch,
                           const double* d_cand_vals, const int64_t* d_supp, int nsupp, const double* d_supp_vals,
                           int64_t j0, int capx, cudaStream_t s) {
    IHTB_LAUNCH(k_pack_sweep, (unsigned)ceil_div(capx, 128), 128, 0, s, d_block, d_st, d_cand, glaunch, d_cand_vals,
                d_supp, nsupp, d_supp_vals, j0, capx);
}

void pack_candidates(int64_t* d_block, int64_t count, const int64_t* d_gidx, const double* d_vals, int capx,
                     cudaStream_t s) {
    IHTB_LAUNCH(k_pack_candidates, (unsigned)ceil_div(count > 0 ? count : 1, 128), 128, 0, s, d_block, count, d_gidx,
                d_vals, capx);
}

void scatter_dense(double* d_dst, const int64_t* d_idx, const double* d_val, int64_t k, int zero_only,
                   cudaStream_t s) {
    if (k == 0) return;
    IHTB_LAUNCH(k_scatter, (unsigned)ceil_div(k, 128), 128, 0, s, d_dst, d_idx, d_val, k, zero_only);
}

}
```

Before: 929.5.

## Add programmatic dependent launch, mailbox readbacks, staged uploads and double-banked batch buffers

```diff
diff --git a/mendeliht.jl_b200/csrc/common.cuh b/mendeliht.jl_b200/csrc/common.cuh
--- a/mendeliht.jl_b200/csrc/common.cuh
+++ b/mendeliht.jl_b200/csrc/common.cuh
@@ -47,6 +47,28 @@
                 throw ::ihtb::Error(IHTB_ECUDA, std::string("kernel " #kernel " failed: ") + cudaGetErrorString(e2__)); \
         }                                                            \
     } while (0)
+
+#define IHTB_LAUNCH_PDL(kernel, grid, block, smem, strm, ...)                                                \
+    do {                                                                                                       \
+        cudaLaunchAttribute a__[1];                                                                            \
+        a__[0].id = cudaLaunchAttributeProgrammaticStreamSerialization;                                        \
+        a__[0].val.programmaticStreamSerializationAllowed = 1;                                                 \
+        cudaLaunchConfig_t c__ = {};                                                                           \
+        c__.gridDim = dim3(grid); c__.blockDim = dim3(block); c__.dynamicSmemBytes = (smem); c__.stream = (strm); \
+        c__.attrs = a__; c__.numAttrs = 1;                                                                     \
+        IHTB_CUDA(cudaLaunchKernelEx(&c__, kernel, __VA_ARGS__));                                              \
+        ::ihtb::launch_counter()++;                                                                            \
+        if (::ihtb::debug_sync()) {                                                                            \
+            cudaError_t e2__ = cudaStreamSynchronize(strm);                                                  \
+            if (e2__ != cudaSuccess)                                                                           \
+                throw ::ihtb::Error(IHTB_ECUDA, std::string("kernel " #kernel " failed: ") + cudaGetErrorString(e2__)); \
+        }                                                                                                      \
+    } while (0)
+
+__device__ __forceinline__ void pdl_enter() {
+    asm volatile("griddepcontrol.wait;" ::: "memory");
+    asm volatile("griddepcontrol.launch_dependents;" ::: "memory");
+}
 
 template <typename F>
 static inline int32_t guard(F&& f) {
@@ -106,6 +128,12 @@
         p = nullptr; n = count;
         if (count) IHTB_CUDA(cudaMallocHost((void**)&p, count * sizeof(T)));
     }
+};
+
+template <typename T>
+struct BufView {
+    T* p = nullptr;
+    size_t n = 0;
 };
 
 static inline int64_t ceil_div(int64_t a, int64_t b) { return (a + b - 1) / b; }
diff --git a/mendeliht.jl_b200/csrc/fit.cu b/mendeliht.jl_b200/csrc/fit.cu
--- a/mendeliht.jl_b200/csrc/fit.cu
+++ b/mendeliht.jl_b200/csrc/fit.cu
@@ -45,15 +45,15 @@
     int cap = 4096;
 
     DBuf<unsigned> d_done;
-    DBuf<double> d_y, d_z, d_w, d_xb, d_zc, d_mu, d_r, d_xs, d_dfa, d_part, d_scal, d_small, d_coef, d_gout,
-        d_vbar;
+    DBuf<double> d_y, d_z, d_w, d_xb, d_zc, d_mu, d_r, d_xs, d_dfa, d_part, d_small, d_coef, d_vbar;
     DBuf<uint8_t> d_mask;
     DBuf<uint32_t> d_keyL, d_keyU;
     DBuf<int> d_hist;
-    DBuf<int64_t> d_sel;
     DBuf<int64_t> d_idx, d_cols;
-    HBuf<double> h_scal, h_gout;
-    HBuf<int64_t> h_sel;
+    DBuf<double> d_mbox;
+    HBuf<double> h_mbox;
+    BufView<double> d_scal, d_gout, h_scal, h_gout;
+    BufView<int64_t> d_sel, h_sel;
     void* sweep_scratch = nullptr;
     cudaEvent_t ev0 = nullptr, ev1 = nullptr, tm0 = nullptr, tm1 = nullptr;
     bool sweep_pending = false;
@@ -62,6 +62,9 @@
         size_t maxsupp = 0;
         int M = 0;
         int winner = -1;
+        const int64_t* d_uni = nullptr;
+        const double* d_coef = nullptr;
+        const double* d_cM = nullptr;
     };
     FusedStep* fz = nullptr;
     DBuf<double> d_pick;
@@ -113,6 +116,10 @@
     }
 
     void sync() { IHTB_CUDA(cudaStreamSynchronize(s)); }
+    void readback_mailbox(size_t w0, size_t w1) {
+        IHTB_CUDA(cudaMemcpyAsync(h_mbox.p + w0, d_mbox.p + w0, (w1 - w0) * sizeof(double), cudaMemcpyDeviceToHost, s));
+        sync();
+    }
     void readback_scal(int nv) {
         IHTB_CUDA(cudaMemcpyAsync(h_scal.p, d_scal.p, nv * sizeof(double), cudaMemcpyDeviceToHost, s));
         sync();
@@ -164,7 +171,7 @@
         comm_allreduce_sum_f64(comm, d_out, cnt, s);
     }
 
-    void update_xb() { support_matvec(idx, b, d_xb.p); }
+    void update_xb() { support_matvec(idx, b, glm.xb); }
 
     double glm_update(int add_zc) {
         upload(d_small.p, c.data(), (size_t)q);
@@ -195,7 +202,7 @@
     }
     void fetch_mu() {
         h_mu.resize((size_t)n);
-        IHTB_CUDA(cudaMemcpyAsync(h_mu.data(), d_mu.p, n * sizeof(double), cudaMemcpyDeviceToHost, s));
+        IHTB_CUDA(cudaMemcpyAsync(h_mu.data(), glm.mu, n * sizeof(double), cudaMemcpyDeviceToHost, s));
         sync();
     }
     double nb_logl(double r) {
@@ -276,9 +283,11 @@
         n_cand_iter += (int64_t)need.size();
     }
 
+    bool mailbox_trip() const { return !comm && !(grouped() && !init_plain); }
     void score_and_sweep() {
         glm_score(glm, s, d_vbar.p);
-        IHTB_CUDA(cudaMemcpyAsync(h_scal.p, d_scal.p, (2 + q) * sizeof(double), cudaMemcpyDeviceToHost, s));
+        if (!mailbox_trip())
+            IHTB_CUDA(cudaMemcpyAsync(h_scal.p, d_scal.p, (2 + q) * sizeof(double), cudaMemcpyDeviceToHost, s));
         IHTB_CUDA(cudaEventRecord(ev0, s));
         sweep_coef = geno_bound_coef(g, cfg.sweep_mode == IHTB_SWEEP_FAST ? kFastBound : kExactBound);
         const double t_sw = now();
@@ -286,7 +295,7 @@
             IHTB_CHECK(!grouped() && !comm, IHTB_EUNSUPPORTED, "paired sweeps serve plain single-device fits only");
             if (pairer->sweep(pair_slot, g, d_r.p, d_vbar.p, d_dfa.p, s, sweep_scratch)) {
                 sweep_coef = kPairBound;
-                IHTB_CUDA(cudaMemcpyAsync(h_scal.p + 3 + q, pairer->d_l2 + pair_slot, sizeof(double), cudaMemcpyDeviceToHost, s));
+                IHTB_CUDA(cudaMemcpyAsync(d_scal.p + 3 + q, pairer->d_l2 + pair_slot, sizeof(double), cudaMemcpyDeviceToDevice, s));
             }
         } else if (cfg.k > 0 && !(grouped() && !init_plain)) {
             const TopkFuse tf = topk_absdf_fuse_begin(tk, geno_bound_scale(g), d_scal.p, sweep_coef);
@@ -319,7 +328,8 @@
             for (int64_t j : idx)
                 if (is_local(j)) supp_loc.push_back(j - j0);
         const int nsupp = (int)supp_loc.size();
-        const int64_t* d_supp = fused ? d_idx.p : d_cols.p;
+        const bool staged = !fused && !rerun && win_supp != nullptr;
+        const int64_t* d_supp = fused ? fz->d_uni : staged ? win_supp : d_cols.p;
         int glaunch = 0;
         if (cfg.k > 0) {
             const int64_t ksel = cfg.k + (int64_t)(fused ? fz->maxsupp : idx.size());
@@ -332,29 +342,30 @@
                                                           : ksel + 64;
             glaunch = (int)std::min<int64_t>(comm ? capx / 2 : cap, want);
         }
-        if (nsupp && !fused) upload(d_cols.p, supp_loc.data(), supp_loc.size());
+        if (nsupp && !fused && !staged) upload(d_cols.p, supp_loc.data(), supp_loc.size());
         xt_gather2(g, tk.cand, glaunch, d_supp, nsupp, d_r.p, 1, d_vbar.p, d_gout.p, s);
         denom_ready = false;
         if (!rerun) {
             if (fused) {
-                glm_winner_coef(d_pick.p, d_coefM.p, nsupp, d_gout.p + glaunch, d_coef.p, d_cM.p, q, d_small.p + q, s);
+                glm_winner_coef(d_pick.p, fz->d_coef, nsupp, d_gout.p + glaunch, d_coef.p, fz->d_cM, q, d_small.p + q, s);
                 support_matvec_dev(d_supp, nsupp, d_coef.p, d_xs.p);
                 IHTB_CUDA(cudaMemcpyAsync(h_pick.p, d_pick.p, (size_t)(1 + fz->M) * sizeof(double), cudaMemcpyDeviceToHost, s));
                 IHTB_CUDA(cudaMemcpyAsync(h_scalM.p, d_scalM.p, (size_t)(3 * fz->M) * sizeof(double), cudaMemcpyDeviceToHost, s));
             } else {
                 support_matvec_dev(d_supp, nsupp, d_gout.p + glaunch, d_xs.p);
-                std::vector<double> mask((size_t)q);
-                for (int64_t l = 0; l < q; ++l) mask[l] = idc[l] ? 1.0 : 0.0;
-                upload(d_small.p + q, mask.data(), (size_t)q);
-            }
-            glm_stepsize(glm, d_scal.p + 2, d_xs.p, s, d_small.p + q, d_scal.p + 2 + q);
-            IHTB_CUDA(cudaMemcpyAsync(h_scal.p + 2 + q, d_scal.p + 2 + q, sizeof(double), cudaMemcpyDeviceToHost, s));
+                if (!staged) {
+                    std::vector<double> mask((size_t)q);
+                    for (int64_t l = 0; l < q; ++l) mask[l] = idc[l] ? 1.0 : 0.0;
+                    upload(d_small.p + q, mask.data(), (size_t)q);
+                }
+            }
+            glm_stepsize(glm, d_scal.p + 2, d_xs.p, s, fused || !staged ? d_small.p + q : win_mask, d_scal.p + 2 + q);
+            if (comm) IHTB_CUDA(cudaMemcpyAsync(h_scal.p + 2 + q, d_scal.p + 2 + q, sizeof(double), cudaMemcpyDeviceToHost, s));
             denom_ready = true;
         }
         if (!comm) {
-            IHTB_CUDA(cudaMemcpyAsync(h_sel.p, d_sel.p, (2 + glaunch) * sizeof(int64_t), cudaMemcpyDeviceToHost, s));
-            IHTB_CUDA(cudaMemcpyAsync(h_gout.p, d_gout.p, (glaunch + nsupp) * sizeof(double), cudaMemcpyDeviceToHost, s));
-            sync();
+            const size_t w_sel = d_scal.n, w_gout = w_sel + d_sel.n;
+            readback_mailbox(rerun ? w_sel : 0, w_gout + (size_t)(glaunch + nsupp));
             const double t_host = now();
             struct Acc { double& a; double t0; ~Acc() { a += now() - t0; } } acc_host{dbg[2], t_host};
             if (fused) adopt_winner();
@@ -773,10 +784,10 @@
     }
 
     void compute_pve() {
-        glm_sum2(glm, d_mu.p, d_y.p, s);
+        glm_sum2(glm, glm.mu, d_y.p, s);
         readback_scal(2);
         double mm = h_scal.p[0] / (double)n, my = h_scal.p[1] / (double)n;
-        glm_ssq2(glm, d_mu.p, mm, d_y.p, my, s);
+        glm_ssq2(glm, glm.mu, mm, d_y.p, my, s);
         readback_scal(2);
         pve = h_scal.p[0] / h_scal.p[1];
     }
@@ -892,6 +903,7 @@
         idc.assign(zkeep.begin(), zkeep.end()); idc0 = idc;
         df_exact.clear(); dfs_idx.clear(); dfs_val.clear(); df_sparse = false;
         last_bt = kMaxBatch;
+        set_current(d_xb.p, d_zc.p, d_mu.p);
         d_xb.zero(s);
         const uint8_t* dm = nullptr;
         if (train_mask) {
@@ -974,8 +986,17 @@
     static constexpr int kMaxBatch = 4;
     static constexpr int64_t kAdaptiveBatchN = 131072;
     int last_bt = kMaxBatch;
-    DBuf<double> d_xbM, d_zcM, d_muM, d_partM, d_scalM, d_cM, d_coefM;
+    DBuf<double> d_xbM, d_zcM, d_muM, d_partM, d_scalM;
     HBuf<double> h_scalM;
+    DBuf<double> d_stage;
+    HBuf<double> h_stage;
+    const int64_t* win_supp = nullptr;
+    const double* win_mask = nullptr;
+    void set_current(double* xb, double* zc, double* mu) { glm.xb = xb; glm.zc = zc; glm.mu = mu; }
+    size_t free_bank() const {
+        const bool in0 = glm.xb >= d_xbM.p && glm.xb < d_xbM.p + (size_t)kMaxBatch * n;
+        return in0 ? (size_t)kMaxBatch * n : 0;
+    }
     bool batch_ok() const {
         static const bool off = [] { const char* e = getenv("IHTB_NO_BATCH"); return e && *e == '1'; }();
         return !off && cfg.est_r == 0 && cfg.max_step >= 1 && cfg.max_step + 1 <= kMaxBatch;
@@ -983,14 +1004,20 @@
     struct StepModel { double eta; std::vector<int64_t> idx; std::vector<double> b, c; std::vector<uint8_t> idc; };
     std::vector<StepModel> step_models;
     void ensure_batch_buffers() {
-        if (d_xbM.n < (size_t)(kMaxBatch * n)) {
-            d_xbM.alloc((size_t)(kMaxBatch * n)); d_zcM.alloc((size_t)(kMaxBatch * n)); d_muM.alloc((size_t)(kMaxBatch * n));
+        if (d_xbM.n < (size_t)(2 * kMaxBatch * n)) {
+            const size_t slots = (size_t)(2 * kMaxBatch * n);
+            d_xbM.alloc(slots); d_zcM.alloc(slots); d_muM.alloc(slots);
             d_partM.alloc((size_t)kMaxBatch * GLM_MAX_BLOCKS * 3); d_scalM.alloc(kMaxBatch * 3); h_scalM.alloc(kMaxBatch * 3);
-            d_cM.alloc((size_t)(kMaxBatch * q)); d_coefM.alloc((size_t)kMaxBatch * (size_t)cap);
+            const size_t stage = (size_t)(1 + kMaxBatch) * d_idx.n + (size_t)kMaxBatch * (size_t)cap + 2 * (size_t)(kMaxBatch * q);
+            d_stage.alloc(stage); h_stage.alloc(stage);
             d_pick.alloc(1 + kMaxBatch); h_pick.alloc(1 + kMaxBatch);
         }
     }
-    struct StepPlan { int M; int m0; std::vector<int64_t> uni, loc; size_t UL; };
+    struct StepPlan {
+        int M; int m0; std::vector<int64_t> uni, loc; size_t UL;
+        const int64_t* d_loc; const double* d_coef; const double* d_cM;
+        std::vector<size_t> supp_at, mask_at;
+    };
     StepPlan plan_step(double eta0, int m0 = 0, int m1 = -1) {
         const int Mtot = cfg.max_step + 1;
         if (m1 < 0) m1 = Mtot;
@@ -1011,28 +1038,41 @@
         std::sort(pl.uni.begin(), pl.uni.end());
         pl.uni.erase(std::unique(pl.uni.begin(), pl.uni.end()), pl.uni.end());
         const size_t U = pl.uni.size();
-        IHTB_CHECK(U * (size_t)M <= d_coefM.n && U <= d_idx.n, IHTB_ENUMERIC, "support union too large for the batched step");
+        IHTB_CHECK(U * (size_t)M <= (size_t)kMaxBatch * (size_t)cap && U <= d_idx.n, IHTB_ENUMERIC,
+                   "support union too large for the batched step");
         std::vector<size_t> keep_pos;
         for (size_t t = 0; t < U; ++t)
             if (is_local(pl.uni[t])) { pl.loc.push_back(pl.uni[t] - j0); keep_pos.push_back(t); }
         pl.UL = pl.loc.size();
-        std::vector<double> coefL(pl.UL * (size_t)M, 0.0), cM((size_t)(M * q));
+        double* hs = h_stage.p;
+        int64_t* loc = reinterpret_cast<int64_t*>(hs);
+        std::copy(pl.loc.begin(), pl.loc.end(), loc);
+        double* coefL = hs + pl.UL;
+        double* cM = coefL + pl.UL * (size_t)M;
+        std::fill(coefL, cM, 0.0);
+        size_t w = pl.UL * (size_t)(M + 1) + (size_t)(M * q);
         for (int m = 0; m < M; ++m) {
             const StepModel& md = step_models[(size_t)(m0 + m)];
             size_t u = 0;
+            pl.supp_at.push_back(w);
             for (size_t t = 0; t < md.idx.size(); ++t) {
                 if (!is_local(md.idx[t])) continue;
                 const int64_t lj = md.idx[t] - j0;
                 while (pl.loc[u] != lj) ++u;
                 coefL[u + (size_t)m * pl.UL] = md.b[t];
-            }
-            for (int64_t l = 0; l < q; ++l) cM[(size_t)(m * q + l)] = md.c[(size_t)l];
-        }
-        if (pl.UL) {
-            upload(d_idx.p, pl.loc.data(), pl.UL);
-            upload(d_coefM.p, coefL.data(), coefL.size());
-        }
-        upload(d_cM.p, cM.data(), cM.size());
+                reinterpret_cast<int64_t*>(hs)[w++] = lj;
+            }
+            pl.mask_at.push_back(w);
+            for (int64_t l = 0; l < q; ++l) {
+                cM[(size_t)(m * q + l)] = md.c[(size_t)l];
+                hs[w++] = md.idc[(size_t)l] ? 1.0 : 0.0;
+            }
+        }
+        IHTB_CHECK(w <= d_stage.n, IHTB_ENUMERIC, "support union too large for the batched step");
+        upload(d_stage.p, hs, w);
+        pl.d_loc = reinterpret_cast<const int64_t*>(d_stage.p);
+        pl.d_coef = d_stage.p + pl.UL;
+        pl.d_cM = d_stage.p + pl.UL * (size_t)(M + 1);
         return pl;
     }
     void adopt_model(int m) {
@@ -1062,21 +1102,23 @@
     void finish_batched(const StepPlan& pl, double eta0, double t2, double old_logl, double& eta, int& eta_step,
                         double& new_logl) {
         const int Mtot = cfg.max_step + 1;
+        const size_t bank = free_bank();
         auto eval = [&](const StepPlan& P) {
-            const size_t off = (size_t)P.m0 * (size_t)n;
-            support_matvec_dev_m(P.UL ? d_idx.p : nullptr, (int64_t)P.UL, d_coefM.p, P.M, d_xbM.p + off);
-            glm_mu_batched(glm, d_cM.p, P.M, d_xbM.p + off, d_zcM.p + off, d_muM.p + off, d_partM.p, d_scalM.p + 3 * P.m0, s);
+            const size_t off = bank + (size_t)P.m0 * (size_t)n;
+            support_matvec_dev_m(P.UL ? P.d_loc : nullptr, (int64_t)P.UL, P.d_coef, P.M, d_xbM.p + off);
+            glm_mu_batched(glm, P.d_cM, P.M, d_xbM.p + off, d_zcM.p + off, d_muM.p + off, d_partM.p, d_scalM.p + 3 * P.m0, s);
             IHTB_CUDA(cudaMemcpyAsync(h_scalM.p + 3 * P.m0, d_scalM.p + 3 * P.m0, (size_t)(3 * P.M) * sizeof(double),
                                       cudaMemcpyDeviceToHost, s));
             sync();
         };
         int have = pl.M;
         eval(pl);
+        StepPlan rest;
         int sidx = 0;
         new_logl = logl_from_sums(h_scalM.p);
         while (old_logl > new_logl && sidx < cfg.max_step) {
             ++sidx;
-            if (sidx >= have) { eval(plan_step(eta0, have, Mtot)); have = Mtot; }
+            if (sidx >= have) { rest = plan_step(eta0, have, Mtot); eval(rest); have = Mtot; }
             new_logl = logl_from_sums(h_scalM.p + 3 * sidx);
             ++n_backtracks;
         }
@@ -1084,12 +1126,19 @@
         adopt_model(sidx);
         eta = step_models[(size_t)sidx].eta; eta_step = sidx;
         last_dev = h_scalM.p[3 * sidx];
-        const size_t nb = (size_t)n * sizeof(double);
-        IHTB_CUDA(cudaMemcpyAsync(d_xb.p, d_xbM.p + (size_t)sidx * n, nb, cudaMemcpyDeviceToDevice, s));
-        IHTB_CUDA(cudaMemcpyAsync(d_zc.p, d_zcM.p + (size_t)sidx * n, nb, cudaMemcpyDeviceToDevice, s));
-        IHTB_CUDA(cudaMemcpyAsync(d_mu.p, d_muM.p + (size_t)sidx * n, nb, cudaMemcpyDeviceToDevice, s));
+        const size_t slot = bank + (size_t)sidx * n;
+        set_current(d_xbM.p + slot, d_zcM.p + slot, d_muM.p + slot);
+        const StepPlan& last = sidx < pl.M ? pl : rest;
+        win_supp = reinterpret_cast<const int64_t*>(d_stage.p + last.supp_at[(size_t)(sidx - last.m0)]);
+        win_mask = d_stage.p + last.mask_at[(size_t)(sidx - last.m0)];
         double t3 = now(); phase[2] += t3 - t2;
-        score_and_sweep();
+        try {
+            score_and_sweep();
+        } catch (...) {
+            win_supp = nullptr; win_mask = nullptr;
+            throw;
+        }
+        win_supp = nullptr; win_mask = nullptr;
         phase[3] += now() - t3;
         IHTB_CHECK(!std::isnan(new_logl), IHTB_ENUMERIC, "Loglikelihood function is NaN, aborting...");
         IHTB_CHECK(!std::isinf(new_logl), IHTB_ENUMERIC, "Loglikelihood function is Inf, aborting...");
@@ -1115,11 +1164,13 @@
             finish_batched(pl, eta0, t2, old_logl, eta, eta_step, new_logl);
             return;
         }
-        support_matvec_dev_m(pl.UL ? d_idx.p : nullptr, (int64_t)pl.UL, d_coefM.p, M, d_xbM.p);
-        glm_mu_batched(glm, d_cM.p, M, d_xbM.p, d_zcM.p, d_muM.p, d_partM.p, d_scalM.p, s);
-        glm_pick_model(glm, d_scalM.p, M, old_logl, cfg.max_step, d_pick.p, d_xbM.p, d_zcM.p, d_muM.p, s);
+        const size_t bank = free_bank();
+        support_matvec_dev_m(pl.UL ? pl.d_loc : nullptr, (int64_t)pl.UL, pl.d_coef, M, d_xbM.p + bank);
+        glm_mu_batched(glm, pl.d_cM, M, d_xbM.p + bank, d_zcM.p + bank, d_muM.p + bank, d_partM.p, d_scalM.p, s);
+        glm_pick_model(glm, d_scalM.p, M, old_logl, cfg.max_step, d_pick.p, d_xbM.p + bank, d_zcM.p + bank, d_muM.p + bank, s);
         FusedStep ctx;
         ctx.uni_loc = pl.loc; ctx.M = M;
+        ctx.d_uni = pl.d_loc; ctx.d_coef = pl.d_coef; ctx.d_cM = pl.d_cM;
         for (const StepModel& md : step_models) ctx.maxsupp = std::max(ctx.maxsupp, md.idx.size());
         double t3 = now(); phase[2] += t3 - t2;
         fz = &ctx;
@@ -1265,12 +1316,18 @@
     IHTB_CUDA(cudaEventCreate(&f->ev1));
     f->d_y.alloc(n); f->d_z.alloc(n * q); f->d_w.alloc(n); f->d_xb.alloc(n); f->d_zc.alloc(n); f->d_mu.alloc(n);
     f->d_r.alloc(n); f->d_xs.alloc(n + 2 * (size_t)cap + 64); f->d_dfa.alloc(p); f->d_mask.alloc(n);
-    f->d_part.alloc((size_t)GLM_MAX_BLOCKS * (2 + q)); f->d_scal.alloc(2 + q + 8); f->d_small.alloc(2 * q);
+    f->d_part.alloc((size_t)GLM_MAX_BLOCKS * (2 + q)); f->d_small.alloc(2 * q);
     size_t cols_cap = 2 * (size_t)cap + 64;
-    f->d_coef.alloc(cols_cap); f->d_gout.alloc(cols_cap); f->d_vbar.alloc(1);
+    f->d_coef.alloc(cols_cap); f->d_vbar.alloc(1);
     f->d_idx.alloc(cols_cap); f->d_cols.alloc(cols_cap);
-    f->d_keyL.alloc(p); f->d_keyU.alloc(p); f->d_hist.alloc(2 * 3 * 2048); f->d_sel.alloc(2 + cap);
-    f->h_scal.alloc(2 + q + 8); f->h_gout.alloc(cols_cap); f->h_sel.alloc(2 + cap);
+    f->d_keyL.alloc(p); f->d_keyU.alloc(p); f->d_hist.alloc(2 * 3 * 2048);
+    static_assert(sizeof(int64_t) == sizeof(double), "the mailbox is laid out in 8-byte words");
+    const size_t nscal = 2 + (size_t)q + 8, nsel = 2 + (size_t)cap;
+    f->d_mbox.alloc(nscal + nsel + cols_cap); f->h_mbox.alloc(nscal + nsel + cols_cap);
+    f->d_scal = {f->d_mbox.p, nscal}; f->h_scal = {f->h_mbox.p, nscal};
+    f->d_sel = {reinterpret_cast<int64_t*>(f->d_mbox.p + nscal), nsel};
+    f->h_sel = {reinterpret_cast<int64_t*>(f->h_mbox.p + nscal), nsel};
+    f->d_gout = {f->d_mbox.p + nscal + nsel, cols_cap}; f->h_gout = {f->h_mbox.p + nscal + nsel, cols_cap};
     f->sweep_scratch = sweep_scratch_create();
     f->d_hist.zero(f->s);
     return f.release();
@@ -1429,8 +1486,8 @@
             for (size_t t = 0; t < f->best_idx.size(); ++t) beta[f->best_idx[t]] = f->best_b[t];
         }
         if (c) std::copy(f->best_c.begin(), f->best_c.end(), c);
-        if (mu) IHTB_CUDA(cudaMemcpy(mu, f->d_mu.p, f->n * sizeof(double), cudaMemcpyDeviceToHost));
-        if (xb) IHTB_CUDA(cudaMemcpy(xb, f->d_xb.p, f->n * sizeof(double), cudaMemcpyDeviceToHost));
+        if (mu) IHTB_CUDA(cudaMemcpy(mu, f->glm.mu, f->n * sizeof(double), cudaMemcpyDeviceToHost));
+        if (xb) IHTB_CUDA(cudaMemcpy(xb, f->glm.xb, f->n * sizeof(double), cudaMemcpyDeviceToHost));
     });
 }
 
diff --git a/mendeliht.jl_b200/csrc/glm.cu b/mendeliht.jl_b200/csrc/glm.cu
--- a/mendeliht.jl_b200/csrc/glm.cu
+++ b/mendeliht.jl_b200/csrc/glm.cu
@@ -39,6 +39,7 @@
          double* __restrict__ zc, double* __restrict__ mu, const double* __restrict__ y, const double* __restrict__ w,
          int dist, int link, double nb_r, int add_zc, double* __restrict__ part, double* __restrict__ out = nullptr,
          unsigned* __restrict__ done = nullptr) {
+    pdl_enter();
     __shared__ double sh[32];
     c += blockIdx.y * q; xb += blockIdx.y * n; zc += blockIdx.y * n; mu += blockIdx.y * n;
     part += (int64_t)blockIdx.y * gridDim.x * 3;
@@ -111,6 +112,7 @@
            const double* __restrict__ zc,
            const double* __restrict__ mu, const double* __restrict__ w, int dist, int link, double nb_r,
            double* __restrict__ part, double* __restrict__ out = nullptr, unsigned* __restrict__ done = nullptr) {
+    pdl_enter();
     __shared__ double sh[32];
     double a = 0.0;
     for (int64_t i = blockIdx.x * (int64_t)blockDim.x + threadIdx.x; i < n; i += (int64_t)gridDim.x * blockDim.x) {
@@ -289,7 +291,7 @@
 void glm_mu_batched(GlmCtx& c, const double* d_cM, int M, double* xbM, double* zcM, double* muM, double* d_partM,
                     double* d_scalM, cudaStream_t s) {
     int grid = glm_grid(c.n);
-    IHTB_LAUNCH(k_glm_mu, dim3(grid, M), GLM_THREADS, 0, s, c.n, c.q, c.Z, d_cM, xbM, zcM, muM, c.y, c.w, c.dist, c.link,
+    IHTB_LAUNCH_PDL(k_glm_mu, dim3(grid, M), GLM_THREADS, 0, s, c.n, c.q, c.Z, d_cM, xbM, zcM, muM, c.y, c.w, c.dist, c.link,
                 c.nb_r, 1, d_partM, d_scalM, c.done);
     if (!c.done) IHTB_LAUNCH(k_finalize, dim3(1, M), 96, 0, s, d_partM, grid, 3, d_scalM);
 }
@@ -347,7 +349,7 @@
 void glm_stepsize(GlmCtx& c, const double* d_d2, const double* d_xs, cudaStream_t s, const double* d_d2mask,
                   double* d_out) {
     int grid = glm_grid(c.n);
-    IHTB_LAUNCH(k_stepsize, grid, GLM_THREADS, 0, s, c.n, c.q, c.Z, d_d2, d_d2mask, d_xs, c.xb, c.zc, c.mu, c.w, c.dist,
+    IHTB_LAUNCH_PDL(k_stepsize, grid, GLM_THREADS, 0, s, c.n, c.q, c.Z, d_d2, d_d2mask, d_xs, c.xb, c.zc, c.mu, c.w, c.dist,
                 c.link, c.nb_r, c.part, d_out ? d_out : c.scal, c.done);
     if (!c.done) IHTB_LAUNCH(k_finalize, 1, 32, 0, s, c.part, grid, 1, d_out ? d_out : c.scal);
 }
diff --git a/mendeliht.jl_b200/csrc/support.cu b/mendeliht.jl_b200/csrc/support.cu
--- a/mendeliht.jl_b200/csrc/support.cu
+++ b/mendeliht.jl_b200/csrc/support.cu
@@ -13,6 +13,7 @@
 __global__ void __launch_bounds__(256)
 k_x_support(GenoView gv, const int64_t* __restrict__ idx, int64_t k, const double* __restrict__ coef,
             double* __restrict__ out, P2PView pv, unsigned long long seq) {
+    pdl_enter();
     const int64_t nbytes = gv.nbytes, n = gv.n;
     const double* __restrict__ mu = gv.mu;
     const double* __restrict__ sinv = gv.sinv;
@@ -84,7 +85,7 @@
 template <int M>
 static void launch_x_support(const ihtb_geno* g, const int64_t* d_idx, int64_t k, const double* d_coef, double* d_out,
                              cudaStream_t s) {
-    IHTB_LAUNCH((k_x_support<M, false>), (unsigned)ceil_div(g->nbytes, 256), 256, 0, s, geno_view(g), d_idx, k, d_coef,
+    IHTB_LAUNCH_PDL((k_x_support<M, false>), (unsigned)ceil_div(g->nbytes, 256), 256, 0, s, geno_view(g), d_idx, k, d_coef,
                 d_out, P2PView{}, 0ull);
 }
 
@@ -179,6 +180,7 @@
 k_xt_gather_nib(GenoView gv, const int64_t* __restrict__ cols, int64_t n_a, const int64_t* __restrict__ cols_b,
                 int64_t ncols, const double* __restrict__ v, const double* __restrict__ vbar,
                 double* __restrict__ part ) {
+    pdl_enter();
     __shared__ double T[8][16][32];
     const int64_t n = gv.n;
     const int64_t chunk = blockIdx.x, nchunks = gridDim.x;
@@ -213,6 +215,7 @@
                     const int64_t* __restrict__ cols, int64_t n_a, const int64_t* __restrict__ cols_b, int64_t ncols,
                     int nchunks, const double* __restrict__ v, const double* __restrict__ vbar,
                     const double* __restrict__ part, double* __restrict__ out) {
+    pdl_enter();
     const int64_t c = (blockIdx.x * (int64_t)blockDim.x + threadIdx.x) >> 5;
     const int lane = threadIdx.x & 31;
     if (c >= ncols) return;
@@ -253,9 +256,9 @@
             sc.alloc(need_b < 65536 ? 65536 : need_b);
         }
         int groups = (int)std::max<int64_t>(1, std::min<int64_t>(ceil_div(ncols, 8), (8 * g->sm_count) / nchunks + 1));
-        IHTB_LAUNCH(k_xt_gather_nib, dim3((unsigned)nchunks, (unsigned)groups), 256, 0, s, geno_view(g), d_cols, n_a,
+        IHTB_LAUNCH_PDL(k_xt_gather_nib, dim3((unsigned)nchunks, (unsigned)groups), 256, 0, s, geno_view(g), d_cols, n_a,
                     d_cols_b, ncols, d_v, d_vbar, sc.p);
-        IHTB_LAUNCH(k_xt_gather_fin_nib, (unsigned)ceil_div(ncols * 32, 128), 128, 0, s, geno_view(g), g->miss_ptr.p,
+        IHTB_LAUNCH_PDL(k_xt_gather_fin_nib, (unsigned)ceil_div(ncols * 32, 128), 128, 0, s, geno_view(g), g->miss_ptr.p,
                     g->miss_idx.p, d_cols, n_a, d_cols_b, ncols, nchunks, d_v, d_vbar, sc.p, d_out);
         return;
     }
diff --git a/mendeliht.jl_b200/csrc/sweep.cu b/mendeliht.jl_b200/csrc/sweep.cu
--- a/mendeliht.jl_b200/csrc/sweep.cu
+++ b/mendeliht.jl_b200/csrc/sweep.cu
@@ -84,6 +84,7 @@
                  const double* __restrict__ vbar_p,
                  int impute, double* __restrict__ out, const float* __restrict__ scale_p = nullptr,
                  TopkFuse tf = TopkFuse()) {
+    pdl_enter();
     __shared__ int sh[TOPK_BINS];
     const bool fuse = tf.keyL != nullptr;
     if (fuse) {
@@ -223,7 +224,7 @@
                 int64_t n_slabs = sweep_fast_num_slabs(g);
                 if (sc->part32.n < (size_t)(n_slabs * g->p)) sc->part32.alloc((size_t)(n_slabs * g->p));
                 sweep_fast_partials(g, v, d_vbar + t, sc->part32.p, &n_slabs, s);
-                IHTB_LAUNCH((k_sweep_epilogue<float>), (unsigned)ceil_div(g->p, 256), 256, 0, s, sc->part32.p, n_slabs,
+                IHTB_LAUNCH_PDL((k_sweep_epilogue<float>), (unsigned)ceil_div(g->p, 256), 256, 0, s, sc->part32.p, n_slabs,
                             g->p, g->mu.p, g->sinv.p, g->nmiss.p, g->miss_ptr.p, g->miss_idx.p, v, d_vbar + t,
                             g->impute, out, (const float*)nullptr, fuse);
             }
diff --git a/mendeliht.jl_b200/csrc/topk.cu b/mendeliht.jl_b200/csrc/topk.cu
--- a/mendeliht.jl_b200/csrc/topk.cu
+++ b/mendeliht.jl_b200/csrc/topk.cu
@@ -90,6 +90,7 @@
 __global__ void __launch_bounds__(TK_THREADS)
 k_hist_fused(int64_t p, const uint32_t* __restrict__ keyL, const int* __restrict__ hists , int pass, int kk,
              int* __restrict__ hist_out) {
+    pdl_enter();
     __shared__ int sh[TK_BINS];
     __shared__ int sh_scan[32];
     __shared__ int sh_out[2];
@@ -118,6 +119,7 @@
 __global__ void __launch_bounds__(TK_THREADS)
 k_compact_fused(int64_t p, const uint32_t* __restrict__ keyU, const int* __restrict__ hists, int kk,
                 TopkState* __restrict__ st, int64_t* __restrict__ cand, int cap) {
+    pdl_enter();
     __shared__ int sh_scan[32];
     __shared__ int sh_out[2];
     block_pick(hists, TK_BINS, kk, sh_scan, sh_out);
@@ -177,8 +179,8 @@
     c.fused_hist = nullptr;
     const int grid = tk_grid(c.p);
     const int kk = (int)(k < c.p ? k : c.p);
-    IHTB_LAUNCH(k_hist_fused, grid, TK_THREADS, 0, s, c.p, c.keyL, hs, 1, kk, hs + TK_BINS);
-    IHTB_LAUNCH(k_compact_fused, grid, TK_THREADS, 0, s, c.p, c.keyU, hs, kk, c.st, c.cand, c.cap);
+    IHTB_LAUNCH_PDL(k_hist_fused, grid, TK_THREADS, 0, s, c.p, c.keyL, hs, 1, kk, hs + TK_BINS);
+    IHTB_LAUNCH_PDL(k_compact_fused, grid, TK_THREADS, 0, s, c.p, c.keyU, hs, kk, c.st, c.cand, c.cap);
 }
 
 void topk_candidates(TopkCtx& c, const double* d_dfa, const double* d_b0d, const double* d_sinv, double eta,
```

Result: faster. 953.9 (median of 6 runs) (+2.6%).
